# MrTornado24/IDE-3D

Measured on AMD Instinct MI355X. Metric: 512x512 RGB+seg frames/s @96 depth samples (whole job), higher is better.
Workload: dtype f32 (3x3 convs + MLPs: fp32 operands as 3 bf16 pieces, 6 products, f32 accumulate); 1 GPU; BASELINE config 2: random-init ide3d-ffhq-64-512, G.mapping + G.synthesis (64 render -> 512, 96 samples, RGB + 19-class seg) + uint8 frames, batch 4 seeds per GPU; global_batch=4, parallelism=dp1, conv_arithmetic=bf16x6, conv_arithmetic_is_library_default=True

## Files before the change

### ide-3d_amd/csrc/camera.hip

```cpp
#include "common.h"
#include "raymarch_ray.h"

namespace ide3d {

#pragma clang fp contract(off)

struct V3 { float x, y, z; };
__device__ __forceinline__ V3 normalized(V3 v) {
    const float n = sqrtf(v.x * v.x + v.y * v.y + v.z * v.z);
    return V3{v.x / n, v.y / n, v.z / n};
}
__device__ __forceinline__ V3 cross(V3 a, V3 b) { return V3{a.y * b.z - a.z * b.y, a.z * b.x - a.x * b.z, a.x * b.y - a.y * b.x}; }

__global__ void __launch_bounds__(64)
sphere_points_kernel(const float* __restrict__ theta, const float* __restrict__ pitch, int n, float r, int pitch_is_v,
                     float* __restrict__ pos, float* __restrict__ phi_out) {
    const int i = blockIdx.x * 64 + threadIdx.x;
    if (i >= n) return;
    const float kPi = 3.14159265358979323846f;
    float p = fminf(fmaxf(pitch[i], 1e-5f), (float)(3.14159265358979323846 - 1e-5));
    if (pitch[i] != pitch[i]) p = pitch[i];
    if (pitch_is_v) p = acosf(1.f - 2.f * (p * (1.f / kPi)));
    const float t = theta[i], sp = r * sinf(p);
    pos[3 * i + 0] = sp * cosf(t);
// ... 16 lines not shown
        f = V3{forward[3 * i], forward[3 * i + 1], forward[3 * i + 2]};
    }
    f = normalized(f);
    const V3 left = normalized(cross(V3{0.f, 1.f, 0.f}, f));
    const V3 up = normalized(cross(f, left));
    float* m = out + (int64_t)i * 16;
    m[0] = -left.x; m[1] = up.x; m[2]  = -f.x; m[3]  = o.x;
    m[4] = -left.y; m[5] = up.y; m[6]  = -f.y; m[7]  = o.y;
    m[8] = -left.z; m[9] = up.z; m[10] = -f.z; m[11] = o.z;
    m[12] = 0.f;    m[13] = 0.f; m[14] = 0.f;  m[15] = 1.f;
}

__global__ void __launch_bounds__(256)
plane_cells_kernel(ide3d_render_params p, int cells_h, int cells_w, int lds_cells, uint8_t* __restrict__ cells) {
    extern __shared__ __attribute__((aligned(16))) uint8_t s_cells[];
    const int n = blockIdx.y, per_img = p.rays_per_img * p.steps;
    const int i = (int)blockIdx.x * 256 + (int)threadIdx.x;
    uint8_t* const img_cells = cells + (int64_t)n * 3 * cells_h * cells_w;
    if (lds_cells) {
        for (int k = threadIdx.x * 4; k < lds_cells; k += 1024) *reinterpret_cast<uint32_t*>(s_cells + k) = 0u;
        __syncthreads();
    }
    if (i < per_img) {
        const int s = i % p.steps, r = i / p.steps;
        const float zstep = (p.steps > 1) ? (p.z_lin[1] - p.z_lin[0]) : 0.f;
        const float zl = p.z_lin[s];
        float ax, ay, az, bx, by, bz;
        ray_world_point(p, n, r, zl, 0.f, zstep, ax, ay, az);
        ray_world_point(p, n, r, zl, 1.f, zstep, bx, by, bz);
        Tap2 ta[3], tb[3];
        triplane_taps(ax, ay, az, p.W, p.H, ta);
        triplane_taps(bx, by, bz, p.W, p.H, tb);
        uint8_t* const dst = lds_cells ? s_cells : img_cells;
#pragma unroll
        for (int pl = 0; pl < 3; ++pl) {
            const int x_lo = min(max(min(ta[pl].ix0, tb[pl].ix0) - 1, 0), p.W - 1), x_hi = min(max(max(ta[pl].ix0, tb[pl].ix0) + 2, 0), p.W - 1);
            const int y_lo = min(max(min(ta[pl].iy0, tb[pl].iy0) - 1, 0), p.H - 1), y_hi = min(max(max(ta[pl].iy0, tb[pl].iy0) + 2, 0), p.H - 1);
            uint8_t* const c = dst + pl * cells_h * cells_w;
            for (int cy = y_lo >> 2; cy <= (y_hi >> 2); ++cy)
                for (int cx = x_lo >> 2; cx <= (x_hi >> 2); ++cx) c[cy * cells_w + cx] = 1;
        }
    }
    if (lds_cells) {
        __syncthreads();
        for (int k = threadIdx.x * 4; k < lds_cells; k += 1024) {
            const uint32_t v = *reinterpret_cast<const uint32_t*>(s_cells + k);
            if (v == 0u) continue;
#pragma unroll
            for (int e = 0; e < 4; ++e) if ((v >> (8 * e)) & 0xffu) img_cells[k + e] = 1;
        }
    }
}

__global__ void __launch_bounds__(1024)
plane_tile_list_kernel(ide3d_plane_gate g, int n, int tiles_y, int tiles_x, int th, int tw, int32_t* __restrict__ list) {
    __shared__ int s_wave[16];
    const int tid = threadIdx.x, lane = tid & 63, wid = tid >> 6;
    const int total = n * tiles_y * tiles_x;
    int base = 0;
    for (int t0 = 0; t0 < total; t0 += 1024) {
        const int t = t0 + tid;
        bool live = false;
        if (t < total) {
            const int tx = t % tiles_x, ty = (t / tiles_x) % tiles_y, img = t / (tiles_x * tiles_y);
            const int cy0 = (ty * th) >> 2, cy1 = min((ty * th + th - 1) >> 2, g.cells_h - 1);
            const int cx0 = (tx * tw) >> 2, cx1 = min((tx * tw + tw - 1) >> 2, g.cells_w - 1);
            for (int pl = 0; pl < 3; ++pl)
                for (int cy = cy0; cy <= cy1; ++cy)
                    for (int cx = cx0; cx <= cx1; ++cx) live |= g.cells[(((int64_t)img * 3 + pl) * g.cells_h + cy) * g.cells_w + cx] != 0;
        }
        const unsigned long long bal = __builtin_amdgcn_ballot_w64(live);
        if (lane == 0) s_wave[wid] = __popcll(bal);
        __syncthreads();
        int before = base;
        for (int w = 0; w < wid; ++w) before += s_wave[w];
        if (live) list[1 + before + __popcll(bal & ((1ull << lane) - 1ull))] = t;
        for (int w = 0; w < 16; ++w) base += s_wave[w];
        __syncthreads();
    }
    if (tid == 0) list[0] = base;
}

}

extern "C" int ide3d_plane_cells(const float* rays_d_cam, const float* z_lin, const float* cam2world, int32_t n, int32_t rays_per_img,
                                 int32_t steps, int32_t H, int32_t W, uint8_t* cells, void* stream) {
    using namespace ide3d;
    IDE3D_CHECK_ARG(rays_d_cam && z_lin && cam2world && cells, "plane_cells: null pointer");
    IDE3D_CHECK_ARG(n > 0 && rays_per_img > 0 && steps > 0 && H > 0 && W > 0, "plane_cells: bad shape");
    const int cells_h = cdiv(H, 4), cells_w = cdiv(W, 4);
    const int64_t per_img = (int64_t)rays_per_img * steps, map_bytes = 3 * (int64_t)cells_h * cells_w;
    IDE3D_CHECK_ARG(per_img < 0x7fffff00LL && n <= 65535 && n * map_bytes < 0x7fffffffLL, "plane_cells: too many samples, images or cells");
    ide3d_render_params p{};
    p.rays_d_cam = rays_d_cam; p.z_lin = z_lin; p.cam2world = cam2world;
    p.jitter = z_lin;
    p.n = n; p.rays_per_img = rays_per_img; p.steps = steps; p.H = H; p.W = W;
    hipStream_t st = (hipStream_t)stream;
    const hipError_t e = hipMemsetAsync(cells, 0, (size_t)(n * map_bytes), st);
    if (e != hipSuccess) { set_error("plane_cells: hipMemsetAsync: %s", hipGetErrorString(e)); return IDE3D_ELAUNCH; }
    const int lds_cells = (map_bytes % 4 == 0 && map_bytes <= 48 * 1024) ? (int)map_bytes : 0;
    hipLaunchKernelGGL(plane_cells_kernel, dim3((unsigned)cdiv64(per_img, 256), (unsigned)n), dim3(256), (size_t)lds_cells, st, p, cells_h, cells_w, lds_cells, cells);
    IDE3D_CHECK_LAUNCH("plane_cells");
    return IDE3D_OK;
}

extern "C" int ide3d_plane_tile_list(const ide3d_plane_gate* gate, int32_t n, int32_t h, int32_t w, int32_t tile_h, int32_t tile_w, int32_t* list, void* stream) {
    using namespace ide3d;
    IDE3D_CHECK_ARG(gate && gate->cells && list, "plane_tile_list: null pointer");
    IDE3D_CHECK_ARG(n > 0 && h > 0 && w > 0 && tile_h > 0 && tile_w > 0 && tile_h % 4 == 0 && tile_w % 4 == 0, "plane_tile_list: bad shape (tiles are multiples of the 4 x 4 cell)");
    IDE3D_CHECK_ARG(4 * (int64_t)gate->cells_h >= h && 4 * (int64_t)gate->cells_w >= w, "plane_tile_list: the cell map does not cover the output");
    const int tiles_y = cdiv(h, tile_h), tiles_x = cdiv(w, tile_w);
    IDE3D_CHECK_ARG((int64_t)n * tiles_y * tiles_x < 0x7fffffffLL, "plane_tile_list: too many tiles");
    hipLaunchKernelGGL(plane_tile_list_kernel, dim3(1), dim3(1024), 0, (hipStream_t)stream, *gate, n, tiles_y, tiles_x, tile_h, tile_w, list);
    IDE3D_CHECK_LAUNCH("plane_tile_list");
    return IDE3D_OK;
}

extern "C" int ide3d_sphere_points(const float* theta, const float* pitch, int32_t n, float r, int32_t pitch_is_v,
                                   float* pos, float* phi_out, void* stream) {
    using namespace ide3d;
    IDE3D_CHECK_ARG(theta && pitch && pos, "sphere_points: null pointer");
    IDE3D_CHECK_ARG(n > 0, "sphere_points: bad shape");
    hipLaunchKernelGGL(sphere_points_kernel, dim3(cdiv(n, 64)), dim3(64), 0, (hipStream_t)stream, theta, pitch, n, r, pitch_is_v, pos, phi_out);
    IDE3D_CHECK_LAUNCH("sphere_points");
    return IDE3D_OK;
}

extern "C" int ide3d_cam2world(const float* forward, const float* origin, const float* lookat, int32_t lookat_stride, int32_t n,
                               float* out, void* stream) {
    using namespace ide3d;
    IDE3D_CHECK_ARG(origin && out && (forward || lookat), "cam2world: null pointer");
    IDE3D_CHECK_ARG(n > 0 && (lookat_stride == 0 || lookat_stride == 3), "cam2world: bad shape");
    hipLaunchKernelGGL(cam2world_kernel, dim3(cdiv(n, 64)), dim3(64), 0, (hipStream_t)stream, forward, origin, lookat, lookat_stride, n, out);
    IDE3D_CHECK_LAUNCH("cam2world");
    return IDE3D_OK;
}
```

### ide-3d_amd/csrc/common.h

```cpp
#pragma once

#include <hip/hip_runtime.h>
#include <hip/hip_fp16.h>
#include <hip/hip_bf16.h>
#include <stdint.h>
#include <stdarg.h>
#include <stdio.h>

#include "../../include/ide3d_hip.h"

namespace ide3d {

constexpr int kWave = 64;
constexpr int kNumCU = 256;
constexpr int kNumXCD = 8;


void set_error(const char* fmt, ...);

const char* modconv_build_flags();
const char* triplane_tile_build_flags();
const char* raymarch_build_flags();

void note_exclusive_violation(const char* kernel, int blocks_per_cu);
// ... 55 lines not shown

__device__ __forceinline__ void amax_raise(float* amax, int n, float v) {
    unsigned* const slot = reinterpret_cast<unsigned*>(amax) + (size_t)n * IDE3D_AMAX_FLOATS + (blockIdx.x % IDE3D_AMAX_SLOTS) * IDE3D_AMAX_STRIDE;
    __hip_atomic_fetch_max(slot, __float_as_uint(v), __ATOMIC_RELAXED, __HIP_MEMORY_SCOPE_AGENT);
}
__device__ __forceinline__ void amax_raise_block(float* amax, int n, float v, float* scratch) {
#pragma unroll
    for (int off = 32; off > 0; off >>= 1) v = fmaxf(v, __shfl_xor(v, off));
    __syncthreads();
    if ((threadIdx.x & 63) == 0) scratch[threadIdx.x >> 6] = v;
    __syncthreads();
    if (threadIdx.x == 0) {
        float m = scratch[0];
        for (int i = 1; i < (int)(blockDim.x >> 6); ++i) m = fmaxf(m, scratch[i]);
        if (m > 0.f) amax_raise(amax, n, m);
    }
}
__device__ __forceinline__ void amax_lds_flush(unsigned* s_am, int n, float v) { if (v > 0.f) atomicMax(&s_am[n & 63], __float_as_uint(v)); }
__device__ __forceinline__ void amax_lds_commit(float* amax, const unsigned* s_am, int p_n) {
    __syncthreads();
    if ((int)threadIdx.x < p_n && threadIdx.x < 64 && s_am[threadIdx.x] != 0u) amax_raise(amax, (int)threadIdx.x, __uint_as_float(s_am[threadIdx.x]));
}

__host__ __device__ __forceinline__ int64_t cdiv64(int64_t a, int64_t b) { return (a + b - 1) / b; }
__host__ __device__ __forceinline__ int     cdiv(int a, int b) { return (a + b - 1) / b; }

__device__ __forceinline__ bool pool_gt(float v, float m) { return v > m || v != v; }

inline bool ptr_aligned(const void* p, uintptr_t bytes) { return (reinterpret_cast<uintptr_t>(p) & (bytes - 1)) == 0; }

inline int stream_grid(int64_t work_items, int per_block) {
    int64_t g = cdiv64(work_items, per_block);
    const int64_t cap = (int64_t)kNumCU * 8;
    if (g > cap) g = cap;
    if (g < 1) g = 1;
    return (int)g;
}

__device__ __forceinline__ bool plane_gate_live(const ide3d_plane_gate& g, int n, int pl0, int npl, int y0, int x0, int th, int tw) {
    const int cy0 = max(y0 >> 2, 0), cx0 = max(x0 >> 2, 0);
    const int cy1 = min((y0 + th - 1) >> 2, g.cells_h - 1), cx1 = min((x0 + tw - 1) >> 2, g.cells_w - 1);
    const int nx = cx1 - cx0 + 1, ny = cy1 - cy0 + 1;
    bool any = false;
    if (nx > 0 && ny > 0) {
        const int per = nx * ny, count = per * npl;
        for (int i = (int)(threadIdx.x & 63u); i < count; i += 64) {
            const int pl = pl0 + i / per, r = i % per;
            any |= g.cells[(((int64_t)n * 3 + pl) * g.cells_h + cy0 + r / nx) * g.cells_w + cx0 + r % nx] != 0;
        }
    }
    return __builtin_amdgcn_ballot_w64(any) != 0ull;
}
ide3d_plane_gate resolve_plane_gate(const ide3d_plane_gate* gate);

__device__ __forceinline__ int xcd_remap(int bid, int nblocks) {
    const int xcd = bid % kNumXCD;
    const int idx = bid / kNumXCD;
    const int q = nblocks / kNumXCD, r = nblocks % kNumXCD;
    const int base = (xcd < r) ? xcd * (q + 1) : r * (q + 1) + (xcd - r) * q;
    return base + idx;
}

}
```

### ide-3d_amd/csrc/core.hip

```cpp
#include "common.h"
#include "knobs.h"
#include <string.h>
#include <stdio.h>
#include <map>
#include <mutex>
#include <tuple>

namespace ide3d {

static thread_local char g_err[512] = "";

void set_error(const char* fmt, ...) {
    va_list ap;
    va_start(ap, fmt);
    vsnprintf(g_err, sizeof(g_err), fmt, ap);
    va_end(ap);
}

static int g_excl_violations = 0;
static char g_excl_text[384] = "";
void note_exclusive_violation(const char* kernel, int blocks_per_cu) {
    ++g_excl_violations;
    snprintf(g_excl_text, sizeof(g_excl_text), "%d workgroups of %.200s fit one CU of this device: exclusive residency (DESIGN.md 4.2) does not hold", blocks_per_cu, kernel);
    fprintf(stderr, "[libide3d_hip] %s; the launch is refused (select IDE3D_CONV_ARITH=fp32)\n", g_excl_text);
}
int exclusive_violations() { return g_excl_violations; }
static thread_local bool g_refused = false;
void refuse_launch(const char* kernel) {
    g_refused = true;
    set_error("%.200s: more than one workgroup fits a CU of this device, exclusive residency (DESIGN.md 4.2) does not hold; launch refused "
              "(IDE3D_CONV_ARITH=fp32 selects the arithmetic that needs none)", kernel);
}
bool take_refused() { const bool r = g_refused; g_refused = false; return r; }

bool exclusive_checked(const void* kernel, int threads, size_t dyn_lds, const char* name) {
    static std::mutex mu;
    static std::map<std::tuple<const void*, int, int, size_t>, int> table;
    int dev = 0;
    if (hipGetDevice(&dev) != hipSuccess) return true;
    int occ;
    {
        std::lock_guard<std::mutex> lock(mu);
        const auto key = std::make_tuple(kernel, dev, threads, dyn_lds);
        auto it = table.find(key);
        if (it == table.end()) {
            int n = 0;
            occ = (hipOccupancyMaxActiveBlocksPerMultiprocessor(&n, kernel, threads, dyn_lds) == hipSuccess && n > 0) ? n : -1;
            table.emplace(key, occ);
            if (occ > 1) note_exclusive_violation(name, occ);
        } else occ = it->second;
    }
    if (occ > 1) refuse_launch(name);
    return occ <= 1;
}

ide3d_plane_gate resolve_plane_gate(const ide3d_plane_gate* gate) {
    if (!gate || !gate->cells || knob_live("IDE3D_NO_PLANE_GATE")) return ide3d_plane_gate{};
    return *gate;
}

}

extern "C" int ide3d_exclusive_violations(void) { return ide3d::g_excl_violations; }
extern "C" const char* ide3d_exclusive_violation_text(void) { return ide3d::g_excl_text; }
extern "C" const char* ide3d_last_error(void) { return ide3d::g_err; }
extern "C" int ide3d_abi_version(void) { return 8; }
extern "C" const char* ide3d_build_arch(void) { return "gfx950"; }
extern "C" const char* ide3d_build_flags(void) {
    static char buf[512] = "";
    static bool done = false;
    if (!done) {
        snprintf(buf, sizeof(buf), "%s%s%s", ide3d::modconv_build_flags(), ide3d::triplane_tile_build_flags(), ide3d::raymarch_build_flags());
        const size_t n = strlen(buf);
        if (n && buf[n - 1] == ' ') buf[n - 1] = 0;
        done = true;
    }
    return buf;
}
```

### ide-3d_amd/csrc/modconv.hip

```cpp
#include "common.h"
#include "knobs.h"
#include <stdlib.h>
#include <string.h>
#include <type_traits>

namespace ide3d {

typedef float f32x16 __attribute__((ext_vector_type(16)));

#ifdef IDE3D_MC_TRACE
__device__ unsigned long long g_mc_dbg[256];
#define IDE3D_MC_TS(k) { const unsigned long long now_ = __builtin_readcyclecounter(); mc_acc[k] += now_ - mc_last; mc_last = now_; }
#else
#define IDE3D_MC_TS(k)
#endif

enum { MODE_CONV3 = 0, MODE_CONV1 = 1, MODE_TCONV3 = 2, MODE_TCONV3A = 3, MODE_CONV3S2 = 4 };

template <int MODE> struct ModeCfg;
template <> struct ModeCfg<MODE_CONV3>  { static constexpr int KC = 4, WTAPS = 9, MAXT = 9; };
template <> struct ModeCfg<MODE_CONV1>  { static constexpr int KC = 16, WTAPS = 1, MAXT = 1; };
template <> struct ModeCfg<MODE_CONV3S2> { static constexpr int KC = 4, WTAPS = 9, MAXT = 9; };
template <> struct ModeCfg<MODE_TCONV3> { static constexpr int KC = 4, WTAPS = 9, MAXT = 4; };
template <> struct ModeCfg<MODE_TCONV3A> { static constexpr int KC = 4, WTAPS = 9, MAXT = 9; };
// ... 1368 lines not shown
                                       : (TI * PH * PW <= 128 && MODE != MODE_CONV3S2) ? 3 : 2)
modconv_kernel(ide3d_modconv_params p, const float* __restrict__ wp, float* __restrict__ partial, ConvGeom g) {
    using K = McCfg<MODE, BIG, TI, PH, PW>;
    __shared__ __attribute__((aligned(16))) float s_w[2 * K::LDS_W];
    __shared__ __attribute__((aligned(16))) float s_x[2 * K::LDS_X];
    const BlockId b = decode_block(g);
    int cls = 0;
    if (MODE == MODE_TCONV3) { cls = (b.tile >= g.tile_base[1]) + (b.tile >= g.tile_base[2]) + (b.tile >= g.tile_base[3]); }
    modconv_tile<MODE, BIG, TI, PH, PW>(p, wp, partial, g, s_w, s_x, b.mb, b.tile - g.tile_base[cls], b.grp, b.split, cls, g.tiles_x[cls]);
}


#ifdef IDE3D_SP_SHARED_SIMD
constexpr bool kSpExclusive = false;
#else
constexpr bool kSpExclusive = true;
#endif
template <int MODE, int BIG, int PH, int PARTS, int WBUF, int NWV>
constexpr int sp_waves_per_simd() {
    using K = SpCfg<MODE, BIG, PH, PARTS, WBUF, NWV>;
    return (NWV == 8) ? 2 : (!kSpExclusive && K::LDS_BYTES <= 80 * 1024 && (WBUF == 1 || K::NCLS * K::MTW * K::NTW <= 8)) ? 2 : 1;
}
template <int MODE, int BIG, int PH, int PARTS, int WBUF = 2, int NWV = 4, int F16 = 0>
__global__ void __launch_bounds__(64 * NWV, (sp_waves_per_simd<MODE, BIG, PH, PARTS, WBUF, NWV>()))
modconv_split_kernel(ide3d_modconv_params p, const u32x4* __restrict__ wp, float* __restrict__ partial, ConvGeom g, const float* __restrict__ row_unscale) {
    using K = SpCfg<MODE, BIG, PH, PARTS, WBUF, NWV>;
    if constexpr (kSpExclusive) { if constexpr (NWV == 8) asm volatile("" ::: "v255"); else asm volatile("" ::: "v255", "a255"); }
    __shared__ __attribute__((aligned(16))) unsigned char sp_smem[K::LDS_BYTES];
    const BlockId b = decode_block(g);
    modconv_split_tile<MODE, BIG, PH, PARTS, WBUF, NWV, F16>(p, wp, partial, g, sp_smem, b.mb, b.tile, b.grp, b.split, g.tiles_x[0], row_unscale);
}

template <int BIG, int PH, int HEAD_MT>
__global__ void __launch_bounds__(512, 2)
modconv_split_heads_kernel(ide3d_modconv_params p, const u32x4* __restrict__ wp, ConvGeom g, HeadEpi he) {
    using K = SpCfg<MODE_CONV3, BIG, PH, 3, 2, 8>;
    if constexpr (kSpExclusive) asm volatile("" ::: "v255");
    __shared__ __attribute__((aligned(16))) unsigned char sp_smem[K::LDS_BYTES];
    BlockId b;
    if (he.gate.tile_list) {
        const int live = __builtin_amdgcn_readfirstlane(he.gate.tile_list[0]);
        if ((int)blockIdx.x >= live) return;
        const int id = __builtin_amdgcn_readfirstlane(he.gate.tile_list[1 + xcd_remap(blockIdx.x, live)]);
        b.mb = 0; b.split = 0; b.tile = id % g.tile_base[4]; b.grp = id / g.tile_base[4];
    } else {
        b = decode_block(g);
        if (he.gate.cells && !plane_gate_live(he.gate, b.grp, 0, 3, (b.tile / g.tiles_x[0]) * PH, (b.tile % g.tiles_x[0]) * K::PW, PH, K::PW)) return;
    }
    modconv_split_tile<MODE_CONV3, BIG, PH, 3, 2, 8, 0, 1, -1, HEAD_MT>(p, wp, nullptr, g, sp_smem, b.mb, b.tile, b.grp, b.split, g.tiles_x[0], nullptr, nullptr, &he);
}

template <int BIG, int PH, int PARTS, int F16 = 0>
__global__ void __launch_bounds__(512, 2)
modconv_split_pair_kernel(ide3d_modconv_params p, const u32x4* __restrict__ wp, float* __restrict__ partial, ConvGeom g, const float* __restrict__ row_unscale) {
    using K = SpCfg<MODE_TCONV3A, BIG, PH, PARTS, 2, 8, 1>;
    if constexpr (kSpExclusive) asm volatile("" ::: "v255");
    __shared__ __attribute__((aligned(16))) unsigned char sp_smem[K::LDS_BYTES];
    const int half_grid = (int)(gridDim.x >> 1);
    const int par = __builtin_amdgcn_readfirstlane((int)blockIdx.x >= half_grid ? 1 : 0);
    int bid = xcd_remap((int)blockIdx.x - par * half_grid, half_grid);
    BlockId b;
    b.mb = bid % g.mblocks; bid /= g.mblocks;
    b.tile = bid % g.tile_base[4]; bid /= g.tile_base[4];
    b.grp = bid % g.img_groups; bid /= g.img_groups;
    b.split = bid;
    if (par == 0) modconv_split_tile<MODE_TCONV3A, BIG, PH, PARTS, 2, 8, F16, 1, 0>(p, wp, partial, g, sp_smem, b.mb, b.tile, b.grp, b.split, g.tiles_x[0], row_unscale);
    else          modconv_split_tile<MODE_TCONV3A, BIG, PH, PARTS, 2, 8, F16, 1, 1>(p, wp, partial, g, sp_smem, b.mb, b.tile, b.grp, b.split, g.tiles_x[0], row_unscale);
}

template <int MODE, int BIG, int PH, int PARTS, int WBUF, int F16>
__global__ void __launch_bounds__(512, 2)
modconv_split_teams_kernel(ide3d_modconv_params p, const u32x4* __restrict__ wp, float* __restrict__ partial, ConvGeom g, const float* __restrict__ row_unscale) {
    using K = SpCfg<MODE, BIG, PH, PARTS, WBUF, 4>;
    static_assert(2 * K::LDS_BYTES <= 160 * 1024, "both teams' LDS must fit");
    asm volatile("" ::: "v255");
    __shared__ __attribute__((aligned(16))) unsigned char sp_smem[2 * K::LDS_BYTES];
    const int team = (int)(threadIdx.x >> 8);
    int bid = xcd_remap(blockIdx.x, gridDim.x);
    const int mpairs = g.mblocks >> 1;
    BlockId b;
    b.mb = 2 * (bid % mpairs) + team; bid /= mpairs;
    b.tile = bid % g.tile_base[4]; bid /= g.tile_base[4];
    b.grp = bid % g.img_groups; bid /= g.img_groups;
    b.split = bid;
    modconv_split_tile<MODE, BIG, PH, PARTS, WBUF, 4, F16, 2>(p, wp, partial, g, sp_smem + team * K::LDS_BYTES, b.mb, b.tile, b.grp, b.split, g.tiles_x[0], row_unscale,
                                                              reinterpret_cast<float*>(sp_smem));
}

__global__ void __launch_bounds__(256)
modconv_epilogue_kernel(ide3d_modconv_params p, const float* __restrict__ partial, int split_k, int oh, int ow) {
    const int64_t per = (int64_t)p.n * p.cout * oh * ow;
    const int64_t stride = (int64_t)gridDim.x * blockDim.x;
    int am_n = -1; float am = 0.f;
    __shared__ unsigned s_am[64];
    const bool am_lds = p.y_amax && p.n <= 64;
    if (p.y_amax) { if (threadIdx.x < 64) s_am[threadIdx.x] = 0u; __syncthreads(); }
    const int hw = oh * ow;
    if (p.y_pitch <= 0 && (hw & 3) == 0) {
        typedef float f32x4v __attribute__((ext_vector_type(4)));
        const int64_t per4 = per >> 2;
        for (int64_t q = (int64_t)blockIdx.x * blockDim.x + threadIdx.x; q < per4; q += stride) {
            const int64_t i = q << 2;
            f32x4v v = {0.f, 0.f, 0.f, 0.f};
            int s = 0;
            for (; s + 4 <= split_k; s += 4) {
                f32x4v t[4];
#pragma unroll
                for (int k = 0; k < 4; ++k) t[k] = *reinterpret_cast<const f32x4v*>(partial + (int64_t)(s + k) * per + i);
#pragma unroll
                for (int k = 0; k < 4; ++k) v += t[k];
            }
            for (; s < split_k; ++s) v += *reinterpret_cast<const f32x4v*>(partial + (int64_t)s * per + i);
            const int pix = (int)(i % hw);
            const int co = (int)((i / hw) % p.cout);
            const int n = (int)(i / ((int64_t)hw * p.cout));
            const float d = p.dcoefs ? p.dcoefs[(int64_t)n * p.cout + co] : 1.f, bb = p.bias ? p.bias[co] : 0.f;
#pragma unroll
            for (int e = 0; e < 4; ++e) {
// ... 200 lines not shown
        g.tiles_x[c] = cdiv(gw[c], ts.cols); g.tiles_y[c] = cdiv(gh[c], ts.rows);
        g.tile_base[c + 1] = g.tile_base[c] + (c < ncls ? g.tiles_x[c] * g.tiles_y[c] : 0);
    }
    g.img_groups = cdiv(p.n, ts.images);
    g.mblocks = pl.mblocks; g.cchunks = pl.cchunks; g.oh = pl.oh; g.ow = pl.ow;
    const int64_t base_blocks = (int64_t)g.mblocks * g.tile_base[4] * g.img_groups;
    int split = 1;
    if (base_blocks < split_min && pl.cchunks >= 8) {
        split = (int)cdiv64(768, base_blocks);
        if (split > pl.cchunks / 4) split = pl.cchunks / 4;
        if (split > 16) split = 16;
        if (split < 1) split = 1;
    }
    if (one_round) want_split = 1;
    if (want_split > 0) split = want_split < pl.cchunks ? want_split : pl.cchunks;
    g.chunks_per_split = cdiv(pl.cchunks, split);
    g.split_k = cdiv(pl.cchunks, g.chunks_per_split);
    pl.partial_floats = (g.split_k > 1) ? (int64_t)g.split_k * p.n * p.cout * pl.oh * pl.ow : 0;
}

template <int MODE, int BIG>
static void launch_tiles(const ide3d_modconv_params& p, const ConvPlan& pl, const float* wp, float* partial, hipStream_t st) {
    const ConvGeom& g = pl.g;
    const unsigned nblocks = (unsigned)((int64_t)g.mblocks * g.tile_base[4] * g.img_groups * g.split_k);
    if constexpr (MODE == MODE_TCONV3A) {
        if constexpr (BIG != 0) {
            if (pl.tile == TA8x16) hipLaunchKernelGGL((modconv_kernel<MODE, BIG, 1, 8, 16>), dim3(nblocks), dim3(256), 0, st, p, wp, partial, g);
            else if (pl.tile == TA16x16) { if constexpr (BIG == 2) hipLaunchKernelGGL((modconv_kernel<MODE, BIG, 1, 16, 16>), dim3(nblocks), dim3(256), 0, st, p, wp, partial, g); }
            else hipLaunchKernelGGL((modconv_kernel<MODE, BIG, 1, 4, 16>), dim3(nblocks), dim3(256), 0, st, p, wp, partial, g);
        }
    } else
    if (pl.tile == TFLAT128) {
        if constexpr (MODE == MODE_CONV1)
            hipLaunchKernelGGL((modconv_kernel<MODE, BIG, 1, 1, 128>), dim3(nblocks), dim3(256), 0, st, p, wp, partial, g);
    }
    else if (pl.tile == T8x16) hipLaunchKernelGGL((modconv_kernel<MODE, BIG, 1, 8, 16>), dim3(nblocks), dim3(256), 0, st, p, wp, partial, g);
    else if (pl.tile == T2x8x8) hipLaunchKernelGGL((modconv_kernel<MODE, BIG, 2, 8, 8>), dim3(nblocks), dim3(256), 0, st, p, wp, partial, g);
    else if (pl.tile == T8x4x4) hipLaunchKernelGGL((modconv_kernel<MODE, BIG, 8, 4, 4>), dim3(nblocks), dim3(256), 0, st, p, wp, partial, g);
    else if constexpr (BIG == 1 && MODE != MODE_CONV1 && MODE != MODE_CONV3S2)
        hipLaunchKernelGGL((modconv_kernel<MODE, BIG, 1, 16, 16>), dim3(nblocks), dim3(256), 0, st, p, wp, partial, g);
}


struct SpForm { int waves; bool teams; };
static SpForm sp_form(const ConvPlan& pl) {
    if constexpr (kSpExclusive) {
        if (pl.tile == TA4x16) return {4, pl.big == 2 && (pl.mblocks & 1) == 0};
        return {pl.tile == T8x16 ? 4 : 8, false};
    } else {
        return {(pl.tile == T16x16 || pl.tile == T32x16) ? 8 : 4, false};
    }
}
template <int MODE, int BIG, int PARTS, int F16 = 0>
static void launch_split(const ide3d_modconv_params& p, const ConvPlan& pl, const float* wp, float* partial, hipStream_t st) {
    const ConvGeom& g = pl.g;
    const unsigned nblocks = (unsigned)((int64_t)g.mblocks * g.tile_base[4] * g.img_groups * g.split_k);
    const u32x4* wu = reinterpret_cast<const u32x4*>(wp);
    const float* ru = F16 ? wp + pl.packed_floats + (int64_t)pl.mblocks * pl.bm : nullptr;
    if constexpr (kSpExclusive) {
        if (pl.pair) {
            if constexpr (MODE == MODE_TCONV3A) IDE3D_EXCL_LAUNCH((modconv_split_pair_kernel<BIG, (BIG == 1 ? 16 : 32), PARTS, F16>), dim3(2 * nblocks), 512, 0, st, p, wu, partial, g, ru);
        }
        else if (pl.tile == TA4x16) {
            if constexpr (MODE == MODE_TCONV3A) {
                if (sp_form(pl).teams) { if constexpr (BIG == 2) IDE3D_EXCL_LAUNCH((modconv_split_teams_kernel<MODE, BIG, 4, PARTS, 2, F16>), dim3(nblocks / 2), 512, 0, st, p, wu, partial, g, ru); }
                else IDE3D_EXCL_LAUNCH((modconv_split_kernel<MODE, BIG, 4, PARTS, 2, 4, F16>), dim3(nblocks), 256, 0, st, p, wu, partial, g, ru);
            }
        }
        else if (pl.tile == T8x16) {
            if constexpr (MODE == MODE_CONV3) IDE3D_EXCL_LAUNCH((modconv_split_kernel<MODE, BIG, 8, PARTS, 2, 4, F16>), dim3(nblocks), 256, 0, st, p, wu, partial, g, ru);
        }
        else if (pl.tile == TA8x16) {
            if constexpr (MODE == MODE_TCONV3A) IDE3D_EXCL_LAUNCH((modconv_split_kernel<MODE, BIG, 8, PARTS, 2, 8, F16>), dim3(nblocks), 512, 0, st, p, wu, partial, g, ru);
        }
        else if (pl.tile == T32x16) {
            if constexpr (MODE == MODE_CONV3 && BIG == 2) IDE3D_EXCL_LAUNCH((modconv_split_kernel<MODE, BIG, 32, PARTS, 2, 8, F16>), dim3(nblocks), 512, 0, st, p, wu, partial, g, ru);
        }
        else if constexpr (MODE == MODE_CONV3 || BIG == 2)
            IDE3D_EXCL_LAUNCH((modconv_split_kernel<MODE, BIG, 16, PARTS, 2, 8, F16>), dim3(nblocks), 512, 0, st, p, wu, partial, g, ru);
    } else {
        if (pl.tile == TA4x16) {
            if constexpr (MODE == MODE_TCONV3A) IDE3D_EXCL_LAUNCH((modconv_split_kernel<MODE, BIG, 4, PARTS, 2, 4, F16>), dim3(nblocks), 256, 0, st, p, wu, partial, g, ru);
        }
        else if (pl.tile == T8x16) {
            if constexpr (MODE == MODE_CONV3) IDE3D_EXCL_LAUNCH((modconv_split_kernel<MODE, BIG, 8, PARTS, 1, 4, F16>), dim3(nblocks), 256, 0, st, p, wu, partial, g, ru);
        }
        else if (pl.tile == TA8x16) {
            if constexpr (MODE == MODE_TCONV3A && BIG == 2) IDE3D_EXCL_LAUNCH((modconv_split_kernel<MODE, BIG, 8, PARTS, 2, 4, F16>), dim3(nblocks), 256, 0, st, p, wu, partial, g, ru);
        }
        else if (pl.tile == T16x16) {
            if constexpr (MODE == MODE_CONV3 && BIG == 1) IDE3D_EXCL_LAUNCH((modconv_split_kernel<MODE, BIG, 16, PARTS, 2, 8, F16>), dim3(nblocks), 512, 0, st, p, wu, partial, g, ru);
        }
    }
}

}

static bool head_split_applies(const ide3d_modconv_params& p, int arith) {
    return arith != 1 && p.k == 1 && p.mode == 0 && p.w_batch_stride > 0 && !p.styles && !p.dcoefs && !p.noise && p.act == 1 &&
           (p.cout <= 32 || (p.cout > 160 && p.cout <= 192)) && p.cin >= 32 &&
           (int64_t)p.n * ide3d::cdiv64((int64_t)p.h * p.w_, 32 * ide3d::head_waves(p.cout <= 32 ? 1 : 6)) >= ide3d::kNumCU;
}

static bool head_small_applies(const ide3d_modconv_params& p) {
    return p.k == 1 && p.mode == 0 && p.w_batch_stride > 0 && !p.styles && !p.dcoefs && !p.noise && p.act == 1 && (int64_t)p.h * p.w_ <= 256 &&
           p.y_pitch == 0 && p.n <= 65535;
}
static bool head_resident_applies(const ide3d_modconv_params& p) {
    const int mt = p.cout <= 32 ? 1 : 6, cchunks = ide3d::cdiv(p.cin, 16);
    const int hw = p.h * p.w_, wgs_img = ide3d::kNumCU / p.n, tiles32 = hw / 32;
    return ide3d::kSpExclusive && p.cin % 16 == 0 && hw % 32 == 0 && wgs_img >= 1 && p.y_pitch == 0 &&
           ((mt == 1 && (cchunks == 4 || cchunks == 8)) || (mt == 6 && cchunks == 8)) && tiles32 >= 2 * wgs_img * 8;
}

// ... 2 lines not shown
    IDE3D_CHECK_ARG(p.n > 0 && p.cin > 0 && p.cout > 0 && p.h > 0 && p.w_ > 0, "modconv2d: bad shape");
    IDE3D_CHECK_ARG(p.k == 1 || p.k == 3, "modconv2d: kernel size must be 1 or 3 (got %d)", p.k);
    IDE3D_CHECK_ARG(p.mode == 0 || ((p.mode == 1 || p.mode == 2) && p.k == 3),
                    "modconv2d: mode must be 0 (conv), 1 (3x3 stride-2 conv, no padding) or 2 (3x3 transposed, stride 2)");
    IDE3D_CHECK_ARG(p.mode != 1 || (p.h >= 3 && p.w_ >= 3), "modconv2d: stride-2 convolution needs an input of at least 3x3");
    IDE3D_CHECK_ARG((int64_t)p.n * p.cin * p.h * p.w_ < 0x7fffffffLL, "modconv2d: input too large for 32-bit indexing");
    return IDE3D_OK;
}

extern "C" int64_t ide3d_modconv_workspace_bytes(int32_t n, int32_t cin, int32_t cout, int32_t h, int32_t w, int32_t k, int32_t mode,
                                                 int32_t per_image_weights) {
    using namespace ide3d;
    ide3d_modconv_params p{};
    p.n = n; p.cin = cin; p.cout = cout; p.h = h; p.w_ = w; p.k = k; p.mode = mode; p.w_batch_stride = per_image_weights ? 1 : 0;
    if (check_modconv(p) != IDE3D_OK) return -1;
    p.x = nullptr;
    int64_t packed = 0, part = 0;
    static const float dummy = 0.f;
    for (int epi = 0; epi < 2; ++epi) {
        ide3d_modconv_params q0 = p;
        q0.act = 1; q0.gain = 1.f; q0.clamp = -1.f;
        if (epi == 1) { q0.noise = &dummy; q0.bias = &dummy; q0.noise_strength = 1.f; q0.act = 3; q0.alpha = 0.2f; q0.gain = 1.41421356f; }
        for (int arith : {1, 3, 6, 16}) {
            ConvPlan pl; plan_conv(q0, pl, arith);
            ConvPlan pf; plan_conv(flatten_pointwise(q0), pf, arith);
            for (const ConvPlan* q : {&pl, &pf}) {
                if (q->packed_floats + q->aux_floats > packed) packed = q->packed_floats + q->aux_floats;
                if (q->partial_floats > part) part = q->partial_floats;
            }
        }
    }
    int64_t bytes = (packed + part) * (int64_t)sizeof(float);
    if (per_image_weights && k == 1) {
        const int64_t hb = head_packed_units(n, cdiv(cin, 16), 3, cout <= 32 ? 1 : 6) * 16;
        if (hb > bytes) bytes = hb;
    }
    return bytes;
}

static void pack_split_weights(const ide3d_modconv_params& p, const ide3d::ConvPlan& pl, float* wp, hipStream_t st) {
    using namespace ide3d;
    const int64_t items = (int64_t)pl.mblocks * pl.cchunks * 9 * 2 * pl.bm;
    if (pl.f16) {
        float* const rs = wp + pl.packed_floats;
        const int rows = pl.mblocks * pl.bm;
        hipLaunchKernelGGL(modconv_row_scale_kernel, dim3(cdiv(rows, 4)), dim3(256), 0, st, p.w, p.cout, p.cin * 9, rows, rs, rs + rows);
        hipLaunchKernelGGL((modconv_pack_split_kernel<2, 1>), dim3(stream_grid(items, 256)), dim3(256), 0, st, p.w, p.cout, p.cin, pl.bm, pl.mblocks, pl.cchunks, reinterpret_cast<u32x4*>(wp), rs);
    }
    else if (pl.parts == 2) hipLaunchKernelGGL(modconv_pack_split_kernel<2>, dim3(stream_grid(items, 256)), dim3(256), 0, st, p.w, p.cout, p.cin, pl.bm, pl.mblocks, pl.cchunks, reinterpret_cast<u32x4*>(wp), nullptr);
    else               hipLaunchKernelGGL(modconv_pack_split_kernel<3>, dim3(stream_grid(items, 256)), dim3(256), 0, st, p.w, p.cout, p.cin, pl.bm, pl.mblocks, pl.cchunks, reinterpret_cast<u32x4*>(wp), nullptr);
}

extern "C" int ide3d_modconv2d(const ide3d_modconv_params* pp, void* stream) {
    using namespace ide3d;
    IDE3D_CHECK_ARG(pp != nullptr, "modconv2d: null params");
    const ide3d_modconv_params p = flatten_pointwise(*pp);
    IDE3D_CHECK_ARG(p.x && p.w && p.y && p.workspace, "modconv2d: null tensor / workspace pointer");
    int rc = check_modconv(p);
    if (rc) return rc;
    IDE3D_CHECK_ARG(p.act == 1 || p.act == 3, "modconv2d: act must be linear (1) or lrelu (3)");
    IDE3D_CHECK_ARG(p.y_pitch == 0 || (p.mode == 2 && p.y_pitch >= 2 * p.w_ + 1), "modconv2d: y_pitch is the row pitch of a transposed convolution's output (>= 2 w + 1), or 0");
    hipStream_t st_head = (hipStream_t)stream;
    {
        const int64_t hw = (int64_t)p.h * p.w_;
        if (head_small_applies(p)) {
            if (hw <= 64) hipLaunchKernelGGL((head_small_kernel<64, 32>), dim3(cdiv(p.cout, HS_RB), 1, p.n), dim3(HS_THREADS), 0, st_head, p, (int)hw);
            else          hipLaunchKernelGGL((head_small_kernel<256, 8>), dim3(cdiv(p.cout, HS_RB), cdiv((int)hw, 256), p.n), dim3(HS_THREADS), 0, st_head, p, (int)hw);
            IDE3D_CHECK_LAUNCH("modconv2d (small-map heads)");
            return IDE3D_OK;
        }
    }
    if (head_split_applies(p, resolve_arith(p.arith))) {
        const int parts = resolve_arith(p.arith) == 3 ? 2 : 3, mt = p.cout <= 32 ? 1 : 6, cchunks = cdiv(p.cin, 16);
        IDE3D_CHECK_ARG(p.workspace_bytes >= head_packed_units(p.n, cchunks, parts, mt) * 16, "modconv2d: workspace too small for the packed head weights");
        u32x4* wu = reinterpret_cast<u32x4*>(p.workspace);
        const int64_t items = (int64_t)p.n * cchunks * 2 * mt * 32;
        const int tiles = cdiv(p.h * p.w_, 32 * head_waves(mt));
        const int hw_h = p.h * p.w_, wgs_img = kNumCU / p.n, tiles32 = hw_h / 32;
        const bool resident = head_resident_applies(p);
#define IDE3D_HEAD_RES(P, M, C) IDE3D_EXCL_LAUNCH((head_resident_kernel<P, M, C>), dim3(p.n * wgs_img), 512, 0, st_head, p, wu, wgs_img, tiles32)
#define IDE3D_HEAD(P, M) do { \
            hipLaunchKernelGGL(head_pack_split_kernel<P>, dim3(stream_grid(items, 256)), dim3(256), 0, st_head, p.w, p.w_batch_stride, p.n, p.cout, p.cin, M * 32, cchunks, wu); \
            if (resident) { if (M == 6) IDE3D_HEAD_RES(P, 6, 8); else if (cchunks == 4) IDE3D_HEAD_RES(P, 1, 4); else IDE3D_HEAD_RES(P, 1, 8); } \
            else IDE3D_EXCL_LAUNCH((head_split_kernel<P, M>), dim3(p.n * tiles), 64 * head_waves(M), 0, st_head, p, wu, cchunks, tiles); } while (0)
        if (parts == 2) { if (mt == 1) IDE3D_HEAD(2, 1); else IDE3D_HEAD(2, 6); }
        else            { if (mt == 1) IDE3D_HEAD(3, 1); else IDE3D_HEAD(3, 6); }
#undef IDE3D_HEAD
#undef IDE3D_HEAD_RES
        IDE3D_CHECK_LAUNCH("modconv2d (split-bf16 heads)");
        return IDE3D_OK;
    }
    int arith_eff = resolve_arith(p.arith);
    if (arith_eff == 16 && !p.x_amax) arith_eff = 6;
    ConvPlan pl; plan_conv(p, pl, arith_eff);
    IDE3D_CHECK_ARG(p.workspace_bytes >= (pl.packed_floats + pl.aux_floats + pl.partial_floats) * (int64_t)sizeof(float),
                    "modconv2d: workspace too small (need %lld bytes)", (long long)((pl.packed_floats + pl.aux_floats + pl.partial_floats) * sizeof(float)));
    hipStream_t st = (hipStream_t)stream;
    float* wp = p.workspace;
    float* partial = p.workspace + pl.packed_floats + pl.aux_floats;
    if (pl.parts) {
        if (!p.weights_packed) pack_split_weights(p, pl, wp, st);
#define IDE3D_SP_DISPATCH(M) \
        do { if (pl.big == 1) { if (pl.f16) launch_split<M, 1, 2, 1>(p, pl, wp, partial, st); else if (pl.parts == 2) launch_split<M, 1, 2>(p, pl, wp, partial, st); else launch_split<M, 1, 3>(p, pl, wp, partial, st); } \
             else             { if (pl.f16) launch_split<M, 2, 2, 1>(p, pl, wp, partial, st); else if (pl.parts == 2) launch_split<M, 2, 2>(p, pl, wp, partial, st); else launch_split<M, 2, 3>(p, pl, wp, partial, st); } } while (0)
        if (pl.mode == MODE_CONV3) IDE3D_SP_DISPATCH(MODE_CONV3); else IDE3D_SP_DISPATCH(MODE_TCONV3A);
#undef IDE3D_SP_DISPATCH
    } else {
    if (!p.weights_packed) {
        hipLaunchKernelGGL(modconv_pack_kernel, dim3(stream_grid(pl.packed_floats, 256)), dim3(256), 0, st,
                           p.w, p.w_batch_stride, p.w_batch_stride ? p.n : 1, p.cout, p.cin, pl.taps, pl.bm, pl.kc, pl.mblocks, pl.cchunks, wp);
    }
#define IDE3D_MC_DISPATCH(M) \
    do { if (pl.big == 1) launch_tiles<M, 1>(p, pl, wp, partial, st); else if (pl.big == 2) launch_tiles<M, 2>(p, pl, wp, partial, st); \
         else launch_tiles<M, 0>(p, pl, wp, partial, st); } while (0)
    if (pl.mode == MODE_CONV3)       IDE3D_MC_DISPATCH(MODE_CONV3);
    else if (pl.mode == MODE_CONV1)  IDE3D_MC_DISPATCH(MODE_CONV1);
    else if (pl.mode == MODE_CONV3S2) IDE3D_MC_DISPATCH(MODE_CONV3S2);
    else if (pl.mode == MODE_TCONV3A) IDE3D_MC_DISPATCH(MODE_TCONV3A);
    else                             IDE3D_MC_DISPATCH(MODE_TCONV3);
#undef IDE3D_MC_DISPATCH
    }
    if (pl.g.split_k > 1) {
        const int64_t per = (int64_t)p.n * p.cout * pl.oh * pl.ow;
        hipLaunchKernelGGL(modconv_epilogue_kernel, dim3(stream_grid((p.y_pitch <= 0 && ((pl.oh * pl.ow) & 3) == 0) ? per / 4 : per, 256)), dim3(256), 0, st, p, partial, pl.g.split_k, pl.oh, pl.ow);
    }
    if (pl.mode == MODE_TCONV3A && !p.weights_packed) {
        hipLaunchKernelGGL(tconv_strip_pack_kernel, dim3(stream_grid(pl.strip_floats, 256)), dim3(256), 0, st, p.w, p.cout, p.cin, cdiv(p.cout, STRIP_CO) * STRIP_CO,
                           wp + pl.packed_floats + pl.strip_off);
    }
    if (pl.strip) {
        const int cout_pad = cdiv(p.cout, STRIP_CO) * STRIP_CO;
        float* const wstrip = wp + pl.packed_floats + pl.strip_off;
        const int nb_re = cdiv(p.w_ + 1, 64), nb_ro = cdiv(p.w_, 64), nb_ce = cdiv(p.h, 64), nb_co = cdiv(p.h, 64);
        float* const xs = wstrip + pl.strip_floats;
        hipLaunchKernelGGL(tconv_strip_gather_kernel, dim3(stream_grid((int64_t)p.n * p.cin * (p.h + p.w_), 256)), dim3(256), 0, st, p.x, p.n * p.cin, p.h, p.w_, xs);
        hipLaunchKernelGGL(tconv_strip_kernel, dim3(nb_re + nb_ro + nb_ce + nb_co, cout_pad / STRIP_CO, p.n), dim3(64 * STRIP_WAVES), 0, st, p, wstrip, xs, cout_pad,
                           pl.oh, pl.ow, (int64_t)(p.y_pitch > 0 ? p.y_pitch : pl.ow), nb_re, nb_ro, nb_ce);
    }
    IDE3D_CHECK_LAUNCH("modconv2d");
    return IDE3D_OK;
}

extern "C" int ide3d_modconv2d_heads(const ide3d_modconv_params* pp, const ide3d_modconv_head_epilogue* hp, void* stream) {
    return ide3d_modconv2d_heads_gated(pp, hp, nullptr, stream);
}

extern "C" int ide3d_modconv2d_heads_gated(const ide3d_modconv_params* pp, const ide3d_modconv_head_epilogue* hp, const ide3d_plane_gate* gate, void* stream) {
    using namespace ide3d;
    IDE3D_CHECK_ARG(pp != nullptr && hp != nullptr, "modconv2d_heads: null params");
    const ide3d_modconv_params& p = *pp;
    const ide3d_modconv_head_epilogue& h = *hp;
    IDE3D_CHECK_ARG(p.x && p.w && p.workspace && (p.y || h.no_activation_output) && h.w && h.y && h.workspace, "modconv2d_heads: null tensor / workspace pointer");
    int rc = check_modconv(p);
    if (rc) return rc;
    IDE3D_CHECK_ARG(p.act == 1 || p.act == 3, "modconv2d_heads: act must be linear (1) or lrelu (3)");
    IDE3D_CHECK_ARG(h.rows > 0, "modconv2d_heads: bad head rows");
    auto no_kernel = [](const char* why) { set_error("modconv2d_heads: %s", why); return IDE3D_ENOKERNEL; };
    if (knob_live("IDE3D_MODCONV_NO_HEAD_FUSION")) return no_kernel("IDE3D_MODCONV_NO_HEAD_FUSION is set");
    if (p.k != 3 || p.mode != 0 || p.w_batch_stride != 0 || p.y_amax || p.y_pitch != 0) return no_kernel("not a shared-weight 3x3 layer without side outputs");
    int arith = resolve_arith(p.arith);
    if (arith == 16 && !p.x_amax) arith = 6;
    if (arith != 6) return no_kernel("the fused form exists for bf16x6 only");
    ConvPlan pl; plan_conv(p, pl, arith);
    if (pl.parts != 3 || pl.f16 || pl.mode != MODE_CONV3 || pl.pair || pl.g.split_k != 1 || pl.g.mblocks != 1 || pl.bm != p.cout || kTiles[pl.tile].images != 1)
        return no_kernel("the layer's plan does not hold all channels of a tile in one workgroup");
    const bool tile16 = pl.big == 1 && p.cout == 128 && pl.tile == T16x16 && sp_form(pl).waves == 8;
    const bool tile32 = pl.big == 2 && p.cout == 64 && pl.tile == T32x16;
    const int ph = tile32 ? 32 : 16;
    if (!(tile16 || tile32) || p.h % ph != 0 || p.w_ % 16 != 0) return no_kernel("no fused instance for this tile");
    ide3d_modconv_params q{};
    q.x = p.y; q.w = h.w; q.bias = h.bias; q.y = h.y;
    q.n = p.n; q.cin = p.cout; q.cout = h.rows; q.h = p.h; q.w_ = p.w_; q.k = 1; q.mode = 0;
    q.act = 1; q.alpha = 0.f; q.gain = 1.f; q.clamp = h.clamp; q.w_batch_stride = (int64_t)h.rows * p.cout; q.arith = p.arith;
    const int mt = h.rows <= 32 ? 1 : 6, hcc = p.cout / 16;
    if (head_small_applies(q) || !head_split_applies(q, resolve_arith(q.arith)) || resolve_arith(q.arith) == 3 || (mt == 6 && !tile16))
        return no_kernel("the heads do not take the split-bf16 path");
    IDE3D_CHECK_ARG(p.workspace_bytes >= (pl.packed_floats + pl.aux_floats) * (int64_t)sizeof(float), "modconv2d_heads: workspace too small");
    IDE3D_CHECK_ARG(h.workspace_bytes >= head_packed_units(p.n, hcc, 3, mt) * 16, "modconv2d_heads: head workspace too small");
    hipStream_t st = (hipStream_t)stream;
    if (!p.weights_packed) pack_split_weights(p, pl, p.workspace, st);
    u32x4* const hw_packed = reinterpret_cast<u32x4*>(h.workspace);
    const int64_t items = (int64_t)p.n * hcc * 2 * mt * 32;
    hipLaunchKernelGGL(head_pack_split_kernel<3>, dim3(stream_grid(items, 256)), dim3(256), 0, st, h.w, q.w_batch_stride, p.n, h.rows, p.cout, mt * 32, hcc, hw_packed);
    HeadEpi e;
    e.w = hw_packed; e.bias = h.bias; e.y = h.y; e.rows = h.rows; e.clamp = h.clamp; e.store_x = !h.no_activation_output;
    e.bias_first = head_resident_applies(q) ? 1 : 0;
    e.gate = resolve_plane_gate(gate);
    if (e.gate.cells)
        IDE3D_CHECK_ARG(4 * (int64_t)e.gate.cells_h >= p.h && 4 * (int64_t)e.gate.cells_w >= p.w_, "modconv2d_heads: the plane gate's cell map does not cover the output");
    if (!e.gate.cells || e.gate.tile_h != ph || e.gate.tile_w != 16) e.gate.tile_list = nullptr;
    const ConvGeom& g = pl.g;
    const unsigned nblocks = (unsigned)((int64_t)g.mblocks * g.tile_base[4] * g.img_groups * g.split_k);
    const u32x4* wu = reinterpret_cast<const u32x4*>(p.workspace);
    if (tile32) IDE3D_EXCL_LAUNCH((modconv_split_heads_kernel<2, 32, 1>), dim3(nblocks), 512, 0, st, p, wu, g, e);
    else if (mt == 1) IDE3D_EXCL_LAUNCH((modconv_split_heads_kernel<1, 16, 1>), dim3(nblocks), 512, 0, st, p, wu, g, e);
    else IDE3D_EXCL_LAUNCH((modconv_split_heads_kernel<1, 16, 6>), dim3(nblocks), 512, 0, st, p, wu, g, e);
    IDE3D_CHECK_LAUNCH("modconv2d_heads");
    return IDE3D_OK;
}

extern "C" int ide3d_modconv_plan(const ide3d_modconv_params* pp, ide3d_modconv_plan_info* out) {
    using namespace ide3d;
    IDE3D_CHECK_ARG(pp != nullptr && out != nullptr, "modconv_plan: null argument");
    const ide3d_modconv_params p = flatten_pointwise(*pp);
    int rc = check_modconv(p);
    if (rc) return rc;
    *out = ide3d_modconv_plan_info{};
    const int arith = resolve_arith(p.arith);
    if (head_small_applies(p)) {
        const int hw = p.h * p.w_;
        out->kind = IDE3D_PLAN_HEAD_SMALL; out->tile_h = 1; out->tile_w = hw <= 64 ? 64 : 256; out->rows = HS_RB; out->waves = HS_THREADS / 64; out->split_k = 1;
        out->workgroups = (int64_t)cdiv(p.cout, HS_RB) * (hw <= 64 ? 1 : cdiv(hw, 256)) * p.n;
        return IDE3D_OK;
    }
    if (head_split_applies(p, arith)) {
        const int mt = p.cout <= 32 ? 1 : 6;
        out->rows = mt * 32; out->parts = arith == 3 ? 2 : 3; out->split_k = 1; out->tile_h = 1;
        if (head_resident_applies(p)) { out->kind = IDE3D_PLAN_HEAD_RESIDENT; out->tile_w = 32; out->waves = 8; out->workgroups = (int64_t)p.n * (kNumCU / p.n); }
        else { out->kind = IDE3D_PLAN_HEAD_SPLIT; out->waves = head_waves(mt); out->tile_w = 32 * out->waves; out->workgroups = (int64_t)p.n * cdiv(p.h * p.w_, out->tile_w); }
        return IDE3D_OK;
    }
    int arith_eff = arith;
    if (arith_eff == 16 && !p.x_amax) arith_eff = 6;
    ConvPlan pl; plan_conv(p, pl, arith_eff);
    const int64_t blocks = (int64_t)pl.g.mblocks * pl.g.tile_base[4] * pl.g.img_groups * pl.g.split_k * (pl.pair ? 2 : 1);
    out->tile_h = kTiles[pl.tile].rows; out->tile_w = kTiles[pl.tile].cols; out->images_per_tile = kTiles[pl.tile].images;
    out->rows = pl.bm; out->parts = pl.parts; out->f16 = pl.f16; out->split_k = pl.g.split_k; out->strip = pl.strip;
    out->transposed_all_class = (pl.mode == MODE_TCONV3A);
    if (pl.parts) {
        const SpForm f = sp_form(pl);
        out->kind = f.teams ? IDE3D_PLAN_SPLIT_TEAMS : IDE3D_PLAN_SPLIT; out->waves = f.teams ? 8 : f.waves; out->workgroups = f.teams ? blocks / 2 : blocks;
    } else {
        out->kind = IDE3D_PLAN_FP32; out->waves = 4; out->workgroups = blocks;
    }
    return IDE3D_OK;
}

extern "C" int ide3d_set_conv_arithmetic(int32_t arith) {
    IDE3D_CHECK_ARG(arith == 0 || arith == 1 || arith == 3 || arith == 6 || arith == 16,
                    "set_conv_arithmetic: 0 (environment default), 1 (fp32), 3 (bf16x3), 6 (bf16x6) or 16 (f16x3)");
    ide3d::g_conv_arith = arith;
    return IDE3D_OK;
}
// ... 21 lines not shown
```

### ide-3d_amd/csrc/upfirdn2d.hip

```cpp
#include "common.h"
#include "knobs.h"
#include <type_traits>

namespace ide3d {

template <class T>
__device__ __forceinline__ typename Elem<T>::math_t
apply_epilogue(typename Elem<T>::math_t v, const ide3d_upfirdn2d_epilogue& ep, int n, int c, int oy, int ox, int out_w) {
    using M = typename Elem<T>::math_t;
    if (ep.add) v += Elem<T>::ld((const T*)ep.add + n * ep.add_stride[0] + c * ep.add_stride[1] + oy * ep.add_stride[2] + ox * ep.add_stride[3]);
    if (ep.noise) v += (M)(ep.noise[oy * out_w + ox] * ep.noise_strength);
    if (ep.fused_act) {
        if (ep.bias) v += Elem<T>::ld((const T*)ep.bias + c);
        if (ep.act == 3) v = (v > 0) ? v : v * (M)ep.alpha;
        v *= (M)ep.act_gain;
        if (ep.clamp >= 0.f) v = (v > (M)ep.clamp) ? (M)ep.clamp : ((v < -(M)ep.clamp) ? -(M)ep.clamp : v);
    }
    return v;
}

template <class T, int NO>
__device__ __forceinline__ void epilogue_row(typename Elem<T>::math_t (&row)[NO], const ide3d_upfirdn2d_epilogue& ep,
                                             const T* add_plane, typename Elem<T>::math_t bias, int oy, int ox0, int out_w, bool full) {
    using M = typename Elem<T>::math_t;
// ... 415 lines not shown
            for (int wx = 0; wx < 7; ++wx) win[wy][wx] = wsrc[wy * LW + wx];
    }
    const bool has_noise = ep.noise != nullptr, act_on = ep.fused_act != 0;
    const float nstr = ep.noise_strength;
    const float bias = (act_on && ep.bias) ? ((const float*)ep.bias)[c] : 0.f;
    const bool lrelu = act_on && ep.act == 3, lrelu_max = lrelu && ep.alpha >= 0.f && ep.alpha <= 1.f;
    const float alpha = ep.alpha, again = act_on ? ep.act_gain : 1.f;
    const bool clamp_on = act_on && ep.clamp >= 0.f;
    const float cl = ep.clamp;
    float* __restrict__ yp = (float*)p.y + n * p.y_stride[0] + c * p.y_stride[1];
    const unsigned ypitch = (unsigned)p.y_stride[2];
    const int ox0 = tx_i * TCX + tx * 4, oy0 = ty_i * TCY + ty * 4;
    const bool full = ox0 + 4 <= p.out_w;
    float amax_t = 0.f;
    if (full) {
#pragma unroll
        for (int cy = 0; cy < 4; ++cy) {
            const int oy = oy0 + cy;
            if (oy >= p.out_h) break;
            float row[4];
#pragma unroll
            for (int cx = 0; cx < 4; ++cx) {
                float acc = 0.f;
#pragma unroll
                for (int ky = 0; ky < 4; ++ky)
#pragma unroll
                    for (int kx = 0; kx < 4; ++kx) acc += win[cy + ky][cx + kx] * g[ky][kx];
                row[cx] = acc;
            }
            if (has_noise) {
                const float4 a = *reinterpret_cast<const float4*>(ep.noise + ((unsigned)oy * (unsigned)p.out_w + (unsigned)ox0));
                row[0] += a.x * nstr; row[1] += a.y * nstr; row[2] += a.z * nstr; row[3] += a.w * nstr;
            }
            if (act_on) {
#pragma unroll
                for (int j = 0; j < 4; ++j) {
                    float v = row[j] + bias;
                    if (lrelu_max) v = fmaxf(v, v * alpha);
                    else if (lrelu) v = (v > 0.f) ? v : v * alpha;
                    v *= again;
                    if (clamp_on) v = (v > cl) ? cl : ((v < -cl) ? -cl : v);
                    row[j] = v;
                }
            }
#pragma unroll
            for (int j = 0; j < 4; ++j) amax_t = fmaxf(amax_t, fabsf(row[j]));
            *reinterpret_cast<float4*>(yp + ((unsigned)oy * ypitch + (unsigned)ox0)) = make_float4(row[0], row[1], row[2], row[3]);
        }
    }
    if (ep.y_amax) amax_raise_block(ep.y_amax, n, amax_t, s_in);
}

__global__ void __launch_bounds__(256)
fir_up2_kernel(ide3d_upfirdn2d_params p, ide3d_upfirdn2d_epilogue ep, int tiles_x, int tiles_y) {
    using AX = Axis<2, 1, 4>;
    constexpr int TCX = 64, TCY = 16, LW = 72, LH = TCY + 2, NV = LW / 4, NLD = (LH * NV + 255) / 256;
    static_assert(AX::window(TCX) + 3 <= LW && AX::NT == 2 && AX::window(2) == 4, "window of the 4-tap polyphase filter");
    __shared__ __attribute__((aligned(16))) float s_in[LH * LW];
    float g[4][4];
#pragma unroll
    for (int ky = 0; ky < 4; ++ky)
#pragma unroll
        for (int kx = 0; kx < 4; ++kx) {
            const int fy = p.flip ? ky : 3 - ky, fx = p.flip ? kx : 3 - kx;
            g[ky][kx] = p.f[fy * p.f_stride[0] + fx * p.f_stride[1]] * p.gain;
        }
    int bid = xcd_remap(blockIdx.x, gridDim.x);
    const int tx_i = bid % tiles_x; bid /= tiles_x;
    const int ty_i = bid % tiles_y; bid /= tiles_y;
    const int n = bid / p.c, c = bid % p.c;
    const int qx0 = floordiv(-p.pad_x0, 2) + tx_i * TCX, qy0 = floordiv(-p.pad_y0, 2) + ty_i * TCY;
    const int x_al = qx0 & ~3, xoff = qx0 - x_al;
    const float* __restrict__ xp = (const float*)p.x + n * p.x_stride[0] + c * p.x_stride[1];
    const unsigned pitch = (unsigned)p.x_stride[2];
    const int w4 = (p.in_w + 3) & ~3;
    {
        float4 v4[NLD];
        int gy[NLD], gx[NLD];
#pragma unroll
        for (int k = 0; k < NLD; ++k) {
            const int idx = (int)threadIdx.x + k * 256;
            const int ly = idx / NV, lv = idx - ly * NV;
            gy[k] = qy0 + ly; gx[k] = x_al + 4 * lv;
            const unsigned cy_ = (unsigned)min(max(gy[k], 0), p.in_h - 1), cx_ = (unsigned)min(max(gx[k], 0), w4 - 4);
            v4[k] = *reinterpret_cast<const float4*>(xp + (cy_ * pitch + cx_));
        }
#pragma unroll
        for (int k = 0; k < NLD; ++k) {
            const int idx = (int)threadIdx.x + k * 256;
            if (idx < LH * NV) {
                const bool rowok = (unsigned)gy[k] < (unsigned)p.in_h;
                float4 w = v4[k];
                w.x = (rowok && (unsigned)(gx[k] + 0) < (unsigned)p.in_w) ? w.x : 0.f;
                w.y = (rowok && (unsigned)(gx[k] + 1) < (unsigned)p.in_w) ? w.y : 0.f;
                w.z = (rowok && (unsigned)(gx[k] + 2) < (unsigned)p.in_w) ? w.z : 0.f;
                w.w = (rowok && (unsigned)(gx[k] + 3) < (unsigned)p.in_w) ? w.w : 0.f;
                *reinterpret_cast<float4*>(s_in + 4 * idx) = w;
            }
        }
    }
    __syncthreads();
    const int tx = threadIdx.x & 31, ty = threadIdx.x >> 5;
    float win[4][4];
    {
        const float* wsrc = s_in + (ty * 2) * LW + tx * 2 + xoff;
#pragma unroll
// ... 12 lines not shown
    const float* __restrict__ ap = has_add ? (const float*)ep.add + n * ep.add_stride[0] + c * ep.add_stride[1] : nullptr;
    const unsigned ypitch = (unsigned)p.y_stride[2], apitch = (unsigned)ep.add_stride[2];
    const int ox0 = (qx0 + tx * 2) * 2 + p.pad_x0;
    const bool full = ox0 >= 0 && ox0 + 4 <= p.out_w;
    float amax_t = 0.f;
    if (full) {
#pragma unroll
        for (int cy = 0; cy < 2; ++cy)
#pragma unroll
            for (int ry = 0; ry < 2; ++ry) {
                const int oy = (qy0 + ty * 2 + cy) * 2 + ry + p.pad_y0;
                if (oy < 0 || oy >= p.out_h) continue;
                float row[4];
#pragma unroll
                for (int cx = 0; cx < 2; ++cx)
#pragma unroll
                    for (int rx = 0; rx < 2; ++rx) {
                        float acc = 0.f;
#pragma unroll
                        for (int ty_ = 0; ty_ < 2; ++ty_)
#pragma unroll
                            for (int tx_ = 0; tx_ < 2; ++tx_)
                                acc += win[cy + AX::off(ry) + ty_][cx + AX::off(rx) + tx_] * g[AX::first(ry) + ty_ * 2][AX::first(rx) + tx_ * 2];
                        row[cx * 2 + rx] = acc;
                    }
                if (has_add) {
                    const float4 a = *reinterpret_cast<const float4*>(ap + ((unsigned)oy * apitch + (unsigned)ox0));
                    row[0] += a.x; row[1] += a.y; row[2] += a.z; row[3] += a.w;
                }
                if (has_noise) {
                    const float4 a = *reinterpret_cast<const float4*>(ep.noise + ((unsigned)oy * (unsigned)p.out_w + (unsigned)ox0));
                    row[0] += a.x * nstr; row[1] += a.y * nstr; row[2] += a.z * nstr; row[3] += a.w * nstr;
                }
                if (act_on) {
#pragma unroll
                    for (int j = 0; j < 4; ++j) {
                        float v = row[j] + bias;
                        if (lrelu_max) v = fmaxf(v, v * alpha);
                        else if (lrelu) v = (v > 0.f) ? v : v * alpha;
                        v *= again;
                        if (clamp_on) v = (v > cl) ? cl : ((v < -cl) ? -cl : v);
                        row[j] = v;
                    }
                }
#pragma unroll
                for (int j = 0; j < 4; ++j) amax_t = fmaxf(amax_t, fabsf(row[j]));
                *reinterpret_cast<float4*>(yp + ((unsigned)oy * ypitch + (unsigned)ox0)) = make_float4(row[0], row[1], row[2], row[3]);
            }
    }
    if (ep.y_amax) amax_raise_block(ep.y_amax, n, amax_t, s_in);
}


static bool fir44_applies(const ide3d_upfirdn2d_params& p, const ide3d_upfirdn2d_epilogue& ep) {
    const bool off = knob_live("IDE3D_FIR_NO_LEAN");
    if (off || p.dtype != IDE3D_F32 || p.f_w != 4 || p.f_h != 4 || p.up_x != 1 || p.up_y != 1 || p.down_x != 1 || p.down_y != 1) return false;
    if (p.x_stride[3] != 1 || p.y_stride[3] != 1 || ep.add || p.out_w <= 64 || (p.out_w & 3)) return false;
    const int64_t pitch = p.x_stride[2], w4 = (p.in_w + 3) & ~3;
    if ((pitch & 3) || pitch < w4 || w4 > (p.in_w > p.x_row_floats ? p.in_w : p.x_row_floats)) return false;
    if ((reinterpret_cast<uintptr_t>(p.x) & 15) || (p.x_stride[0] & 3) || (p.x_stride[1] & 3)) return false;
    if ((reinterpret_cast<uintptr_t>(p.y) & 15) || (p.y_stride[0] & 3) || (p.y_stride[1] & 3) || (p.y_stride[2] & 3)) return false;
    if (ep.noise && (reinterpret_cast<uintptr_t>(ep.noise) & 15)) return false;
    if (pitch * p.in_h >= (1ll << 29) || p.y_stride[2] * (int64_t)p.out_h >= (1ll << 29) || (int64_t)p.out_w * p.out_h >= (1ll << 29)) return false;
    if (p.x_stride[2] <= 0 || p.y_stride[2] <= 0) return false;
    return true;
}

static bool fir_up2_applies(const ide3d_upfirdn2d_params& p, const ide3d_upfirdn2d_epilogue& ep) {
    const bool off = knob_live("IDE3D_FIR_NO_LEAN");
    if (off || p.dtype != IDE3D_F32 || p.f_w != 4 || p.f_h != 4 || p.up_x != 2 || p.up_y != 2 || p.down_x != 1 || p.down_y != 1) return false;
    if (p.x_stride[3] != 1 || p.y_stride[3] != 1 || (p.out_w & 3) || (p.in_w & 3)) return false;
    if (p.pad_x0 & 1) return false;
    const int64_t pitch = p.x_stride[2];
    if ((pitch & 3) || pitch < p.in_w || pitch <= 0 || p.y_stride[2] <= 0) return false;
    if ((reinterpret_cast<uintptr_t>(p.x) & 15) || (p.x_stride[0] & 3) || (p.x_stride[1] & 3)) return false;
    if ((reinterpret_cast<uintptr_t>(p.y) & 15) || (p.y_stride[0] & 3) || (p.y_stride[1] & 3) || (p.y_stride[2] & 3)) return false;
    if (ep.add && (ep.add_stride[3] != 1 || (reinterpret_cast<uintptr_t>(ep.add) & 15) || (ep.add_stride[0] & 3) || (ep.add_stride[1] & 3) || (ep.add_stride[2] & 3) ||
                   ep.add_stride[2] <= 0 || ep.add_stride[2] * (int64_t)p.out_h >= (1ll << 29))) return false;
    if (ep.noise && (reinterpret_cast<uintptr_t>(ep.noise) & 15)) return false;
    if (pitch * p.in_h >= (1ll << 29) || p.y_stride[2] * (int64_t)p.out_h >= (1ll << 29) || (int64_t)p.out_w * p.out_h >= (1ll << 29)) return false;
    return true;
}

static bool cell_applies(const ide3d_upfirdn2d_params& p, const ide3d_upfirdn2d_epilogue& ep) {
    if (knob_live("IDE3D_FIR_NO_CELL")) return false;
    if (p.up_x != p.up_y || (p.up_x != 2 && p.up_x != 4) || p.down_x != 1 || p.down_y != 1 || ep.y_amax) return false;
    if ((int64_t)p.f_w * p.f_h < 36) return false;
    const int U = p.up_x;
    return (int64_t)cell_row_floats(cdiv(p.f_w, U), U) * (cdiv(p.f_h, U) + 1) * U * 4 <= 48 * 1024 && p.x_stride[3] * (int64_t)p.in_w < (1ll << 31);
}

static inline int cells_of(int out, int pad0, int U) {
    if (U == 1) return out;
    return floordiv(out - 1 - pad0, U) - floordiv(-pad0, U) + 1;
}

static int tile_staging(const ide3d_upfirdn2d_params& p) {
    int staged = 0, planes = 0;
    for (int n = 0; n < (p.n < 4 ? p.n : 4); ++n)
        for (int c = 0; c < (p.c < 4 ? p.c : 4); ++c, ++planes)
            staged += tile_stage16_plane(p.x_stride[2], p.in_w, p.x_row_floats,
                                         reinterpret_cast<uintptr_t>(p.x) + (uintptr_t)((n * p.x_stride[0] + c * p.x_stride[1]) * 4)) ? 1 : 0;
    return staged == planes ? 1 : staged == 0 ? 0 : 2;
}

template <int UX, int UY, int DX, int DY, int FW, int FH, int CX, int CY>
static int plan_tile(const ide3d_upfirdn2d_params& p, ide3d_upfirdn2d_plan_info* o) {
    using G = TileGeom<UX, UY, DX, DY, FW, FH, CX, CY>;
    o->form = IDE3D_UPFIRDN_TILE;
    o->ux = UX; o->uy = UY; o->dx = DX; o->dy = DY; o->fw = FW; o->fh = FH; o->cx = CX; o->cy = CY;
// ... 136 lines not shown

static int upfirdn2d_checked_plan(const ide3d_upfirdn2d_params* pp, const ide3d_upfirdn2d_epilogue* epp, ide3d_upfirdn2d_epilogue* ep_out,
                                  ide3d_upfirdn2d_plan_info* plan) {
    using namespace ide3d;
    IDE3D_CHECK_ARG(pp != nullptr, "upfirdn2d: null params");
    const ide3d_upfirdn2d_params& p = *pp;
    ide3d_upfirdn2d_epilogue ep{};
    if (epp) ep = *epp;
    IDE3D_CHECK_ARG(p.x && p.f && p.y, "upfirdn2d: null tensor pointer");
    IDE3D_CHECK_ARG(p.n > 0 && p.c > 0 && p.in_h > 0 && p.in_w > 0, "upfirdn2d: x is empty");
    IDE3D_CHECK_ARG(p.f_h >= 1 && p.f_w >= 1, "upfirdn2d: f is empty");
    IDE3D_CHECK_ARG(p.up_x >= 1 && p.up_y >= 1, "upfirdn2d: upsampling factor must be at least 1");
    IDE3D_CHECK_ARG(p.down_x >= 1 && p.down_y >= 1, "upfirdn2d: downsampling factor must be at least 1");
    IDE3D_CHECK_ARG(p.out_h >= 1 && p.out_w >= 1, "upfirdn2d: output must be at least 1x1");
    IDE3D_CHECK_ARG(!ep.fused_act || ep.act == 1 || ep.act == 3, "upfirdn2d_ex: fused activation must be linear (1) or lrelu (3)");
    if (p.dtype != IDE3D_F32 && p.dtype != IDE3D_F16 && p.dtype != IDE3D_BF16 && p.dtype != IDE3D_F64) {
        set_error("upfirdn2d: unsupported dtype code %d", p.dtype);
        return IDE3D_EINVAL;
    }
    *ep_out = ep;
    return upfirdn2d_plan(p, ep, plan);
}

static int upfirdn2d_entry(const ide3d_upfirdn2d_params* pp, const ide3d_upfirdn2d_epilogue* epp, void* stream) {
    using namespace ide3d;
    ide3d_upfirdn2d_epilogue ep;
    ide3d_upfirdn2d_plan_info plan;
    const int rc = upfirdn2d_checked_plan(pp, epp, &ep, &plan);
    if (rc != IDE3D_OK) return rc;
    const ide3d_upfirdn2d_params& p = *pp;
    hipStream_t st = (hipStream_t)stream;
    switch (p.dtype) {
    case IDE3D_F32:  return launch_planned<float>(p, ep, plan, st);
    case IDE3D_F16:  return launch_planned<__half>(p, ep, plan, st);
    case IDE3D_BF16: return launch_planned<__hip_bfloat16>(p, ep, plan, st);
    default:         return launch_planned<double>(p, ep, plan, st);
    }
}

extern "C" int ide3d_upfirdn2d_plan(const ide3d_upfirdn2d_params* pp, const ide3d_upfirdn2d_epilogue* epp, ide3d_upfirdn2d_plan_info* out) {
    using namespace ide3d;
    IDE3D_CHECK_ARG(out, "upfirdn2d_plan: null pointer");
    ide3d_upfirdn2d_epilogue ep;
    return upfirdn2d_checked_plan(pp, epp, &ep, out);
}

extern "C" int ide3d_upfirdn2d(const ide3d_upfirdn2d_params* pp, void* stream) {
    return upfirdn2d_entry(pp, nullptr, stream);
}

extern "C" int ide3d_upfirdn2d_ex(const ide3d_upfirdn2d_params* pp, const ide3d_upfirdn2d_epilogue* ep, void* stream) {
    return upfirdn2d_entry(pp, ep, stream);
}
```

### ide-3d_amd/torch_utils/hip_plugin.py

```python

import ctypes
import math
import os
import threading
import weakref

import torch

_LIB_ENV = 'IDE3D_HIP_LIB'
_ABI_VERSION = 8
AMAX_SLOTS, AMAX_STRIDE = 32, 64
AMAX_FLOATS = AMAX_SLOTS * AMAX_STRIDE

_DTYPE_CODE = {torch.float32: 0, torch.float16: 1, torch.bfloat16: 2, torch.float64: 3}

_lock = threading.Lock()
_lib = None

CALLS = {}


def lib_path():
    env = os.environ.get(_LIB_ENV)
    if env:
# ... 303 lines not shown
        lib.ide3d_build_flags.restype = ctypes.c_char_p
        lib.ide3d_build_flags.argtypes = []
        flags = lib.ide3d_build_flags().decode('ascii', 'replace').split()
        unsafe = [f for f in flags if f.startswith('!')]
        if unsafe and os.environ.get('IDE3D_ALLOW_EXPERIMENT_BUILD') != '1':
            raise RuntimeError(f'{path} was built with experiment knobs that change results or drop a safety property ({" ".join(unsafe)}); '
                               'rebuild without EXTRA=..., or set IDE3D_ALLOW_EXPERIMENT_BUILD=1 for timing experiments')
        protos = {
            'ide3d_bias_act': [vp, vp, vp, vp, vp, vp, ctypes.c_int, ctypes.c_int, ctypes.c_int, f32, f32, f32, i64, i64, i64, vp],
            'ide3d_upfirdn2d': [ctypes.POINTER(_UpfirdnParams), vp],
            'ide3d_upfirdn2d_ex': [ctypes.POINTER(_UpfirdnParams), ctypes.POINTER(_UpfirdnEpilogue), vp],
            'ide3d_upfirdn2d_plan': [ctypes.POINTER(_UpfirdnParams), ctypes.POINTER(_UpfirdnEpilogue), ctypes.POINTER(_UpfirdnPlanInfo)],
            'ide3d_filtered_lrelu': [ctypes.POINTER(_FlreluParams), vp],
            'ide3d_filtered_lrelu_act': [vp, vp, ctypes.c_int, i32, i32, i32, i32, ctypes.POINTER(i64 * 4),
                                         i32, i32, i32, i32, f32, f32, f32, ctypes.c_int, vp],
            'ide3d_triplane_sample': [vp, ctypes.POINTER(i64 * 4), i32, i32, i32, i32, vp, i64, vp, vp],
            'ide3d_triplane_sample_rays': [vp, ctypes.POINTER(i64 * 4), i32, i32, i32, i32, vp, i64, vp, i32, i32, i32, vp],
            'ide3d_triplane_taps': [i32, i32, vp, i64, vp, vp],
            'ide3d_triplane_tile_masks': [i32, i32, vp, i32, i32, i32, i32, vp, vp],
            'ide3d_triplane_sample_backward': [vp, vp, ctypes.POINTER(i64 * 4), i32, i32, i32, i32, vp, i64,
                                               vp, ctypes.POINTER(i64 * 4), vp, vp],
            'ide3d_composite': [vp, vp, vp, vp, i64, i32, i32, ctypes.c_int, ctypes.c_int, ctypes.c_int, f32,
                                ctypes.c_int, vp, vp, vp, vp],
            'ide3d_composite_plan': [vp, i64, i32, i32, ctypes.POINTER(_CompositePlanInfo)],
            'ide3d_sample_pdf': [vp, vp, vp, i64, i64, i32, i32, f32, vp, vp],
            'ide3d_render_rays': [ctypes.POINTER(_RenderParams), vp],
            'ide3d_render_ray_weights': [ctypes.POINTER(_RenderParams), vp, vp, vp, vp, vp],
            'ide3d_merge_depths': [vp, vp, i64, i32, i32, vp, vp, vp],
            'ide3d_render_rays_merged': [ctypes.POINTER(_RenderParams), vp, vp, vp, i32, vp],
            'ide3d_render_rays_backward': [ctypes.POINTER(_RenderParams), ctypes.POINTER(_RenderGrads), vp],
            'ide3d_render_param_grad_workspace_bytes': [ctypes.POINTER(_RenderParams)],
            'ide3d_render_rays_backward_params': [ctypes.POINTER(_RenderParams), ctypes.POINTER(_RenderGrads), ctypes.POINTER(_RenderParamGrads), vp],
            'ide3d_render_camera_grad_workspace_bytes': [ctypes.POINTER(_RenderParams)],
            'ide3d_render_rays_backward_camera': [ctypes.POINTER(_RenderParams), ctypes.POINTER(_RenderGrads), ctypes.POINTER(_RenderParamGrads),
                                                  ctypes.POINTER(_RenderCameraGrads), vp],
            'ide3d_render_merged_param_grad_workspace_bytes': [ctypes.POINTER(_RenderParams)],
            'ide3d_render_rays_merged_backward': [ctypes.POINTER(_RenderParams), vp, vp, vp, i32, ctypes.POINTER(_RenderGrads),
                                                  ctypes.POINTER(_RenderParamGrads), vp],
            'ide3d_sample_voxel': [ctypes.POINTER(_RenderParams), vp, i64, vp, vp, ctypes.c_int, vp],
            'ide3d_lattice_points': [ctypes.POINTER(_Lattice), i64, i64, vp, vp],
            'ide3d_density_lattice': [ctypes.POINTER(_RenderParams), ctypes.POINTER(_Lattice), i64, i64, vp, vp],
            'ide3d_mesh_workspace_bytes': [i32, i32, i32],
            'ide3d_mesh_count': [vp, i32, i32, i32, f32, vp, vp, i64, vp],
            'ide3d_mesh_emit': [vp, i32, i32, i32, f32, vp, ctypes.POINTER(_Lattice), i32, vp, i64, i64, i64, vp, vp, vp, vp],
            'ide3d_raster_workspace_bytes': [i32, i64, i32, i32],
            'ide3d_raster_project': [vp, i64, vp, i32, i32, i32, f32, f32, f32, f32, f32, f32, f32, vp, i64, vp],
            'ide3d_raster_depth': [vp, i64, i64, i32, i32, i32, i32, i32, vp, i64, vp],
            'ide3d_raster_shade': [vp, vp, i64, i32, i32, i32, vp, vp, vp, vp, i32, f32, f32, ctypes.POINTER(ctypes.c_float * 3), f32, vp, i64, vp, vp, vp, vp, vp],
            'ide3d_modconv2d': [ctypes.POINTER(_ModconvParams), vp],
            'ide3d_modconv2d_heads': [ctypes.POINTER(_ModconvParams), ctypes.POINTER(_ModconvHeadEpilogue), vp],
            'ide3d_modconv2d_heads_gated': [ctypes.POINTER(_ModconvParams), ctypes.POINTER(_ModconvHeadEpilogue), ctypes.POINTER(_PlaneGate), vp],
            'ide3d_plane_cells': [vp, vp, vp, i32, i32, i32, i32, i32, vp, vp],
            'ide3d_plane_tile_list': [ctypes.POINTER(_PlaneGate), i32, i32, i32, i32, i32, vp, vp],
            'ide3d_skip_upsample_add_cl_gated': [vp, ctypes.POINTER(i64 * 4), vp, ctypes.POINTER(i64 * 4), i32, i32, i32, i32, vp, ctypes.POINTER(_PlaneGate), vp],
            'ide3d_modconv_plan': [ctypes.POINTER(_ModconvParams), ctypes.POINTER(_ModconvPlanInfo)],
            'ide3d_modconv_workspace_bytes': [i32, i32, i32, i32, i32, i32, i32, i32],
            'ide3d_act_bwd_workspace_bytes': [i32, i32, i32, i32],
            'ide3d_modconv_act_backward': [ctypes.POINTER(_ActBwdParams), vp],
            'ide3d_modconv_scale_dot': [vp, vp, vp, vp, vp, i32, i32, i32, i32, vp, i64, vp],
            'ide3d_head_wgrad_workspace_bytes': [i32, i32, i32, i32, i32],
            'ide3d_head_weight_grad': [vp, vp, vp, i32, i32, i32, i32, i32, vp, i64, vp],
            'ide3d_wgrad_workspace_bytes': [i32, i32, i32, i32, i32],
            'ide3d_modconv_weight_grad': [ctypes.POINTER(_WgradParams), vp],
            'ide3d_bias_noise_workspace_bytes': [i32, i32, i32, i32],
            'ide3d_bias_noise_grad': [vp, vp, vp, i32, i32, i32, i32, vp, i64, vp],
            'ide3d_noise_reg_workspace_bytes': [ctypes.POINTER(i32), i32],
            'ide3d_noise_reg_levels': [ctypes.POINTER(i32), i32],
            'ide3d_noise_reg': [vp, ctypes.POINTER(i32), i32, vp, i64, vp, vp, vp],
            'ide3d_noise_reg_backward': [vp, ctypes.POINTER(i32), i32, vp, i64, vp, vp, vp, vp],
            'ide3d_noise_normalize_workspace_bytes': [ctypes.POINTER(i32), i32],
            'ide3d_noise_normalize': [vp, ctypes.POINTER(i32), i32, vp, i64, vp],
            'ide3d_lpips_prep': [vp, vp, vp, vp, i32, i32, i32, i32, f32, f32, vp],
            'ide3d_lpips_prep_backward': [vp, vp, vp, i32, i32, i32, i32, f32, vp],
            'ide3d_maxpool2': [vp, vp, i64, i32, i32, vp],
            'ide3d_lpips_stage_backward': [vp, vp, vp, vp, i64, i32, i32, vp],
            'ide3d_lpips_head_workspace_bytes': [ctypes.POINTER(_LpipsTap), i32, i32],
            'ide3d_lpips_head': [ctypes.POINTER(_LpipsTap), i32, i32, vp, i64, vp, vp],
            'ide3d_lpips_head_backward': [ctypes.POINTER(_LpipsTap), i32, i32, vp, vp],
            'ide3d_unfold2d': [vp, vp, i32, i32, i32, i32, i32, i32, i32, vp],
            'ide3d_fold2d': [vp, vp, i32, i32, i32, i32, i32, i32, i32, vp],
            'ide3d_maxpool3s2p0': [vp, vp, vp, i64, i32, i32, vp],
            'ide3d_lpips_tap_backward': [vp, vp, vp, vp, vp, i64, i32, i32, i32, vp],
            'ide3d_feat_l1_workspace_bytes': [ctypes.POINTER(_FeatL1Tap), i32, i32],
            'ide3d_feat_l1': [ctypes.POINTER(_FeatL1Tap), i32, i32, vp, i64, vp, vp],
            'ide3d_feat_l1_tap_backward': [vp, vp, vp, vp, vp, f32, i64, i32, i32, i64, vp],
            'ide3d_maxpool2_relu_backward': [vp, vp, vp, i64, i32, i32, vp],
            'ide3d_resize_bilinear': [vp, vp, i64, i32, i32, i32, i32, vp],
            'ide3d_resize_bilinear_backward': [vp, vp, i64, i32, i32, i32, i32, vp],
            'ide3d_parse_ce_workspace_bytes': [i32, i32, i32, i32, i32, i32],
            'ide3d_parse_ce': [vp, vp, i32, i32, i32, i32, i32, i32, vp, vp, i64, vp, vp],
            'ide3d_parse_ce_backward': [vp, vp, vp, vp, vp, i32, i32, i32, i32, i32, i32, vp],
            'ide3d_maxpool3s2': [vp, vp, vp, i64, i32, i32, vp],
            'ide3d_maxpool3s2_backward': [vp, vp, vp, vp, i64, i32, i32, vp],
            'ide3d_parse_join': [ctypes.POINTER(_ParseJoinParams), vp],
            'ide3d_plane_sums': [vp, vp, vp, i64, i64, f32, vp],
            'ide3d_parse_stem_backward': [vp, vp, vp, i32, i32, i32, i32, vp],
            'ide3d_id_prep': [vp, vp, i32, i32, vp],
            'ide3d_id_prep_backward': [vp, vp, i32, i32, vp],
            'ide3d_prelu': [vp, vp, vp, i32, i32, i32, i32, vp],
            'ide3d_prelu_backward': [vp, i64, i64, i32, vp, vp, vp, i32, i32, i32, i32, vp],
            'ide3d_se_gate': [vp, vp, vp, vp, i32, i32, i32, vp],
            'ide3d_se_gate_backward': [vp, vp, vp, vp, vp, vp, i32, i32, i32, vp],
            'ide3d_linear_workspace_bytes': [i32, i32, i32],
            'ide3d_linear_backward_input_workspace_bytes': [i32, i32, i32],
            'ide3d_linear': [vp, vp, vp, vp, i32, i32, i32, vp, i64, vp],
            'ide3d_linear_backward_input': [vp, vp, vp, i32, i32, i32, vp, i64, vp],
# ... 6 lines not shown
            'ide3d_frame_u8': [vp, vp, vp, i32, i32, i32, i32, vp, vp],
            'ide3d_sphere_points': [vp, vp, i32, ctypes.c_float, i32, vp, vp, vp],
            'ide3d_cam2world': [vp, vp, vp, i32, i32, vp, vp],
            'ide3d_style_demod': [vp, i64, vp, vp, vp, i32, i32, i32, i32, f32, f32, vp, vp, vp],
            'ide3d_fold_heads': [vp, i64, i32, i32, i32, f32, vp, vp, vp, i32, f32, vp, vp, vp, i32, f32, vp, vp],
            'ide3d_style_demod_batch': [ctypes.POINTER(_StyleJob), i32, i32, i32, vp],
            'ide3d_fold_heads_batch': [ctypes.POINTER(_FoldJob), i32, i32, i32, vp],
            'ide3d_mapping': [ctypes.POINTER(_MappingParams), vp],
            'ide3d_mapping_workspace_bytes': [],
            'ide3d_mapping_supported': [],
            'ide3d_skip_upsample_add_cl': [vp, ctypes.POINTER(i64 * 4), vp, ctypes.POINTER(i64 * 4), i32, i32, i32, i32, vp, vp],
            'ide3d_bilinear_up2_split': [vp, i32, i32, i32, i32, ctypes.POINTER(vp * 3), ctypes.POINTER(i32 * 3), ctypes.POINTER(i32 * 3), ctypes.POINTER(ctypes.c_int64 * 3), vp],
            'ide3d_lowres_layers_supported': [i32, i32, i32, ctypes.POINTER(i32), i32, i32],
            'ide3d_lowres_workspace_bytes': [ctypes.POINTER(_LowresParams)],
            'ide3d_lowres_group': [ctypes.POINTER(_LowresParams), vp],
        }
        for name, argtypes in protos.items():
            fn = getattr(lib, name)
            fn.restype = ctypes.c_int64 if name.endswith('_bytes') else ctypes.c_int
            fn.argtypes = argtypes
        _lib = lib
        return _lib


EXPORTED_SYMBOLS = (
    'ide3d_last_error', 'ide3d_abi_version', 'ide3d_build_arch', 'ide3d_build_flags', 'ide3d_exclusive_violations', 'ide3d_exclusive_violation_text', 'ide3d_bias_act', 'ide3d_upfirdn2d', 'ide3d_upfirdn2d_ex', 'ide3d_upfirdn2d_plan',
    'ide3d_filtered_lrelu', 'ide3d_filtered_lrelu_act', 'ide3d_triplane_sample', 'ide3d_triplane_sample_rays', 'ide3d_triplane_taps', 'ide3d_triplane_tile_masks',
    'ide3d_triplane_sample_backward', 'ide3d_composite', 'ide3d_composite_plan', 'ide3d_sample_pdf', 'ide3d_render_rays', 'ide3d_render_rays_backward', 'ide3d_sample_voxel',
    'ide3d_lattice_points', 'ide3d_density_lattice',
    'ide3d_modconv2d', 'ide3d_modconv2d_heads', 'ide3d_modconv_workspace_bytes', 'ide3d_modconv_plan', 'ide3d_set_conv_arithmetic', 'ide3d_get_conv_arithmetic', 'ide3d_frame_u8', 'ide3d_sphere_points', 'ide3d_cam2world', 'ide3d_style_demod', 'ide3d_fold_heads',
    'ide3d_style_demod_batch', 'ide3d_fold_heads_batch',
    'ide3d_skip_upsample_add_cl', 'ide3d_bilinear_up2_split', 'ide3d_mapping', 'ide3d_mapping_workspace_bytes', 'ide3d_mapping_supported',
    'ide3d_lowres_layers_supported', 'ide3d_lowres_phase_r_plan', 'ide3d_lowres_workspace_bytes', 'ide3d_lowres_group',
    'ide3d_act_bwd_workspace_bytes', 'ide3d_modconv_act_backward', 'ide3d_modconv_scale_dot', 'ide3d_head_wgrad_workspace_bytes',
    'ide3d_head_weight_grad', 'ide3d_wgrad_workspace_bytes', 'ide3d_modconv_weight_grad', 'ide3d_bias_noise_workspace_bytes',
    'ide3d_bias_noise_grad', 'ide3d_render_param_grad_workspace_bytes', 'ide3d_render_rays_backward_params',
    'ide3d_noise_reg_workspace_bytes', 'ide3d_noise_reg_levels', 'ide3d_noise_reg', 'ide3d_noise_reg_backward',
    'ide3d_noise_normalize_workspace_bytes', 'ide3d_noise_normalize',
    'ide3d_render_camera_grad_workspace_bytes', 'ide3d_render_rays_backward_camera',
    'ide3d_lpips_prep', 'ide3d_lpips_prep_backward', 'ide3d_maxpool2', 'ide3d_lpips_stage_backward', 'ide3d_lpips_head_workspace_bytes',
    'ide3d_lpips_head', 'ide3d_lpips_head_backward',
    'ide3d_unfold2d', 'ide3d_fold2d', 'ide3d_maxpool3s2p0', 'ide3d_lpips_tap_backward',
    'ide3d_feat_l1_workspace_bytes', 'ide3d_feat_l1', 'ide3d_feat_l1_tap_backward', 'ide3d_maxpool2_relu_backward',
    'ide3d_resize_bilinear', 'ide3d_resize_bilinear_backward', 'ide3d_parse_ce_workspace_bytes', 'ide3d_parse_ce', 'ide3d_parse_ce_backward',
    'ide3d_maxpool3s2', 'ide3d_maxpool3s2_backward', 'ide3d_parse_join', 'ide3d_plane_sums', 'ide3d_parse_stem_backward',
    'ide3d_id_prep', 'ide3d_id_prep_backward', 'ide3d_prelu', 'ide3d_prelu_backward', 'ide3d_se_gate', 'ide3d_se_gate_backward',
    'ide3d_linear_workspace_bytes', 'ide3d_linear_backward_input_workspace_bytes', 'ide3d_linear', 'ide3d_linear_backward_input',
    'ide3d_linear_weight_grad', 'ide3d_residual_join', 'ide3d_id_head', 'ide3d_id_head_backward',
    'ide3d_mesh_workspace_bytes', 'ide3d_mesh_count', 'ide3d_mesh_emit',
    'ide3d_render_ray_weights', 'ide3d_merge_depths', 'ide3d_render_rays_merged',
    'ide3d_render_merged_param_grad_workspace_bytes', 'ide3d_render_rays_merged_backward',
    'ide3d_raster_workspace_bytes', 'ide3d_raster_project', 'ide3d_raster_depth', 'ide3d_raster_shade',
    'ide3d_plane_cells', 'ide3d_plane_tile_list', 'ide3d_modconv2d_heads_gated', 'ide3d_skip_upsample_add_cl_gated',
)


def exclusive_violations():
    lib = load()
    lib.ide3d_exclusive_violations.restype = ctypes.c_int
    lib.ide3d_exclusive_violation_text.restype = ctypes.c_char_p
    return int(lib.ide3d_exclusive_violations()), lib.ide3d_exclusive_violation_text().decode('utf-8', 'replace')


def _check(rc, what):
    if rc == 0:
        CALLS[what] = CALLS.get(what, 0) + 1
    if rc != 0:
        msg = load().ide3d_last_error().decode('utf-8', 'replace')
        raise RuntimeError(f'{what} failed (code {rc}): {msg}')


_raw_stream = getattr(torch._C, '_cuda_getCurrentRawStream', None)


def _stream_handle(device):
    if _raw_stream is not None:
        return _raw_stream(device.index if device.index is not None else torch.cuda.current_device())
    return torch.cuda.current_stream(device).cuda_stream


def _stream(t):
    return ctypes.c_void_p(_stream_handle(t.device))


_private_streams = {}


def _hip_runtime():
    paths = _hip_runtimes_mapped()
    if len(paths) != 1:
        raise RuntimeError(f'expected exactly one HIP runtime mapped in this process, found {sorted(paths)}')
    rt = ctypes.CDLL(next(iter(paths)))
    rt.hipStreamCreateWithFlags.argtypes = [ctypes.POINTER(ctypes.c_void_p), ctypes.c_uint]
    rt.hipStreamCreateWithFlags.restype = ctypes.c_int
    return rt


def private_stream(device, purpose):
    device = torch.device(device)
    idx = device.index if device.index is not None else torch.cuda.current_device()
    key = (idx, purpose)
    st = _private_streams.get(key)
    if st is None:
        with _lock:
            st = _private_streams.get(key)
            if st is None:
# ... 118 lines not shown
        _require(b.numel() == 0 or (b.ndim == 1 and 0 <= dim < x.ndim and b.shape[0] == x.shape[dim]),
                 'b must be a vector matching dimension `dim` of x')
        _require(b.numel() == 0 or b.is_contiguous(), 'b must be contiguous')
        for name, t in (('xref', xref), ('yref', yref), ('dy', dy)):
            _require(t.numel() == 0 or (t.shape == x.shape and t.stride() == x.stride()),
                     f'{name} must have the same shape and layout as x')
        _require(grad >= 0, 'grad must be non-negative')
        _require(_dense(x) or x.numel() == 0 or x.is_non_overlapping_and_dense(), 'x must be non-overlapping and dense')
        y = torch.empty_like(x)
        _require(y.stride() == x.stride(), 'internal: output layout differs from input layout')
        if x.numel() == 0:
            return y
        step_b = x.stride(dim) if b.numel() else 1
        with _dev_guard(x.device):
            rc = load().ide3d_bias_act(_ptr(x), _ptr(b), _ptr(xref), _ptr(yref), _ptr(dy), _ptr(y),
                                       _DTYPE_CODE[x.dtype], int(grad), int(act), float(alpha), float(gain), float(clamp),
                                       x.numel(), max(b.numel(), 1), int(step_b), _stream(x))
        _check(rc, 'bias_act')
        return y



def _upfirdn_params(x_shape, x_stride, dtype, x_ptr, row_floats, f_shape, f_stride, f_ptr, upx, upy, downx, downy, padx0, padx1, pady0, pady1, flip, gain):
    _require(f_shape[0] >= 1 and f_shape[1] >= 1, 'f must be at least 1x1')
    _require(upx >= 1 and upy >= 1, 'upsampling factor must be at least 1')
    _require(downx >= 1 and downy >= 1, 'downsampling factor must be at least 1')
    n, c, ih, iw = x_shape
    ow = (iw * upx + padx0 + padx1 - f_shape[1] + downx) // downx
    oh = (ih * upy + pady0 + pady1 - f_shape[0] + downy) // downy
    _require(ow >= 1 and oh >= 1, 'output must be at least 1x1')
    cl = x_stride[1] == 1 and c > 1
    p = _UpfirdnParams()
    p.x, p.f = x_ptr, f_ptr
    p.dtype = _DTYPE_CODE[dtype]
    p.n, p.c, p.in_h, p.in_w, p.out_h, p.out_w = n, c, ih, iw, oh, ow
    p.x_stride = _i64x4(x_stride)
    p.f_h, p.f_w = f_shape
    p.f_stride = (ctypes.c_int64 * 2)(f_stride[0], f_stride[1])
    p.up_x, p.up_y, p.down_x, p.down_y = upx, upy, downx, downy
    p.pad_x0, p.pad_y0 = padx0, pady0
    p.flip, p.gain = int(bool(flip)), float(gain)
    p.x_row_floats = row_floats
    return p, (n, c, oh, ow), cl


class Upfirdn2dPlugin:

    @staticmethod
    def upfirdn2d(x, f, upx, upy, downx, downy, padx0, padx1, pady0, pady1, flip, gain):
        return Upfirdn2dPlugin.upfirdn2d_ex(x, f, upx, upy, downx, downy, padx0, padx1, pady0, pady1, flip, gain)

    @staticmethod
    def upfirdn2d_ex(x, f, upx, upy, downx, downy, padx0, padx1, pady0, pady1, flip, gain,
                     add=None, noise=None, noise_strength=1.0, bias=None, act=None, alpha=0.0, act_gain=1.0, clamp=-1.0, y_amax=None):
        _require(x.is_cuda, 'x must reside on CUDA device')
        _require(f.device == x.device, 'f must reside on the same device as x')
        _require(f.dtype == torch.float32, 'f must be float32')
        _require(x.dtype in _DTYPE_CODE, 'x must be float16, bfloat16, float32 or float64')
        _require(x.numel() > 0, 'x has zero size')
        _require(f.numel() > 0, 'f has zero size')
        _require(x.ndim == 4, 'x must be rank 4')
        _require(f.ndim == 2, 'f must be rank 2')
        p, (n, c, oh, ow), cl = _upfirdn_params(tuple(x.shape), x.stride(), x.dtype, x.data_ptr(), _row_floats_readable(x), tuple(f.shape), f.stride(), f.data_ptr(),
                                                upx, upy, downx, downy, padx0, padx1, pady0, pady1, flip, gain)
        y = torch.empty([n, c, oh, ow], dtype=x.dtype, device=x.device,
                        memory_format=torch.channels_last if cl else torch.contiguous_format)
        p.y, p.y_stride = y.data_ptr(), _i64x4(y.stride())
        plain = add is None and noise is None and act is None and y_amax is None
        with _dev_guard(x.device):
            if plain:
                rc = load().ide3d_upfirdn2d(ctypes.byref(p), _stream(x))
            else:
                ep = _UpfirdnEpilogue()
                keep = []
                if y_amax is not None:
                    _require(y_amax.is_cuda and y_amax.device == x.device and y_amax.dtype == torch.float32 and tuple(y_amax.shape) == (n, AMAX_FLOATS)
                             and y_amax.is_contiguous() and x.dtype == torch.float32, 'y_amax must be a contiguous float32 [n, AMAX_FLOATS] tensor on the device of a float32 x')
                    ep.y_amax = y_amax.data_ptr()
                if add is not None:
                    _require(add.shape == y.shape and add.dtype == x.dtype and add.device == x.device, 'add must match the output')
                    ep.add, ep.add_stride = add.data_ptr(), _i64x4(add.stride())
                if noise is not None:
                    noise = noise.to(torch.float32).contiguous(); keep.append(noise)
                    _require(tuple(noise.shape[-2:]) == (oh, ow) and noise.numel() == oh * ow, 'noise must be [out_h, out_w]')
                    ep.noise, ep.noise_strength = noise.data_ptr(), float(noise_strength)
                if act is not None:
                    ep.fused_act, ep.act = 1, int(act)
                    ep.alpha, ep.act_gain, ep.clamp = float(alpha), float(act_gain), float(clamp)
                    if bias is not None:
                        bias = bias.to(x.dtype).contiguous(); keep.append(bias)
                        _require(bias.numel() == c, 'bias must have one entry per channel')
                        ep.bias = bias.data_ptr()
                rc = load().ide3d_upfirdn2d_ex(ctypes.byref(p), ctypes.byref(ep), _stream(x))
        _check(rc, 'upfirdn2d')
        return y



class FilteredLReluPlugin:

    @staticmethod
    def filtered_lrelu(x, fu, fd, b, si, up, down, px0, px1, py0, py1, sx, sy, gain, slope, clamp, flip_filters, write_signs):
        _require(x.is_cuda, 'x must reside on CUDA device')
        _require(fu.device == x.device and fd.device == x.device and b.device == x.device,
                 'all input tensors must reside on the same device')
        _require(fu.dtype == torch.float32 and fd.dtype == torch.float32, 'fu and fd must be float32')
        _require(b.dtype == x.dtype, 'x and b must have the same dtype')
        _require(x.dtype in (torch.float16, torch.float32, torch.bfloat16), 'x and b must be float16, bfloat16 or float32')
        _require(x.ndim == 4, 'x must be rank 4')
        _require(x.numel() > 0, 'x is empty')
        _require(fu.ndim in (1, 2) and fd.ndim in (1, 2), 'fu and fd must be rank 1 or 2')
        _require(fu.numel() > 0, 'fu is empty')
        _require(fd.numel() > 0, 'fd is empty')
        _require(b.ndim == 1 and b.shape[0] == x.shape[1], 'b must be a vector with the same number of channels as x')
        _require(up >= 1 and down >= 1, 'up and down must be at least 1')
        n, c, xh, xw = x.shape
        fut_w, fut_h = fu.shape[-1] - 1, fu.shape[0] - 1
        fdt_w, fdt_h = fd.shape[-1] - 1, fd.shape[0] - 1
        cw = xw * up + (px0 + px1) - fut_w
        ch = xh * up + (py0 + py1) - fut_h
        _require(cw > fdt_w and ch > fdt_h, 'upsampled buffer must be at least the size of downsampling filter')
        yw = (cw - fdt_w + (down - 1)) // down
        yh = (ch - fdt_h + (down - 1)) // down
        _require(yw > 0 and yh > 0, 'output must be at least 1x1')
        read_signs = si.numel() > 0
        so = torch.empty([0], dtype=torch.uint8, device=x.device)
        s = si
        sw_active = 0
        if write_signs:
            sw_active = yw * down - (down - 1) + fdt_w
            sh = yh * down - (down - 1) + fdt_h
            sw = (sw_active + 15) & ~15
            s = so = torch.empty([n, c, sh, sw >> 2], dtype=torch.uint8, device=x.device)
        elif read_signs:
            sw_active = s.shape[3] << 2
        if read_signs or write_signs:
            _require(s.is_contiguous(), 'signs must be contiguous')
            _require(s.dtype == torch.uint8, 'signs must be uint8')
            _require(s.device == x.device, 'signs must reside on the same device as x')
            _require(s.ndim == 4, 'signs must be rank 4')
            _require(s.shape[0] == n and s.shape[1] == c, 'signs must have same batch & channels as x')
        cl = x.stride(1) == 1 and c > 1
        y = torch.empty([n, c, yh, yw], dtype=x.dtype, device=x.device,
                        memory_format=torch.channels_last if cl else torch.contiguous_format)
        p = _FlreluParams()
        p.x, p.y, p.b = x.data_ptr(), y.data_ptr(), b.contiguous().data_ptr()
# ... 446 lines not shown
        if count:
            with _dev_guard(tex_planes.device):
                rc = load().ide3d_density_lattice(ctypes.byref(p), ctypes.byref(lat), int(first), int(count), _ptr(sig), _stream(tex_planes))
            if rc == -2:
                return None
            _check(rc, 'density_lattice')
        return sig


class ModconvPlugin:
    _ws = _Workspaces(limit=1024)
    _heads_declined = set()

    @staticmethod
    def _workspace(lib, x, w, n, cin, cout, h, wd, k, mode, per_image, arith):
        key = (0 if per_image else w.data_ptr(), tuple(w.shape), n, h, wd, mode, x.device.index, _ws_domain(x.device), arith)
        def alloc():
            nbytes = lib.ide3d_modconv_workspace_bytes(n, cin, cout, h, wd, k, mode, int(per_image))
            _require(nbytes >= 0, 'modconv2d: unsupported configuration')
            return torch.empty([max(nbytes // 4, 1)], dtype=torch.float32, device=x.device)
        return ModconvPlugin._ws.entry(key, alloc)

    @staticmethod
    def _params(lib, x, w, y, styles, dcoefs, noise, noise_strength, bias, act, alpha, gain, clamp, mode, arith, x_amax, y_amax):
        n, cin, h, wd = x.shape
        per_image = (w.ndim == 5)
        cout, _, k, _ = w.shape[-4:]
        ent = ModconvPlugin._workspace(lib, x, w, n, cin, cout, h, wd, k, mode, per_image, arith)
        p = _ModconvParams()
        p.x, p.w, p.y = x.data_ptr(), w.data_ptr(), (y.data_ptr() if y is not None else None)
        keep = []
        for name, t in (('styles', styles), ('dcoefs', dcoefs), ('noise', noise), ('bias', bias)):
            if t is not None:
                t = t.contiguous(); keep.append(t)
                _require(t.is_cuda and t.dtype == torch.float32, f'modconv2d: {name} must be float32 on GPU')
                _require(t.device == x.device, f'modconv2d: {name} must reside on the same device as x')
                setattr(p, name, t.data_ptr())
        p.n, p.cin, p.cout, p.h, p.w_, p.k = n, cin, cout, h, wd, k
        p.noise_strength = float(noise_strength)
        p.act, p.alpha, p.gain, p.clamp = int(act), float(alpha), float(gain), float(clamp)
        p.mode = mode
        p.weights_packed = int((not per_image) and ModconvPlugin._ws.packed(ent, (w,))[0])
        p.w_batch_stride = (cout * cin * k * k) if per_image else 0
        p.arith = arith
        for name, t in (('x_amax', x_amax), ('y_amax', y_amax)):
            if t is not None:
                _require(t.is_cuda and t.device == x.device and t.dtype == torch.float32 and tuple(t.shape) == (n, AMAX_FLOATS) and t.is_contiguous(),
                         f'modconv2d: {name} must be a contiguous float32 [n, AMAX_FLOATS] tensor on the device of x')
                setattr(p, name, t.data_ptr())
        p.workspace, p.workspace_bytes = ent[0].data_ptr(), ent[0].numel() * 4
        return p, ent, keep

    @staticmethod
    def modconv2d(x, w, styles, dcoefs, noise, noise_strength, bias, act, alpha, gain, clamp, mode=0, arith=0, x_amax=None, y_amax=None, pad_rows=False):
        for t in (x, w):
            _require(t.is_cuda and t.dtype == torch.float32 and t.is_contiguous(), 'modconv2d: contiguous float32 CUDA tensors required')
        _require(w.device == x.device, 'modconv2d: w must reside on the same device as x')
        n, cin, h, wd = x.shape
        per_image = (w.ndim == 5)
        if per_image:
            _require(w.shape[0] == n and styles is None, 'modconv2d: per-image weights need w.shape[0] == batch and styles=None')
        cout, cin2, k, k2 = w.shape[-4:]
        _require(cin == cin2 and k == k2 and k in (1, 3), 'modconv2d: weight must be [cout, cin, k, k] with k in {1, 3}')
        _require(mode in (0, 1, 2), 'modconv2d: mode must be 0, 1 or 2')
        _require(mode != 1 or (k == 3 and h >= 3 and wd >= 3), 'modconv2d: mode 1 is a 3x3 stride-2 convolution on an input of at least 3x3')
        oh, ow = (2 * h + 1, 2 * wd + 1) if mode == 2 else (((h - 3) // 2 + 1, (wd - 3) // 2 + 1) if mode == 1 else (h, wd))
        pitch = (ow + 3) // 4 * 4 if (pad_rows and mode == 2) else ow
        y = torch.empty([n, cout, oh, pitch], dtype=torch.float32, device=x.device)
        lib = load()
        arith = int(arith) or int(lib.ide3d_get_conv_arithmetic())
        if arith == 16 and x_amax is None:
            arith = 6
        p, ent, keep = ModconvPlugin._params(lib, x, w, y, styles, dcoefs, noise, noise_strength, bias, act, alpha, gain, clamp, mode, arith, x_amax, y_amax)
        p.y_pitch = pitch if pitch != ow else 0
        with _dev_guard(x.device):
            rc = lib.ide3d_modconv2d(ctypes.byref(p), _stream(x))
        _check(rc, 'modconv2d')
        ModconvPlugin._ws.mark_packed(ent, () if per_image else (w,))
        return y if pitch == ow else y[..., :ow]

    @staticmethod
    def modconv2d_heads(x, w, styles, dcoefs, noise, noise_strength, bias, act, alpha, gain, clamp, head_w, head_bias, head_clamp,
                        want_x=True, arith=0, gate=None, heads_out=None):
        for t in (x, w, head_w):
            _require(t.is_cuda and t.dtype == torch.float32 and t.is_contiguous(), 'modconv2d_heads: contiguous float32 CUDA tensors required')
        n, cin, h, wd = x.shape
        cout = w.shape[0]
        _require(w.ndim == 4 and tuple(w.shape[1:]) == (cin, 3, 3), 'modconv2d_heads: w must be [cout, cin, 3, 3]')
        _require(head_w.ndim == 5 and head_w.shape[0] == n and head_w.shape[2] == cout and tuple(head_w.shape[3:]) == (1, 1),
                 'modconv2d_heads: head_w must be [n, rows, cout, 1, 1]')
        lib = load()
        arith = int(arith) or int(lib.ide3d_get_conv_arithmetic())
        if arith == 16:
            arith = 6
        rows = head_w.shape[1]
        shape_key = (n, cin, cout, h, wd, rows, arith)
        knob_off = 'IDE3D_MODCONV_NO_HEAD_FUSION' in os.environ
        if knob_off or shape_key in ModconvPlugin._heads_declined:
            return None
        y = torch.empty([n, cout, h, wd], dtype=torch.float32, device=x.device) if want_x else None
        heads = torch.empty([n, rows, h, wd], dtype=torch.float32, device=x.device) if heads_out is None else heads_out
        _require(heads.dtype == torch.float32 and heads.device == x.device and tuple(heads.shape) == (n, rows, h, wd) and heads.is_contiguous(),
                 'modconv2d_heads: heads_out must be a contiguous float32 [n, rows, h, w] tensor on the device of x')
        p, ent, keep = ModconvPlugin._params(lib, x, w, y, styles, dcoefs, noise, noise_strength, bias, act, alpha, gain, clamp, 0, arith, None, None)
        hent = ModconvPlugin._workspace(lib, heads, head_w, n, cout, rows, h, wd, 1, 0, True, arith)
        e = _ModconvHeadEpilogue()
        e.w, e.y, e.rows, e.clamp, e.no_activation_output = head_w.data_ptr(), heads.data_ptr(), rows, float(head_clamp), int(not want_x)
        if head_bias is not None:
            head_bias = head_bias.contiguous()
            _require(head_bias.is_cuda and head_bias.dtype == torch.float32 and head_bias.numel() == rows, 'modconv2d_heads: head_bias must be float32 [rows] on GPU')
            e.bias = head_bias.data_ptr()
        e.workspace, e.workspace_bytes = hent[0].data_ptr(), hent[0].numel() * 4
        with _dev_guard(x.device):
            if gate is not None:
                rc = lib.ide3d_modconv2d_heads_gated(ctypes.byref(p), ctypes.byref(e), ctypes.byref(_plane_gate(gate, n, h, wd)), _stream(x))
            else:
                rc = lib.ide3d_modconv2d_heads(ctypes.byref(p), ctypes.byref(e), _stream(x))
        if rc == -2:
            ModconvPlugin._heads_declined.add(shape_key)
            return None
        _check(rc, 'modconv2d_heads')
        ModconvPlugin._ws.mark_packed(ent, (w,))
        return y, heads


class ModconvGradPlugin:

    @staticmethod
    def _f32(t, name, dev, shape=None):
# ... 1219 lines not shown

    @staticmethod
    def mapping(z, c, embed_w, embed_b, embed_wgain, embed_bgain, fc_ws, fc_bs, lr_multiplier, alpha, act_gain, num_ws, w_avg, psi, cutoff, trusted=False):
        dev = z.device
        if trusted:
            _require(z.is_cuda and z.dtype == torch.float32 and z.is_contiguous() and (c is None or (c.device == dev and c.dtype == torch.float32 and c.is_contiguous()
                                                                                                 and tuple(c.shape) == (z.shape[0], embed_w.shape[1]))),
                     'mapping: z / c must be contiguous float32 tensors on one CUDA device, c [n, c_dim]')
            return MappingPlugin._launch(z, c, embed_w, embed_b, embed_wgain, embed_bgain, fc_ws, fc_bs, lr_multiplier, alpha, act_gain, num_ws, w_avg, psi, cutoff)
        f32c = lambda t: t is None or (t.is_cuda and t.device == dev and t.dtype == torch.float32 and t.is_contiguous())
        _require(all(f32c(t) for t in (z, c, embed_w, embed_b, w_avg, *fc_ws, *fc_bs)), 'mapping: contiguous float32 tensors on one CUDA device required')
        n, z_dim = z.shape
        embed = 0 if embed_w is None else embed_w.shape[0]
        _require(MappingPlugin.supports(n, z_dim, embed, [w.shape[0] for w in fc_ws], device=dev), 'mapping: unsupported shape')
        _require((embed_w is None) or (c is not None and embed_w.ndim == 2 and tuple(c.shape) == (n, embed_w.shape[1])),
                 f'mapping: c must be [{n}, {None if embed_w is None else embed_w.shape[1]}] (got {None if c is None else tuple(c.shape)})')
        _require(embed_b is None or (embed_w is not None and tuple(embed_b.shape) == (embed,)), 'mapping: embed bias must be [embed]')
        _require(w_avg is None or w_avg.numel() == fc_ws[-1].shape[0], 'mapping: w_avg must have w_dim elements')
        _require(num_ws >= 1, 'mapping: num_ws must be positive')
        k = z_dim + embed
        for w, b in zip(fc_ws, fc_bs):
            _require(w.ndim == 2 and w.shape[1] == k and (b is None or tuple(b.shape) == (w.shape[0],)), 'mapping: layer widths do not chain')
            k = w.shape[0]
        return MappingPlugin._launch(z, c, embed_w, embed_b, embed_wgain, embed_bgain, fc_ws, fc_bs, lr_multiplier, alpha, act_gain, num_ws, w_avg, psi, cutoff)

    @staticmethod
    def _launch(z, c, embed_w, embed_b, embed_wgain, embed_bgain, fc_ws, fc_bs, lr_multiplier, alpha, act_gain, num_ws, w_avg, psi, cutoff):
        dev = z.device
        n, z_dim = z.shape
        embed = 0 if embed_w is None else embed_w.shape[0]
        k = fc_ws[-1].shape[0]
        lib = load()
        wsp = MappingPlugin._ws.entry((dev.index, _ws_domain(dev)), lambda: torch.zeros([lib.ide3d_mapping_workspace_bytes() // 4 + 4], dtype=torch.float32, device=dev))[0]
        out = torch.empty([n, num_ws, k], dtype=torch.float32, device=dev)
        p = _MappingParams()
        p.z, p.c = z.data_ptr(), (c.data_ptr() if c is not None else 0)
        p.embed_w, p.embed_b = (embed_w.data_ptr() if embed_w is not None else 0), (embed_b.data_ptr() if embed_b is not None else 0)
        for i, (w, b) in enumerate(zip(fc_ws, fc_bs)):
            p.fc_w[i], p.fc_b[i], p.fc_out[i] = w.data_ptr(), (b.data_ptr() if b is not None else 0), w.shape[0]
        p.w_avg = w_avg.data_ptr() if w_avg is not None else 0
        p.ws, p.workspace, p.workspace_bytes = out.data_ptr(), wsp.data_ptr(), wsp.numel() * 4
        p.n, p.z_dim, p.c_dim, p.embed, p.layers, p.num_ws = n, z_dim, (c.shape[1] if c is not None else 0), embed, len(fc_ws), num_ws
        p.embed_weight_gain, p.embed_bias_gain, p.lr_multiplier = float(embed_wgain), float(embed_bgain), float(lr_multiplier)
        p.alpha, p.act_gain, p.truncation_psi = float(alpha), float(act_gain), float(psi)
        p.truncation_cutoff = -1 if cutoff is None else (int(cutoff) if cutoff >= 0 else max(num_ws + int(cutoff), 0))
        with _dev_guard(dev):
            rc = lib.ide3d_mapping(ctypes.byref(p), _stream(z))
        _check(rc, 'mapping')
        return out


class _PlaneGate(ctypes.Structure):
    _fields_ = [('cells', ctypes.c_void_p), ('cells_h', ctypes.c_int32), ('cells_w', ctypes.c_int32),
                ('tile_list', ctypes.c_void_p), ('tile_h', ctypes.c_int32), ('tile_w', ctypes.c_int32)]


def _plane_gate(gate, n, h, w):
    cells, tiles, tile_hw = gate if isinstance(gate, tuple) else (gate, None, None)
    _require(cells.is_cuda and cells.dtype == torch.uint8 and cells.is_contiguous() and tuple(cells.shape) == (n, 3, (h + 3) // 4, (w + 3) // 4),
             f'plane gate: cells must be a contiguous uint8 CUDA tensor [{n}, 3, {(h + 3) // 4}, {(w + 3) // 4}], got {list(cells.shape)} {cells.dtype}')
    g = _PlaneGate()
    g.cells, g.cells_h, g.cells_w = cells.data_ptr(), cells.shape[2], cells.shape[3]
    if tiles is not None:
        th, tw = tile_hw
        _require(tiles.is_cuda and tiles.dtype == torch.int32 and tiles.is_contiguous() and tiles.device == cells.device
                 and tiles.numel() == 1 + n * (-(-h // th)) * (-(-w // tw)), 'plane gate: the tile list must be plane_tile_list(cells, h, w, tile_h, tile_w)')
        g.tile_list, g.tile_h, g.tile_w = tiles.data_ptr(), th, tw
    return g


def plane_tile_list(cells, h, w, tile_h, tile_w):
    n = cells.shape[0]
    g = _plane_gate(cells, n, h, w)
    out = torch.empty([1 + n * (-(-h // tile_h)) * (-(-w // tile_w))], dtype=torch.int32, device=cells.device)
    with _dev_guard(cells.device):
        rc = load().ide3d_plane_tile_list(ctypes.byref(g), n, int(h), int(w), int(tile_h), int(tile_w), _ptr(out), _stream(cells))
    _check(rc, 'plane_tile_list')
    return out


def plane_cells(rays_d_cam, z_lin, cam2world, H, W):
    for t in (rays_d_cam, z_lin, cam2world):
        _require(t.is_cuda and t.dtype == torch.float32 and t.is_contiguous(), 'plane_cells: contiguous float32 CUDA tensors required')
    _require(rays_d_cam.ndim == 2 and rays_d_cam.shape[1] == 3 and z_lin.ndim == 1 and cam2world.ndim == 3 and tuple(cam2world.shape[1:]) == (4, 4),
             'plane_cells: rays_d_cam [R, 3], z_lin [S], cam2world [n, 4, 4]')
    n = cam2world.shape[0]
    cells = torch.empty([n, 3, (H + 3) // 4, (W + 3) // 4], dtype=torch.uint8, device=cam2world.device)
    with _dev_guard(cells.device):
        rc = load().ide3d_plane_cells(_ptr(rays_d_cam), _ptr(z_lin), _ptr(cam2world), n, rays_d_cam.shape[0], z_lin.shape[0], int(H), int(W),
                                      _ptr(cells), _stream(cells))
    _check(rc, 'plane_cells')
    return cells


class ResamplePlugin:
    @staticmethod
    def skip_upsample_add_cl(lo, add, gate=None, out=None):
        _require(lo.is_cuda and lo.dtype == torch.float32 and add.dtype == torch.float32 and add.device == lo.device,
                 'skip_upsample_add_cl: float32 CUDA tensors on one device required')
        n, c, h, w = lo.shape
        _require(tuple(add.shape) == (n, c, 2 * h, 2 * w), 'skip_upsample_add_cl: add must be [n, c, 2h, 2w]')
        _require(c % 4 == 0, 'skip_upsample_add_cl: channel count must be a multiple of 4')
        if out is None:
            out = torch.empty([n, c, 2 * h, 2 * w], dtype=torch.float32, device=lo.device, memory_format=torch.channels_last)
        _require(out.dtype == torch.float32 and out.device == lo.device and tuple(out.shape) == (n, c, 2 * h, 2 * w)
                 and out.is_contiguous(memory_format=torch.channels_last), 'skip_upsample_add_cl: out must be a channels_last float32 [n, c, 2h, 2w] tensor')
        with _dev_guard(lo.device):
            if gate is not None:
                rc = load().ide3d_skip_upsample_add_cl_gated(_ptr(lo), ctypes.byref(_i64x4(lo.stride())), _ptr(add), ctypes.byref(_i64x4(add.stride())),
                                                             n, c, h, w, _ptr(out), ctypes.byref(_plane_gate(gate, n, 2 * h, 2 * w)), _stream(lo))
            else:
                rc = load().ide3d_skip_upsample_add_cl(_ptr(lo), ctypes.byref(_i64x4(lo.stride())), _ptr(add), ctypes.byref(_i64x4(add.stride())),
                                                       n, c, h, w, _ptr(out), _stream(lo))
        _check(rc, 'skip_upsample_add_cl')
        return out

    @staticmethod
    def bilinear_up2_split(x, ranges, adjacent=None):
        _require(x.is_cuda and x.dtype == torch.float32, 'bilinear_up2_split: float32 CUDA tensor required')
        _require(1 <= len(ranges) <= 3, 'bilinear_up2_split: one to three channel ranges')
        x = x.contiguous()
        n, c, h, w = x.shape
        outs = [None if (adjacent and k in adjacent) else torch.empty([n, cnt, 2 * h, 2 * w], dtype=torch.float32, device=x.device) for k, (_b, cnt) in enumerate(ranges)]
        bs = [0, 0, 0]
        if adjacent:
            i, j = adjacent
            _require(j == i + 1 and 0 <= i and j < len(ranges), 'bilinear_up2_split: adjacent outputs must be consecutive')
            ci, cj = ranges[i][1], ranges[j][1]
            both = torch.empty([n, ci + cj, 2 * h, 2 * w], dtype=torch.float32, device=x.device)
            outs[i], outs[j] = both[:, :ci], both[:, ci:]
            bs[i] = bs[j] = (ci + cj) * 4 * h * w
# ... 115 lines not shown
```

### ide-3d_amd/training/graph_cache.py

```python

import collections
import contextlib
import os
import threading
import warnings
import weakref

import torch

_tls = threading.local()
_caches = weakref.WeakKeyDictionary()
_pools = {}

STATS = collections.Counter()


_PASS_ENV = ('IDE3D_NO_SKIP_MERGE', 'IDE3D_NO_STYLE_PREFETCH', 'IDE3D_NO_STYLE_BATCH', 'IDE3D_NO_LOWRES_GROUP', 'IDE3D_NO_PLANE_GATE')


def _env_int(name, default):
    try:
        return int(os.environ.get(name, default))
    except ValueError:
        return default


def enabled():
    return os.environ.get('IDE3D_AUTO_GRAPH', '1') != '0' and not getattr(_tls, 'off', 0)


@contextlib.contextmanager
def disabled():
    _tls.off = getattr(_tls, 'off', 0) + 1
    try:
        yield
    finally:
        _tls.off -= 1


def reset(module=None):
    if module is None:
        for c in list(_caches.values()):
            c.clear()
    elif module in _caches:
        _caches[module].clear()


def stats(module):
    c = _caches.get(module)
    return {'graphs': 0 if c is None else len(c.entries), 'seen': 0 if c is None else len(c.seen)}


def tree_stamp(root):
    acc = []
    push = acc.append
    requires_grad = False
    hooked = False
    stack = [root]
    while stack:
        m = stack.pop()
        if m._forward_hooks or m._forward_pre_hooks:
            hooked = True
        for p in m._parameters.values():
            if p is not None:
                push(p._version); push(p.data_ptr())
                if p.requires_grad:
                    requires_grad = True
        for b in m._buffers.values():
            if b is not None:
                push(b._version); push(b.data_ptr())
# ... 254 lines not shown
```

### ide-3d_amd/training/networks.py

```python

import math

import numpy as np
import torch

from dnnlib import util
from torch_utils import custom_ops
from torch_utils import misc
from torch_utils import persistence
from torch_utils.ops import bias_act
from torch_utils.ops import conv2d_resample
from torch_utils.ops import fma
from torch_utils.ops import upfirdn2d

_modconv_plugin = None

use_hip_modconv = True


def _upfirdn_plugin():
    upfirdn2d._init()
    return upfirdn2d._plugin


# ... 480 lines not shown


def _adjacent_views(a, b):
    if a is None or b is None or a._base is None or a._base is not b._base:
        return None
    t = a._base
    if (t.ndim != 4 or a.ndim != 4 or b.ndim != 4 or not t.is_contiguous() or t.shape[1] != a.shape[1] + b.shape[1]
            or a.shape[0] != t.shape[0] or a.shape[2:] != t.shape[2:] or b.shape[0] != t.shape[0] or b.shape[2:] != t.shape[2:]
            or a.stride() != t.stride() or b.stride() != t.stride()
            or a.data_ptr() != t.data_ptr() or b.data_ptr() != t.data_ptr() + a.shape[1] * t.stride(1) * t.element_size()):
        return None
    return t


def _dual_head_weights(torgb, toseg, w):
    wcat = _take_prefetched(torgb, w) if _prefetch_table() else None
    if wcat is None:
        wcat = _folded_head_weights(torgb, toseg, w)
    if wcat is None:
        s_rgb = torgb.affine(w) * torgb.weight_gain
        s_seg = toseg.affine(w) * toseg.weight_gain
        wr = torgb.weight[None, :, :, 0, 0] * s_rgb[:, None, :]
        ws = toseg.weight[None, :, :, 0, 0] * s_seg[:, None, :]
        wcat = torch.cat([wr, ws], dim=1)[:, :, :, None, None].contiguous()
    return wcat


def _dual_head(x, torgb, toseg, w, wcat=None):
    if (hip_conv_grad and torch.is_grad_enabled() and torgb.weight.shape[2] == 1 and torgb.conv_clamp == toseg.conv_clamp and x.ndim == 4
            and w.ndim == 2 and w.shape[0] == x.shape[0] and x.numel() < 2 ** 31
            and x.shape[0] * (torgb.weight.shape[0] + toseg.weight.shape[0]) * x.shape[2] * x.shape[3] < 2 ** 31
            and _conv_grad_ok(x, w, *_head_params(torgb, toseg))):
        y = _DualHeadGrad.apply(x, _dual_head_weights(torgb, toseg, w), _cat_cached(torgb.bias, toseg.bias),
                                -1.0 if torgb.conv_clamp is None else torgb.conv_clamp)
        co = torgb.weight.shape[0]
        return y[:, :co], y[:, co:]
    if not (use_hip_modconv and torgb.weight.shape[2] == 1 and torgb.conv_clamp == toseg.conv_clamp
            and _inference_on_gpu(x, w, *_head_params(torgb, toseg)) and _modconv_init()):
        return None
    n = x.shape[0]
    if w.shape[0] != n:
        return None
    if wcat is None:
        wcat = _dual_head_weights(torgb, toseg, w)
    bias = _cat_cached(torgb.bias, toseg.bias)
    clamp = -1.0 if torgb.conv_clamp is None else torgb.conv_clamp
    y = _modconv_plugin.modconv2d(x.contiguous(), wcat, None, None, None, 0.0, bias, 1, 0.0, 1.0, clamp)
    co = torgb.weight.shape[0]
    return y[:, :co], y[:, co:]


class PlaneGate:

    def __init__(self, cells):
        self.cells, self.taken = cells, False
        self._lists = {}

    def with_tiles(self, h, w, tile_h, tile_w):
        from torch_utils import hip_plugin
        key = (h, w, tile_h, tile_w)
        if key not in self._lists:
            self._lists[key] = hip_plugin.plane_tile_list(self.cells, h, w, tile_h, tile_w)
        return self.cells, self._lists[key], (tile_h, tile_w)


def _conv1_dual_head(block, x, w1, w_shared, want_x, noise_mode='random', gain=1, input_noise=None, _plane_gate=None, **unused):
    c1, tr, ts = block.conv1, block.torgb, block.toseg
    if not (use_hip_modconv and type(c1) is SynthesisLayer and c1.up == 1 and c1.padding == 1 and c1.weight.shape[2:] == (3, 3)
            and c1.activation in ('linear', 'lrelu') and tr.weight.shape[2] == 1 and tr.conv_clamp == ts.conv_clamp
            and x.ndim == 4 and x.shape[0] == w1.shape[0] == w_shared.shape[0]
            and _inference_on_gpu(x, w1, w_shared, *_layer_params(c1), *_head_params(tr, ts))
            and not _hooked(block, c1, tr, ts) and _modconv_init()):
        return None
    from torch_utils import hip_plugin
    if hip_plugin.conv_arithmetic() != 'bf16x6':
        return None
    noise = None
    if c1.use_noise and noise_mode != 'none':
        if input_noise is not None or noise_mode != 'const' or tuple(c1.noise_const.shape) != tuple(x.shape[2:]):
            return None
        noise = _scaled_const_noise(c1.noise_const, c1.noise_strength)
    styles, dcoefs = _styles_and_dcoefs(c1.affine, w1, c1.weight, True)
    if dcoefs is None:
        dcoefs = _demod_coefs(c1.weight, styles)
    spec = bias_act.activation_funcs[c1.activation]
    act_gain = c1.act_gain * gain
    act_clamp = c1.conv_clamp * gain if c1.conv_clamp is not None else None
    bias = c1.bias.to(x.dtype)
    wcat = _dual_head_weights(tr, ts, w_shared)
    hbias = _cat_cached(tr.bias, ts.bias)
    hclamp = -1.0 if tr.conv_clamp is None else tr.conv_clamp
    xc = x.contiguous()
    gate = None
    if _plane_gate is not None and not want_x:
        gate = _plane_gate.with_tiles(x.shape[2], x.shape[3], 16 if c1.weight.shape[0] == 128 else 32, 16)
    out = _modconv_plugin.modconv2d_heads(xc, c1.weight.contiguous(), styles.contiguous(), dcoefs, noise, 1.0, bias,
                                          spec.cuda_idx, spec.def_alpha, act_gain, -1.0 if act_clamp is None else act_clamp,
                                          wcat, hbias, hclamp, want_x=want_x, gate=gate)
    if gate is not None and out is not None:
        _plane_gate.taken = True
    if out is None:
        x = _modconv_bias_act(x, c1.weight, styles, True, noise, 1.0, bias, c1.activation, act_gain, act_clamp, dcoefs=dcoefs)
        return x, _dual_head(x, tr, ts, w_shared, wcat=wcat)
    x, y = out
    co = tr.weight.shape[0]
    return x, (y[:, :co], y[:, co:])


_lowres_plugin = None


def _lowres_init():
    global _lowres_plugin
    if _lowres_plugin is None:
        _lowres_plugin = custom_ops.get_plugin(module_name='lowres_plugin', sources=['lowres.hip'])
    return True


def _hooked(*modules):
    from torch.nn.modules import module as _m
    if _m._global_forward_hooks or _m._global_forward_pre_hooks:
        return True
    return any(m._forward_hooks or m._forward_pre_hooks for m in modules)


def lowres_group_forward(blocks, ws_per_block, noise_mode='const', force_fp32=False, **other_kwargs):
    if os.environ.get('IDE3D_NO_LOWRES_GROUP') or not use_hip_modconv or other_kwargs or noise_mode not in ('const', 'none'):
        return None
    if not blocks or len(blocks) != len(ws_per_block):
        return None
    b0 = blocks[0]
    ws0 = ws_per_block[0]
    if not (torch.is_tensor(ws0) and ws0.is_cuda and ws0.dtype == torch.float32) or (torch.is_grad_enabled() and ws0.requires_grad):
        return None
    if b0.in_channels != 0 or b0.use_single_layer or not hasattr(b0, 'const') or not _inference_on_gpu(b0.const, b0.conv1.weight):
        return None
    from torch_utils import hip_plugin
    if hip_plugin.conv_arithmetic() not in ('bf16x6', 'bf16x3'):
        return None
    C, n = b0.out_channels, ws0.shape[0]
    if C % 32 != 0 or n > 8:
        return None
    cand = []
    for bi, blk in enumerate(blocks):
        ok = (blk.architecture == 'skip' and not blk.use_single_layer and blk.out_channels == C and (bi == 0 or blk.in_channels == C)
              and not (blk.use_fp16 and not force_fp32) and not getattr(blk, 'skip_channels_last', False)
              and blk.torgb.conv_clamp == blk.toseg.conv_clamp and blk.torgb.weight.shape[2] == 1 and blk._filter_is_1331()
              and blk.resolution == b0.resolution << bi
              and not _hooked(blk, blk.conv1, blk.torgb, blk.toseg, *([blk.conv0] if bi else [])))
        if ok and torch.is_grad_enabled():
            ok = _inference_on_gpu(ws_per_block[bi], *([blk.const] if bi == 0 else _layer_params(blk.conv0)), *_layer_params(blk.conv1),
                                   *_head_params(blk.torgb, blk.toseg))
        if not ok:
            break
# ... 314 lines not shown
        x = None
        with torch.autograd.profiler.record_function('input'):
            if self.z_dim > 0:
                misc.assert_shape(z, [None, self.z_dim])
                x = normalize_2nd_moment(z.to(torch.float32))
            if self.c_dim > 0:
                misc.assert_shape(c, [None, self.c_dim])
                y = normalize_2nd_moment(self.embed(c.to(torch.float32)))
                x = torch.cat([x, y], dim=1) if x is not None else y
        for idx in range(self.num_layers):
            x = getattr(self, f'fc{idx}')(x)
        if self.training and self.w_avg_beta is not None and not skip_w_avg_update:
            self._track_w_avg(x)
        if self.num_ws is not None:
            x = x[:, None, :].repeat(1, self.num_ws, 1)
        return self._truncate(x, truncation_psi, truncation_cutoff)

    def _track_w_avg(self, w):
        batch_mean = w.detach().mean(dim=0)
        self.w_avg.copy_(torch.lerp(batch_mean, self.w_avg, self.w_avg_beta))

    def _truncate(self, ws, psi, cutoff):
        if psi == 1:
            return ws
        assert self.w_avg_beta is not None, 'truncation needs the tracked w_avg'
        if cutoff is None or self.num_ws is None:
            return torch.lerp(self.w_avg, ws, psi)
        ws[:, :cutoff] = torch.lerp(self.w_avg, ws[:, :cutoff], psi)
        return ws


@persistence.persistent_class
class SynthesisLayer(torch.nn.Module):

    def __init__(self, in_channels, out_channels, w_dim, resolution, kernel_size=3, up=1, use_noise=True,
                 activation='lrelu', resample_filter=[1, 3, 3, 1], conv_clamp=None, channels_last=False, **unused_kwargs):
        super().__init__()
        self.resolution = resolution
        self.up = up
        self.use_noise = use_noise
        self.activation = activation
        self.conv_clamp = conv_clamp
        self.register_buffer('resample_filter', upfirdn2d.setup_filter(resample_filter))
        self.padding = kernel_size // 2
        self.act_gain = bias_act.activation_funcs[activation].def_gain
        self.affine = FullyConnectedLayer(w_dim, in_channels, bias_init=1)
        memory_format = torch.channels_last if channels_last else torch.contiguous_format
        self.weight = torch.nn.Parameter(torch.randn([out_channels, in_channels, kernel_size, kernel_size]).to(memory_format=memory_format))
        if use_noise:
            self.register_buffer('noise_const', torch.randn([resolution, resolution]))
            self.noise_strength = torch.nn.Parameter(torch.zeros([]))
        self.bias = torch.nn.Parameter(torch.zeros([out_channels]))

    def forward(self, x, w, noise_mode='random', fused_modconv=True, gain=1, input_noise=None, **unused_kwargs):
        assert noise_mode in ['random', 'const', 'none']
        styles, dcoefs_pre = _styles_and_dcoefs(self.affine, w, self.weight, True)
        if styles.size(0) < x.size(0):
            dcoefs_pre = None
            assert x.size(0) % styles.size(0) == 0
            styles = styles.repeat_interleave(x.size(0) // styles.size(0), dim=0)

        noise = None
        const_noise = False
        if self.use_noise:
            if input_noise is not None:
                noise = input_noise * self.noise_strength
            elif noise_mode == 'random':
                noise = torch.randn([x.shape[0], 1, self.up * x.shape[2], self.up * x.shape[3]], device=x.device) * self.noise_strength
            elif noise_mode == 'const':
                const_noise = self.noise_const.shape[-1] >= self.up * x.shape[3]
                noise = _scaled_const_noise(self.noise_const, self.noise_strength)
                if not const_noise:
                    noise = noise.repeat(1, self.up * x.shape[3] // noise.shape[-1])

        act_gain = self.act_gain * gain
        act_clamp = self.conv_clamp * gain if self.conv_clamp is not None else None

        if hip_conv_grad and torch.is_grad_enabled() and input_noise is None and (noise is None or const_noise):
            y = _synthesis_layer_grad(self, x, styles, dcoefs_pre, noise, act_gain, act_clamp)
            if y is not None:
                return y
        if (self.up == 2 and use_hip_modconv and self.weight.shape[2] == 3 and self.padding == 1
                and _inference_on_gpu(x, self.weight, styles, self.bias, noise) and _modconv_init()):
            dcoefs = dcoefs_pre if dcoefs_pre is not None else _demod_coefs(self.weight, styles)
            xc = x.contiguous()
            y = _modconv_plugin.modconv2d(xc, self.weight.contiguous(), styles.contiguous(), dcoefs,
                                          None, 0.0, None, 1, 0.0, 1.0, -1.0, mode=2, x_amax=(_amax_of(x) if xc is x else None), pad_rows=True)
            spec = bias_act.activation_funcs[self.activation]
            if self.activation in ('linear', 'lrelu') and (noise is None or (noise.ndim == 2 and noise.shape == (2 * x.shape[2], 2 * x.shape[3]))):
                amax = _amax_wanted(y)
                return _with_amax(_upfirdn_plugin().upfirdn2d_ex(y, self.resample_filter, 1, 1, 1, 1, 1, 1, 1, 1, False, 4.0,
                                                                 noise=noise, noise_strength=1.0, bias=self.bias, act=spec.cuda_idx,
                                                                 alpha=spec.def_alpha, act_gain=act_gain,
                                                                 clamp=(-1.0 if act_clamp is None else act_clamp), y_amax=amax), amax)
            y = upfirdn2d.upfirdn2d(y, self.resample_filter, padding=[1, 1, 1, 1], gain=4)
            if noise is not None:
                y = y.add_(noise)
            return bias_act.bias_act(y, self.bias.to(x.dtype), act=self.activation, gain=act_gain, clamp=act_clamp)
        if self.up == 1:
            if noise is None or (const_noise and input_noise is None and noise.shape == x.shape[2:]):
                y = _modconv_bias_act(x, self.weight, styles, True, noise, 1.0,
                                      self.bias.to(x.dtype), self.activation, act_gain, act_clamp, dcoefs=dcoefs_pre)
                if y is not None:
                    return y
        x = modulated_conv2d(x=x, weight=self.weight, styles=styles, noise=noise, up=self.up, padding=self.padding,
                             resample_filter=(self.resample_filter if self.up > 1 else None), flip_weight=(self.up == 1),
                             fused_modconv=(fused_modconv and not _inference_on_gpu(x, self.weight, styles)))
        return bias_act.bias_act(x, self.bias.to(x.dtype), act=self.activation, gain=act_gain, clamp=act_clamp)


@persistence.persistent_class
class ToRGBLayer(torch.nn.Module):

    def __init__(self, in_channels, out_channels, w_dim, kernel_size=1, conv_clamp=None, channels_last=False, **unused):
        super().__init__()
        self.conv_clamp = conv_clamp
        self.affine = FullyConnectedLayer(w_dim, in_channels, bias_init=1)
        memory_format = torch.channels_last if channels_last else torch.contiguous_format
        self.weight = torch.nn.Parameter(torch.randn([out_channels, in_channels, kernel_size, kernel_size]).to(memory_format=memory_format))
        self.bias = torch.nn.Parameter(torch.zeros([out_channels]))
        self.weight_gain = 1 / np.sqrt(in_channels * (kernel_size ** 2))

    def forward(self, x, w, fused_modconv=True):
        styles = self.affine(w) * self.weight_gain
        if x.size(0) > styles.size(0):
            assert x.size(0) % styles.size(0) == 0
            styles = styles.repeat_interleave(x.size(0) // styles.size(0), dim=0)
        y = _modconv_bias_act(x, self.weight, styles, False, None, 0.0, self.bias.to(x.dtype), 'linear', 1.0, self.conv_clamp)
        if y is not None:
            return y
        x = modulated_conv2d(x=x, weight=self.weight, styles=styles, demodulate=False, fused_modconv=fused_modconv)
        return bias_act.bias_act(x, self.bias.to(x.dtype), clamp=self.conv_clamp)


@persistence.persistent_class
class SegSynthesisBlock(torch.nn.Module):

    def __init__(self, in_channels, out_channels, w_dim, resolution, img_channels, seg_channels, is_last,
                 architecture='skip', resample_filter=[1, 3, 3, 1], conv_clamp=None, use_fp16=False,
                 fp16_channels_last=False, use_single_layer=False, disable_upsample=False, **layer_kwargs):
        assert architecture in ['orig', 'skip']
        super().__init__()
        self.in_channels, self.out_channels = in_channels, out_channels
        self.w_dim, self.resolution = w_dim, resolution
        self.img_channels, self.seg_channels = img_channels, seg_channels
        self.is_last, self.architecture = is_last, architecture
        self.use_fp16 = use_fp16
# ... 23 lines not shown
            self.num_toseg += 1

    def _merge_skip(self, skip, x):
        if skip is None:
            return None
        if skip.size(-1) * 2 == x.size(-1):
            return upfirdn2d.upsample2d(skip, self.resample_filter)
        if skip.size(-1) == x.size(-1):
            return skip
        raise NotImplementedError

    def _accumulate(self, lo, cur, y, gate=None):
        if lo is not None:
            if (getattr(self, 'skip_channels_last', False) and lo.shape[1] % 4 == 0 and self.resample_filter.shape == (4, 4)
                    and _inference_on_gpu(lo, y) and self._filter_is_1331() and _resample_init()):
                return _resample_plugin.skip_upsample_add_cl(lo, y, gate=(gate.cells if gate is not None and lo.shape[1] % 96 == 0 else None))
            f = self.resample_filter
            return _upfirdn_plugin().upfirdn2d_ex(lo, f, 2, 2, 1, 1, 2, 1, 2, 1, False, 4.0, add=y)
        return cur.add_(y) if cur is not None else y

    def _filter_is_1331(self):
        ok = getattr(self, '_f1331', None)
        if ok is None:
            ref = upfirdn2d.setup_filter([1, 3, 3, 1])
            ok = self._f1331 = bool(torch.equal(self.resample_filter.detach().cpu(), ref))
        return ok

    def forward(self, x, img, seg, ws, force_fp32=False, fused_modconv=None, block_noise=None, disable_rgb=False, **layer_kwargs):
        misc.assert_shape(ws, [None, self.num_conv + self.num_torgb, self.w_dim])
        resume_after_conv0 = bool(layer_kwargs.pop('_resume_after_conv0', False))
        x_unused = bool(layer_kwargs.pop('_x_unused', False))
        plane_gate = layer_kwargs.pop('_plane_gate', None)
        ws_list = ws.unbind(dim=1)
        w_iter = iter(ws_list)
        dtype = torch.float16 if self.use_fp16 and not force_fp32 else torch.float32
        memory_format = torch.channels_last if self.channels_last and not force_fp32 else torch.contiguous_format
        out_dtype = dtype
        if dtype == torch.float16 and ws.is_cuda and not torch.is_grad_enabled() and use_hip_modconv:
            dtype, memory_format = torch.float32, torch.contiguous_format
        if fused_modconv is None:
            with misc.suppress_tracer_warnings():
                fused_modconv = (not self.training) and (dtype == torch.float32 or int(ws.shape[0]) == 1)

        fused = fused_heads = None
        if self.in_channels == 0:
            x = self.const.to(dtype=dtype, memory_format=memory_format)
            x = x.unsqueeze(0).expand(ws.shape[0], *x.size())
            if not self.use_single_layer:
                layer_kwargs['input_noise'] = block_noise[:, 1:2] if block_noise is not None else None
                x = self.conv1(x, next(w_iter), fused_modconv=fused_modconv, **layer_kwargs)
        else:
            x = x.to(dtype=dtype, memory_format=memory_format)
            layer_kwargs['input_noise'] = block_noise[:, 0:1] if block_noise is not None else None
            if resume_after_conv0:
                next(w_iter)
            else:
                x = self.conv0(x, next(w_iter), fused_modconv=fused_modconv, **layer_kwargs)
            if not self.use_single_layer:
                layer_kwargs['input_noise'] = block_noise[:, 1:2] if block_noise is not None else None
                w1 = next(w_iter)
                if (self.is_last or self.architecture == 'skip') and not disable_rgb and dtype == torch.float32:
                    fused = _conv1_dual_head(self, x, w1, ws_list[self.num_conv], not x_unused, _plane_gate=plane_gate, **layer_kwargs)
                if fused is not None:
                    x, fused_heads = fused
                else:
                    x = self.conv1(x, w1, fused_modconv=fused_modconv, **layer_kwargs)

        w_shared = next(w_iter) if (self.is_last or self.architecture == 'skip') else None
        ref = x if x is not None else fused_heads[0]
        img_lo = seg_lo = None
        heads_follow = (self.is_last or self.architecture == 'skip') and not disable_rgb
        if (heads_follow and _inference_on_gpu(ref, img, seg, w_shared, *_head_params(self.torgb, self.toseg)) and img is not None and seg is not None
                and img.size(-1) * 2 == ref.size(-1)):
            img_lo, seg_lo, img, seg = img, seg, None, None
        else:
            img = self._merge_skip(img, ref)
            seg = self._merge_skip(seg, ref)
        if self.is_last or self.architecture == 'skip':
            if disable_rgb:
                img = seg = None
            else:
                heads = fused_heads if fused_heads is not None else _dual_head(x, self.torgb, self.toseg, w_shared)
                if heads is not None:
                    y, y_seg = heads
                else:
                    y = self.torgb(x, w_shared, fused_modconv=fused_modconv).to(dtype=torch.float32, memory_format=torch.contiguous_format)
                    y_seg = self.toseg(x, w_shared, fused_modconv=fused_modconv).to(dtype=torch.float32, memory_format=torch.contiguous_format)
                lo_both, y_both = _adjacent_views(img_lo, seg_lo), _adjacent_views(y, y_seg)
                if (lo_both is not None and y_both is not None and img is None and seg is None and not getattr(self, 'skip_channels_last', False)
                        and not self.is_last and not os.environ.get('IDE3D_NO_SKIP_MERGE')):
                    both = self._accumulate(lo_both, None, y_both)
                    img, seg = both[:, :y.shape[1]], both[:, y.shape[1]:]
                else:
                    skip_gate = plane_gate if (plane_gate is not None and plane_gate.taken) else None
                    img = self._accumulate(img_lo, img, y, gate=skip_gate)
                    seg = self._accumulate(seg_lo, seg, y_seg, gate=skip_gate)
        assert x is None or x.dtype == dtype
        if x is not None and out_dtype != dtype:
            x = x.to(out_dtype)
        assert img is None or img.dtype == torch.float32
        assert seg is None or seg.dtype == torch.float32
        return x, img, seg
```

### ide-3d_amd/training/triplane.py

```python

import contextlib
import dataclasses
import math
import os
from typing import Dict, List, Optional

import numpy as np
import torch

from dnnlib import util
from torch_utils import misc
from torch_utils import persistence
from torch_utils.ops import bias_act
from training import graph_cache
from training import networks
from training import volumetric_rendering as vr

fused_render_grad = True

fused_render_param_grad = False

fused_render_camera_grad = False

fused_hierarchical = False
# ... 378 lines not shown
            up = lambda t: torch.nn.functional.interpolate(t, size=(size, size), mode='bilinear', align_corners=False)
            x = up(feat[:, :fc])
            img = up(feat[:, :self.img_channels])
            seg = up(feat[:, fc:])
        last = len(self.block_resolutions) - 1
        for i, (res, cur_ws) in enumerate(zip(self.block_resolutions, block_ws)):
            extra = dict(_x_unused=True) if i == last else {}
            x, img, seg = getattr(self, f'b{res}')(x, img, seg, cur_ws, **block_kwargs, **extra)
        return img, seg

    def forward(self, ws, c=None, render_params=None, noise_mode='const', return_seg=False, return_raw=False,
                return_dict=False, force_fp32=False, cond_img=None, ray_jitter=None, cached_planes=None, **unused):
        assert c is not None, 'synthesis needs the 25-D camera label c'
        render_params = dict(render_params or {})
        flags = (bool(return_seg), bool(return_raw), bool(return_dict))

        def impl(ws_, c_, jitter_, planes_):
            return self._forward_impl(ws_, c_, render_params, noise_mode, flags, force_fp32, jitter_, planes_)

        if torch.is_tensor(ws) and ws.is_cuda:
            return graph_cache.run(self, impl, ws, c, render_params, noise_mode, flags, force_fp32, ray_jitter, cached_planes, unused)
        return impl(ws, c, ray_jitter, cached_planes)

    def _plane_gate_ok(self, ws, cam2world, render_params):
        if os.environ.get('IDE3D_NO_PLANE_GATE') is not None or not ws.is_cuda or torch.is_grad_enabled() or not networks.use_hip_modconv:
            return False
        hierarchical = render_params.get('hierarchical')
        if (self.spec.hierarchical if hierarchical is None else hierarchical) or not self.renderer.fused_kernel_exists():
            return False
        if cam2world.device != ws.device or any(p.device != ws.device for p in self.renderer.decoder.parameters()):
            return False
        last = getattr(self, f'vb{self.voxel_block_resolutions[-1]}')
        if not getattr(last, 'skip_channels_last', False) or networks._hooked(self, last, self.renderer):
            return False
        from torch_utils import hip_plugin
        return last.out_channels in (64, 128) and hip_plugin.conv_arithmetic() == 'bf16x6'

    def _forward_impl(self, ws, c, render_params, noise_mode, flags, force_fp32, ray_jitter, cached_planes):
        return_seg, return_raw, return_dict = flags
        voxel_ws, block_ws = self.split_ws(ws)
        block_kwargs = dict(noise_mode=noise_mode, force_fp32=force_fp32)
        with self._pass_scope(ws, ([] if cached_planes is not None else list(zip(self.voxel_block_resolutions, voxel_ws)), list(zip(self.block_resolutions, block_ws)))):
            cam2world = c[:, :16].reshape(-1, 4, 4).to(torch.float32)
            if cached_planes is not None:
                img_v, seg_v = cached_planes
            else:
                gate = None
                if not return_dict and self._plane_gate_ok(ws, cam2world, render_params):
                    res = self.voxel_block_resolutions[-1]
                    gate = networks.PlaneGate(self.renderer.needed_cells(
                        cam2world, (res, res), fov=render_params.get('fov'), num_steps=render_params.get('num_steps'),
                        ray_start=render_params.get('ray_start'), ray_end=render_params.get('ray_end')))
                    last = getattr(self, f'vb{res}')
                    gate.with_tiles(res, res, 16 if last.out_channels == 128 else 32, 16)
                img_v, seg_v = self.backbone(voxel_ws, _plane_gate=gate, **block_kwargs)
            feat, depth, wsum = self.renderer(
                img_v, seg_v, cam2world, fov=render_params.get('fov'), num_steps=render_params.get('num_steps'),
                ray_start=render_params.get('ray_start'), ray_end=render_params.get('ray_end'),
                nerf_noise=render_params.get('nerf_noise', 0.0), jitter=ray_jitter,
                hierarchical=render_params.get('hierarchical'), importance_u=render_params.get('importance_u'))
            img, seg = self.superres(feat, block_ws, **block_kwargs)
        img_raw = feat[:, :self.img_channels]
        if return_dict:
            return dict(image=img, image_seg=seg, image_raw=img_raw, image_depth=depth, planes=(img_v, seg_v))
        if return_seg and return_raw:
            return img, seg, img_raw
        if return_seg:
            return img, seg
        if return_raw:
            return img, img_raw
        return img


@persistence.persistent_class
class TriPlaneGenerator(torch.nn.Module):

    def __init__(self, spec: Optional[GeneratorSpec] = None, **spec_overrides):
        super().__init__()
        if spec is None:
            spec = GeneratorSpec(**spec_overrides)
        elif spec_overrides:
            spec = dataclasses.replace(spec, **spec_overrides)
        self.spec = spec
        self.z_dim, self.c_dim, self.w_dim = spec.z_dim, spec.c_dim, spec.w_dim
        self.img_resolution, self.img_channels = spec.img_resolution, spec.img_channels
        self.synthesis = TriplaneSynthesisNetwork(spec)
        self.num_ws = self.synthesis.num_ws
        self.mapping = networks.MappingNetwork(z_dim=spec.z_dim, c_dim=spec.c_dim, w_dim=spec.w_dim, num_ws=self.num_ws,
                                               num_layers=spec.mapping_layers)

    def forward(self, z, c, truncation_psi=1, truncation_cutoff=None, **synthesis_kwargs):
        ws = self.mapping(z, c, truncation_psi=truncation_psi, truncation_cutoff=truncation_cutoff)
        return self.synthesis(ws, c=c, **synthesis_kwargs)



INTRINSICS = (4.2647, 0.0, 0.5, 0.0, 4.2647, 0.5, 0.0, 0.0, 1.0)


def conditioning_label(device='cpu'):
    pose = [1, 0, 0, 0, 0, 1, 0, 0, 0, 0, 1, 2.7, 0, 0, 0, 1]
    return vr.device_const(pose + list(INTRINSICS), torch.float32, device).reshape(1, -1).clone()


def camera_label(yaw, pitch=math.pi * 0.5, radius=2.7, device='cpu'):
    cam, _phi, _theta = vr.sample_camera_positions(device, n=1, r=radius, horizontal_mean=yaw + math.pi * 0.5,
                                                   vertical_mean=pitch, mode=None)
# ... 89 lines not shown
```

### include/ide3d_hip.h

```cpp
#ifndef IDE3D_HIP_H_
#define IDE3D_HIP_H_

#include <stdint.h>

#ifdef __cplusplus
extern "C" {
#endif


#define IDE3D_OK            0
#define IDE3D_EINVAL       (-1)
#define IDE3D_ENOKERNEL    (-2)
#define IDE3D_ELAUNCH      (-3)

#define IDE3D_F32  0
#define IDE3D_F16  1
#define IDE3D_BF16 2
#define IDE3D_F64  3

const char* ide3d_last_error(void);
int         ide3d_abi_version(void);
const char* ide3d_build_arch(void);
const char* ide3d_build_flags(void);
int         ide3d_exclusive_violations(void);
// ... 226 lines not shown
#define IDE3D_RASTER_CULL_FRONT 2
#define IDE3D_RASTER_BEHIND     1
#define IDE3D_RASTER_OUTSIDE    2
#define IDE3D_RASTER_BAD_INDEX  1
#define IDE3D_RASTER_DROPPED    2
int64_t ide3d_raster_workspace_bytes(int32_t N, int64_t V, int32_t H, int32_t W);
int ide3d_raster_project(const float* vertices, int64_t V, const float* world2cam, int32_t N, int32_t H, int32_t W, float fx, float fy,
                         float sx, float ox, float sy, float oy, float near, void* workspace, int64_t workspace_bytes, void* stream);
int ide3d_raster_depth(const int32_t* triangles, int64_t T, int64_t V, int32_t N, int32_t H, int32_t W, int32_t cull,
                       int32_t large_min, void* workspace, int64_t workspace_bytes, void* stream);
int ide3d_raster_shade(const float* vertices, const int32_t* triangles, int64_t V, int32_t N, int32_t H, int32_t W,
                       const float* normals, const uint8_t* colors, const int32_t* labels, const float* light, int32_t two_sided,
                       float ambient, float diffuse, const float* base_color, float bg, const void* workspace, int64_t workspace_bytes,
                       float* depth, int32_t* triangle, float* image, int32_t* label, void* stream);

typedef struct ide3d_modconv_params {
    const float* x; const float* w; const float* styles; const float* dcoefs;
    const float* noise; const float* bias; float* y;
    int32_t n, cin, cout, h, w_, k;
    float noise_strength;
    int32_t act; float alpha, gain, clamp;
    int32_t mode;
    int32_t weights_packed;
    float*  workspace;
    int64_t workspace_bytes;
    int64_t w_batch_stride;
    int32_t arith;
    const float* x_amax;
    float*       y_amax;
    int32_t      y_pitch;
} ide3d_modconv_params;

int64_t ide3d_modconv_workspace_bytes(int32_t n, int32_t cin, int32_t cout, int32_t h, int32_t w, int32_t k, int32_t mode,
                                      int32_t per_image_weights);
int ide3d_modconv2d(const ide3d_modconv_params* p, void* stream);

typedef struct ide3d_modconv_head_epilogue {
    const float* w;
    const float* bias;
    float*       y;
    int32_t      rows;
    float        clamp;
    int32_t      no_activation_output;
    float*       workspace;
    int64_t      workspace_bytes;
} ide3d_modconv_head_epilogue;
int ide3d_modconv2d_heads(const ide3d_modconv_params* p, const ide3d_modconv_head_epilogue* heads, void* stream);

typedef struct ide3d_plane_gate {
    const uint8_t* cells;
    int32_t        cells_h, cells_w;
    const int32_t* tile_list;
    int32_t        tile_h, tile_w;
} ide3d_plane_gate;
int ide3d_plane_cells(const float* rays_d_cam, const float* z_lin, const float* cam2world, int32_t n, int32_t rays_per_img, int32_t steps,
                      int32_t H, int32_t W, uint8_t* cells, void* stream);
int ide3d_plane_tile_list(const ide3d_plane_gate* gate, int32_t n, int32_t h, int32_t w, int32_t tile_h, int32_t tile_w, int32_t* list, void* stream);
int ide3d_modconv2d_heads_gated(const ide3d_modconv_params* p, const ide3d_modconv_head_epilogue* heads, const ide3d_plane_gate* gate, void* stream);

typedef struct ide3d_act_bwd_params {
    const float* dy;
    const float* y;
    float*       dz;
    const float* noise;
    float        noise_strength;
    const float* bias;
    const float* dcoefs;
    float*       ddcoefs;
    int32_t      n, c, h, w, y_pitch;
    int32_t      act;
    float        alpha, gain, clamp;
    float*       workspace;
    int64_t      workspace_bytes;
} ide3d_act_bwd_params;

int64_t ide3d_act_bwd_workspace_bytes(int32_t n, int32_t c, int32_t h, int32_t w);
int ide3d_modconv_act_backward(const ide3d_act_bwd_params* p, void* stream);

int ide3d_modconv_scale_dot(const float* x, const float* t, const float* styles, float* dx, float* dstyles,
                            int32_t n, int32_t c, int32_t h, int32_t w, float* workspace, int64_t workspace_bytes, void* stream);

int64_t ide3d_head_wgrad_workspace_bytes(int32_t n, int32_t rows, int32_t cin, int32_t h, int32_t w);
int ide3d_head_weight_grad(const float* dy, const float* x, float* dw, int32_t n, int32_t rows, int32_t cin, int32_t h, int32_t w,
                           float* workspace, int64_t workspace_bytes, void* stream);

typedef struct ide3d_wgrad_params {
    const float* g;
    const float* x;
    const float* styles;
    const float* dcoefs;
    float*       dw;
    int32_t      n, cin, cout, h, w;
    int32_t      mode;
    int32_t      arith;
    float*       workspace;
    int64_t      workspace_bytes;
} ide3d_wgrad_params;

int64_t ide3d_wgrad_workspace_bytes(int32_t n, int32_t cin, int32_t cout, int32_t h, int32_t w);
int ide3d_modconv_weight_grad(const ide3d_wgrad_params* p, void* stream);

int64_t ide3d_bias_noise_workspace_bytes(int32_t n, int32_t c, int32_t h, int32_t w);
int ide3d_bias_noise_grad(const float* dz, float* db, float* dnoise, int32_t n, int32_t c, int32_t h, int32_t w,
                          float* workspace, int64_t workspace_bytes, void* stream);

enum { IDE3D_PLAN_FP32 = 0,
       IDE3D_PLAN_SPLIT = 1,
       IDE3D_PLAN_SPLIT_TEAMS = 2,
       IDE3D_PLAN_HEAD_SPLIT = 3,
       IDE3D_PLAN_HEAD_RESIDENT = 4,
       IDE3D_PLAN_HEAD_SMALL = 5 };
// ... 236 lines not shown
```

Before: 983.1 frames/s.

## Gate the last triplane block's conv0 and FIR upsample by ray-visible cells

```diff
diff --git a/ide-3d_amd/csrc/camera.hip b/ide-3d_amd/csrc/camera.hip
--- a/ide-3d_amd/csrc/camera.hip
+++ b/ide-3d_amd/csrc/camera.hip
@@ -92,23 +92,43 @@
     }
 }
 
+struct TileListSpec { int tiles_y, tiles_x, th, tw, halo; int32_t* list; };
+struct TileListSpecs { TileListSpec s[IDE3D_PLANE_TILE_LISTS_MAX]; };
 __global__ void __launch_bounds__(1024)
-plane_tile_list_kernel(ide3d_plane_gate g, int n, int tiles_y, int tiles_x, int th, int tw, int32_t* __restrict__ list) {
+plane_tile_list_kernel(ide3d_plane_gate g, int n, TileListSpecs specs, int lds_bytes) {
+    extern __shared__ __attribute__((aligned(16))) uint8_t s_map[];
     __shared__ int s_wave[16];
-    const int tid = threadIdx.x, lane = tid & 63, wid = tid >> 6;
-    const int total = n * tiles_y * tiles_x;
+    const TileListSpec sp = specs.s[blockIdx.x];
+    int32_t* __restrict__ const list = sp.list;
+    const int tid = threadIdx.x, lane = tid & 63, wid = tid >> 6, sub = tid & 3;
+    if (lds_bytes) {
+        for (int k0 = tid * 16; k0 < lds_bytes; k0 += 4 * 16384) {
+            uint4 v[4];
+#pragma unroll
+            for (int u = 0; u < 4; ++u) if (k0 + u * 16384 < lds_bytes) v[u] = *reinterpret_cast<const uint4*>(g.cells + k0 + u * 16384);
+#pragma unroll
+            for (int u = 0; u < 4; ++u) if (k0 + u * 16384 < lds_bytes) *reinterpret_cast<uint4*>(s_map + k0 + u * 16384) = v[u];
+        }
+        __syncthreads();
+    }
+    const int total = n * sp.tiles_y * sp.tiles_x;
     int base = 0;
-    for (int t0 = 0; t0 < total; t0 += 1024) {
-        const int t = t0 + tid;
-        bool live = false;
+    for (int t0 = 0; t0 < total; t0 += 256) {
+        const int t = t0 + (tid >> 2);
+        bool any = false;
         if (t < total) {
-            const int tx = t % tiles_x, ty = (t / tiles_x) % tiles_y, img = t / (tiles_x * tiles_y);
-            const int cy0 = (ty * th) >> 2, cy1 = min((ty * th + th - 1) >> 2, g.cells_h - 1);
-            const int cx0 = (tx * tw) >> 2, cx1 = min((tx * tw + tw - 1) >> 2, g.cells_w - 1);
+            const int tx = t % sp.tiles_x, ty = (t / sp.tiles_x) % sp.tiles_y, img = t / (sp.tiles_x * sp.tiles_y);
+            const int cy0 = max(((ty * sp.th) >> 2) - sp.halo, 0), cy1 = min(((ty * sp.th + sp.th - 1) >> 2) + sp.halo, g.cells_h - 1);
+            const int cx0 = max(((tx * sp.tw) >> 2) - sp.halo, 0), cx1 = min(((tx * sp.tw + sp.tw - 1) >> 2) + sp.halo, g.cells_w - 1);
             for (int pl = 0; pl < 3; ++pl)
-                for (int cy = cy0; cy <= cy1; ++cy)
-                    for (int cx = cx0; cx <= cx1; ++cx) live |= g.cells[(((int64_t)img * 3 + pl) * g.cells_h + cy) * g.cells_w + cx] != 0;
-        }
+                for (int cy = cy0 + sub; cy <= cy1; cy += 4) {
+                    const int64_t row = (((int64_t)img * 3 + pl) * g.cells_h + cy) * g.cells_w;
+                    if (lds_bytes) { for (int cx = cx0; cx <= cx1; ++cx) any |= s_map[row + cx] != 0; }
+                    else           { for (int cx = cx0; cx <= cx1; ++cx) any |= g.cells[row + cx] != 0; }
+                }
+        }
+        const unsigned long long hit = __builtin_amdgcn_ballot_w64(any);
+        const bool live = sub == 0 && ((hit >> (lane & ~3)) & 0xfull) != 0ull;
         const unsigned long long bal = __builtin_amdgcn_ballot_w64(live);
         if (lane == 0) s_wave[wid] = __popcll(bal);
         __syncthreads();
@@ -145,13 +165,33 @@
 }
 
 extern "C" int ide3d_plane_tile_list(const ide3d_plane_gate* gate, int32_t n, int32_t h, int32_t w, int32_t tile_h, int32_t tile_w, int32_t* list, void* stream) {
-    using namespace ide3d;
-    IDE3D_CHECK_ARG(gate && gate->cells && list, "plane_tile_list: null pointer");
-    IDE3D_CHECK_ARG(n > 0 && h > 0 && w > 0 && tile_h > 0 && tile_w > 0 && tile_h % 4 == 0 && tile_w % 4 == 0, "plane_tile_list: bad shape (tiles are multiples of the 4 x 4 cell)");
+    return ide3d_plane_tile_list_halo(gate, n, h, w, tile_h, tile_w, 0, list, stream);
+}
+
+extern "C" int ide3d_plane_tile_list_halo(const ide3d_plane_gate* gate, int32_t n, int32_t h, int32_t w, int32_t tile_h, int32_t tile_w, int32_t halo_cells,
+                                          int32_t* list, void* stream) {
+    return ide3d_plane_tile_lists(gate, n, h, w, 1, &tile_h, &tile_w, &halo_cells, &list, stream);
+}
+
+extern "C" int ide3d_plane_tile_lists(const ide3d_plane_gate* gate, int32_t n, int32_t h, int32_t w, int32_t count, const int32_t* tile_h, const int32_t* tile_w,
+                                      const int32_t* halo_cells, int32_t* const* lists, void* stream) {
+    using namespace ide3d;
+    IDE3D_CHECK_ARG(gate && gate->cells && tile_h && tile_w && halo_cells && lists, "plane_tile_list: null pointer");
+    IDE3D_CHECK_ARG(count >= 1 && count <= IDE3D_PLANE_TILE_LISTS_MAX, "plane_tile_list: 1 .. %d lists per launch", IDE3D_PLANE_TILE_LISTS_MAX);
+    IDE3D_CHECK_ARG(n > 0 && h > 0 && w > 0, "plane_tile_list: bad shape");
     IDE3D_CHECK_ARG(4 * (int64_t)gate->cells_h >= h && 4 * (int64_t)gate->cells_w >= w, "plane_tile_list: the cell map does not cover the output");
-    const int tiles_y = cdiv(h, tile_h), tiles_x = cdiv(w, tile_w);
-    IDE3D_CHECK_ARG((int64_t)n * tiles_y * tiles_x < 0x7fffffffLL, "plane_tile_list: too many tiles");
-    hipLaunchKernelGGL(plane_tile_list_kernel, dim3(1), dim3(1024), 0, (hipStream_t)stream, *gate, n, tiles_y, tiles_x, tile_h, tile_w, list);
+    TileListSpecs specs{};
+    for (int k = 0; k < count; ++k) {
+        IDE3D_CHECK_ARG(lists[k], "plane_tile_list: null pointer");
+        IDE3D_CHECK_ARG(tile_h[k] > 0 && tile_w[k] > 0 && tile_h[k] % 4 == 0 && tile_w[k] % 4 == 0, "plane_tile_list: bad shape (tiles are multiples of the 4 x 4 cell)");
+        IDE3D_CHECK_ARG(halo_cells[k] >= 0 && halo_cells[k] <= 64, "plane_tile_list: the halo is 0 .. 64 cells");
+        const int tiles_y = cdiv(h, tile_h[k]), tiles_x = cdiv(w, tile_w[k]);
+        IDE3D_CHECK_ARG((int64_t)n * tiles_y * tiles_x < 0x7fffff00LL, "plane_tile_list: too many tiles");
+        specs.s[k] = TileListSpec{tiles_y, tiles_x, tile_h[k], tile_w[k], halo_cells[k], lists[k]};
+    }
+    const int64_t map_bytes = (int64_t)n * 3 * gate->cells_h * gate->cells_w;
+    const int lds_bytes = (map_bytes % 16 == 0 && map_bytes <= 60 * 1024 && ptr_aligned(gate->cells, 16)) ? (int)map_bytes : 0;
+    hipLaunchKernelGGL(plane_tile_list_kernel, dim3((unsigned)count), dim3(1024), (size_t)lds_bytes, (hipStream_t)stream, *gate, n, specs, lds_bytes);
     IDE3D_CHECK_LAUNCH("plane_tile_list");
     return IDE3D_OK;
 }
diff --git a/ide-3d_amd/csrc/common.h b/ide-3d_amd/csrc/common.h
--- a/ide-3d_amd/csrc/common.h
+++ b/ide-3d_amd/csrc/common.h
@@ -131,6 +131,8 @@
     return __builtin_amdgcn_ballot_w64(any) != 0ull;
 }
 ide3d_plane_gate resolve_plane_gate(const ide3d_plane_gate* gate);
+ide3d_plane_gate resolve_plane_gate_conv0(const ide3d_plane_gate* gate);
+constexpr int kPlaneGateConv0Halo = 1;
 
 __device__ __forceinline__ int xcd_remap(int bid, int nblocks) {
     const int xcd = bid % kNumXCD;
diff --git a/ide-3d_amd/csrc/core.hip b/ide-3d_amd/csrc/core.hip
--- a/ide-3d_amd/csrc/core.hip
+++ b/ide-3d_amd/csrc/core.hip
@@ -58,6 +58,10 @@
     if (!gate || !gate->cells || knob_live("IDE3D_NO_PLANE_GATE")) return ide3d_plane_gate{};
     return *gate;
 }
+ide3d_plane_gate resolve_plane_gate_conv0(const ide3d_plane_gate* gate) {
+    if (knob_live("IDE3D_NO_PLANE_GATE_CONV0")) return ide3d_plane_gate{};
+    return resolve_plane_gate(gate);
+}
 
 }
 
diff --git a/ide-3d_amd/csrc/modconv.hip b/ide-3d_amd/csrc/modconv.hip
--- a/ide-3d_amd/csrc/modconv.hip
+++ b/ide-3d_amd/csrc/modconv.hip
@@ -1444,18 +1444,30 @@
 
 template <int BIG, int PH, int PARTS, int F16 = 0>
 __global__ void __launch_bounds__(512, 2)
-modconv_split_pair_kernel(ide3d_modconv_params p, const u32x4* __restrict__ wp, float* __restrict__ partial, ConvGeom g, const float* __restrict__ row_unscale) {
+modconv_split_pair_kernel(ide3d_modconv_params p, const u32x4* __restrict__ wp, float* __restrict__ partial, ConvGeom g, const float* __restrict__ row_unscale,
+                          ide3d_plane_gate gate) {
     using K = SpCfg<MODE_TCONV3A, BIG, PH, PARTS, 2, 8, 1>;
     if constexpr (kSpExclusive) asm volatile("" ::: "v255");
     __shared__ __attribute__((aligned(16))) unsigned char sp_smem[K::LDS_BYTES];
     const int half_grid = (int)(gridDim.x >> 1);
     const int par = __builtin_amdgcn_readfirstlane((int)blockIdx.x >= half_grid ? 1 : 0);
-    int bid = xcd_remap((int)blockIdx.x - par * half_grid, half_grid);
+    const int hid = (int)blockIdx.x - par * half_grid;
     BlockId b;
-    b.mb = bid % g.mblocks; bid /= g.mblocks;
-    b.tile = bid % g.tile_base[4]; bid /= g.tile_base[4];
-    b.grp = bid % g.img_groups; bid /= g.img_groups;
-    b.split = bid;
+    if (gate.tile_list) {
+        const int live = __builtin_amdgcn_readfirstlane(gate.tile_list[0]) * g.mblocks;
+        if (hid >= live) return;
+        const int r = xcd_remap(hid, live);
+        const int id = __builtin_amdgcn_readfirstlane(gate.tile_list[1 + r / g.mblocks]);
+        b.mb = r % g.mblocks; b.split = 0; b.tile = id % g.tile_base[4]; b.grp = id / g.tile_base[4];
+    } else {
+        int bid = xcd_remap(hid, half_grid);
+        b.mb = bid % g.mblocks; bid /= g.mblocks;
+        b.tile = bid % g.tile_base[4]; bid /= g.tile_base[4];
+        b.grp = bid % g.img_groups; bid /= g.img_groups;
+        b.split = bid;
+        constexpr int HT = 4 * kPlaneGateConv0Halo;
+        if (gate.cells && !plane_gate_live(gate, b.grp, 0, 3, (b.tile / g.tiles_x[0]) * 2 * PH - HT, (b.tile % g.tiles_x[0]) * 2 * K::PW - HT, 2 * PH + 2 * HT, 2 * K::PW + 2 * HT)) return;
+    }
     if (par == 0) modconv_split_tile<MODE_TCONV3A, BIG, PH, PARTS, 2, 8, F16, 1, 0>(p, wp, partial, g, sp_smem, b.mb, b.tile, b.grp, b.split, g.tiles_x[0], row_unscale);
     else          modconv_split_tile<MODE_TCONV3A, BIG, PH, PARTS, 2, 8, F16, 1, 1>(p, wp, partial, g, sp_smem, b.mb, b.tile, b.grp, b.split, g.tiles_x[0], row_unscale);
 }
@@ -1762,14 +1774,14 @@
     }
 }
 template <int MODE, int BIG, int PARTS, int F16 = 0>
-static void launch_split(const ide3d_modconv_params& p, const ConvPlan& pl, const float* wp, float* partial, hipStream_t st) {
+static void launch_split(const ide3d_modconv_params& p, const ConvPlan& pl, const float* wp, float* partial, hipStream_t st, const ide3d_plane_gate& gate) {
     const ConvGeom& g = pl.g;
     const unsigned nblocks = (unsigned)((int64_t)g.mblocks * g.tile_base[4] * g.img_groups * g.split_k);
     const u32x4* wu = reinterpret_cast<const u32x4*>(wp);
     const float* ru = F16 ? wp + pl.packed_floats + (int64_t)pl.mblocks * pl.bm : nullptr;
     if constexpr (kSpExclusive) {
         if (pl.pair) {
-            if constexpr (MODE == MODE_TCONV3A) IDE3D_EXCL_LAUNCH((modconv_split_pair_kernel<BIG, (BIG == 1 ? 16 : 32), PARTS, F16>), dim3(2 * nblocks), 512, 0, st, p, wu, partial, g, ru);
+            if constexpr (MODE == MODE_TCONV3A) IDE3D_EXCL_LAUNCH((modconv_split_pair_kernel<BIG, (BIG == 1 ? 16 : 32), PARTS, F16>), dim3(2 * nblocks), 512, 0, st, p, wu, partial, g, ru, gate);
         }
         else if (pl.tile == TA4x16) {
             if constexpr (MODE == MODE_TCONV3A) {
@@ -1878,6 +1890,10 @@
 }
 
 extern "C" int ide3d_modconv2d(const ide3d_modconv_params* pp, void* stream) {
+    return ide3d_modconv2d_gated(pp, nullptr, stream);
+}
+
+extern "C" int ide3d_modconv2d_gated(const ide3d_modconv_params* pp, const ide3d_plane_gate* gate, void* stream) {
     using namespace ide3d;
     IDE3D_CHECK_ARG(pp != nullptr, "modconv2d: null params");
     const ide3d_modconv_params p = flatten_pointwise(*pp);
@@ -1921,14 +1937,19 @@
     ConvPlan pl; plan_conv(p, pl, arith_eff);
     IDE3D_CHECK_ARG(p.workspace_bytes >= (pl.packed_floats + pl.aux_floats + pl.partial_floats) * (int64_t)sizeof(float),
                     "modconv2d: workspace too small (need %lld bytes)", (long long)((pl.packed_floats + pl.aux_floats + pl.partial_floats) * sizeof(float)));
+    ide3d_plane_gate g8 = resolve_plane_gate_conv0(gate);
+    if (g8.cells && p.mode == 2)
+        IDE3D_CHECK_ARG(4 * (int64_t)g8.cells_h >= 2 * p.h && 4 * (int64_t)g8.cells_w >= 2 * p.w_, "modconv2d: the plane gate's cell map does not cover the 2h x 2w output");
+    if (!(pl.pair && pl.strip && pl.parts && pl.g.split_k == 1 && kTiles[pl.tile].images == 1 && !p.y_amax)) g8 = ide3d_plane_gate{};
+    if (!g8.cells || g8.tile_h != 2 * kTiles[pl.tile].rows || g8.tile_w != 2 * kTiles[pl.tile].cols || g8.halo_cells != kPlaneGateConv0Halo) g8.tile_list = nullptr;
     hipStream_t st = (hipStream_t)stream;
     float* wp = p.workspace;
     float* partial = p.workspace + pl.packed_floats + pl.aux_floats;
     if (pl.parts) {
         if (!p.weights_packed) pack_split_weights(p, pl, wp, st);
 #define IDE3D_SP_DISPATCH(M) \
-        do { if (pl.big == 1) { if (pl.f16) launch_split<M, 1, 2, 1>(p, pl, wp, partial, st); else if (pl.parts == 2) launch_split<M, 1, 2>(p, pl, wp, partial, st); else launch_split<M, 1, 3>(p, pl, wp, partial, st); } \
-             else             { if (pl.f16) launch_split<M, 2, 2, 1>(p, pl, wp, partial, st); else if (pl.parts == 2) launch_split<M, 2, 2>(p, pl, wp, partial, st); else launch_split<M, 2, 3>(p, pl, wp, partial, st); } } while (0)
+        do { if (pl.big == 1) { if (pl.f16) launch_split<M, 1, 2, 1>(p, pl, wp, partial, st, g8); else if (pl.parts == 2) launch_split<M, 1, 2>(p, pl, wp, partial, st, g8); else launch_split<M, 1, 3>(p, pl, wp, partial, st, g8); } \
+             else             { if (pl.f16) launch_split<M, 2, 2, 1>(p, pl, wp, partial, st, g8); else if (pl.parts == 2) launch_split<M, 2, 2>(p, pl, wp, partial, st, g8); else launch_split<M, 2, 3>(p, pl, wp, partial, st, g8); } } while (0)
         if (pl.mode == MODE_CONV3) IDE3D_SP_DISPATCH(MODE_CONV3); else IDE3D_SP_DISPATCH(MODE_TCONV3A);
 #undef IDE3D_SP_DISPATCH
     } else {
@@ -2014,7 +2035,7 @@
     e.gate = resolve_plane_gate(gate);
     if (e.gate.cells)
         IDE3D_CHECK_ARG(4 * (int64_t)e.gate.cells_h >= p.h && 4 * (int64_t)e.gate.cells_w >= p.w_, "modconv2d_heads: the plane gate's cell map does not cover the output");
-    if (!e.gate.cells || e.gate.tile_h != ph || e.gate.tile_w != 16) e.gate.tile_list = nullptr;
+    if (!e.gate.cells || e.gate.tile_h != ph || e.gate.tile_w != 16 || e.gate.halo_cells != 0) e.gate.tile_list = nullptr;
     const ConvGeom& g = pl.g;
     const unsigned nblocks = (unsigned)((int64_t)g.mblocks * g.tile_base[4] * g.img_groups * g.split_k);
     const u32x4* wu = reinterpret_cast<const u32x4*>(p.workspace);
diff --git a/ide-3d_amd/csrc/upfirdn2d.hip b/ide-3d_amd/csrc/upfirdn2d.hip
--- a/ide-3d_amd/csrc/upfirdn2d.hip
+++ b/ide-3d_amd/csrc/upfirdn2d.hip
@@ -491,6 +491,117 @@
 }
 
 __global__ void __launch_bounds__(256)
+fir44_blocks_kernel(ide3d_upfirdn2d_params p, ide3d_upfirdn2d_epilogue ep, const int32_t* __restrict__ list, int tiles_x, int tiles_y) {
+    constexpr int B = 32, LW = 40, LH = B + 3, NV = LW / 4, NLD = (LH * NV + 63) / 64;
+    __shared__ __attribute__((aligned(16))) float s_all[4 * LH * LW];
+    const int count = __builtin_amdgcn_readfirstlane(list[0]);
+    const int items = count * p.c, wgs = (items + 3) >> 2;
+    if ((int)blockIdx.x >= wgs) return;
+    const int wave = __builtin_amdgcn_readfirstlane((int)(threadIdx.x >> 6)), lane = (int)(threadIdx.x & 63u);
+    const int item = xcd_remap(blockIdx.x, wgs) * 4 + wave;
+    const bool have = item < items;
+    float* const s_in = s_all + wave * (LH * LW);
+    float g[4][4];
+#pragma unroll
+    for (int ky = 0; ky < 4; ++ky)
+#pragma unroll
+        for (int kx = 0; kx < 4; ++kx) {
+            const int fy = p.flip ? ky : 3 - ky, fx = p.flip ? kx : 3 - kx;
+            g[ky][kx] = p.f[fy * p.f_stride[0] + fx * p.f_stride[1]] * p.gain;
+        }
+    const int c = have ? item / count : 0;
+    int id = have ? __builtin_amdgcn_readfirstlane(list[1 + (item - c * count)]) : 0;
+    const int tx_i = id % tiles_x; id /= tiles_x;
+    const int ty_i = id % tiles_y;
+    const int n = id / tiles_y;
+    const int in_x0 = tx_i * B - p.pad_x0, in_y0 = ty_i * B - p.pad_y0;
+    const int x_al = in_x0 & ~3, xoff = in_x0 - x_al;
+    const float* __restrict__ xp = (const float*)p.x + n * p.x_stride[0] + c * p.x_stride[1];
+    const unsigned pitch = (unsigned)p.x_stride[2];
+    const int w4 = (p.in_w + 3) & ~3;
+    if (have) {
+        float4 v4[NLD];
+        int gy[NLD], gx[NLD];
+#pragma unroll
+        for (int k = 0; k < NLD; ++k) {
+            const int idx = lane + k * 64;
+            const int ly = idx / NV, lv = idx - ly * NV;
+            gy[k] = in_y0 + ly; gx[k] = x_al + 4 * lv;
+            const unsigned cy_ = (unsigned)min(max(gy[k], 0), p.in_h - 1), cx_ = (unsigned)min(max(gx[k], 0), w4 - 4);
+            v4[k] = *reinterpret_cast<const float4*>(xp + (cy_ * pitch + cx_));
+        }
+#pragma unroll
+        for (int k = 0; k < NLD; ++k) {
+            const int idx = lane + k * 64;
+            if (idx < LH * NV) {
+                const bool rowok = (unsigned)gy[k] < (unsigned)p.in_h;
+                float4 w = v4[k];
+                w.x = (rowok && (unsigned)(gx[k] + 0) < (unsigned)p.in_w) ? w.x : 0.f;
+                w.y = (rowok && (unsigned)(gx[k] + 1) < (unsigned)p.in_w) ? w.y : 0.f;
+                w.z = (rowok && (unsigned)(gx[k] + 2) < (unsigned)p.in_w) ? w.z : 0.f;
+                w.w = (rowok && (unsigned)(gx[k] + 3) < (unsigned)p.in_w) ? w.w : 0.f;
+                *reinterpret_cast<float4*>(s_in + 4 * idx) = w;
+            }
+        }
+    }
+    __syncthreads();
+    if (!have) return;
+    const int tx = lane & 7, ty = lane >> 3;
+    float win[7][7];
+    {
+        const float* wsrc = s_in + (ty * 4) * LW + tx * 4 + xoff;
+#pragma unroll
+        for (int wy = 0; wy < 7; ++wy)
+#pragma unroll
+            for (int wx = 0; wx < 7; ++wx) win[wy][wx] = wsrc[wy * LW + wx];
+    }
+    const bool has_noise = ep.noise != nullptr, act_on = ep.fused_act != 0;
+    const float nstr = ep.noise_strength;
+    const float bias = (act_on && ep.bias) ? ((const float*)ep.bias)[c] : 0.f;
+    const bool lrelu = act_on && ep.act == 3, lrelu_max = lrelu && ep.alpha >= 0.f && ep.alpha <= 1.f;
+    const float alpha = ep.alpha, again = act_on ? ep.act_gain : 1.f;
+    const bool clamp_on = act_on && ep.clamp >= 0.f;
+    const float cl = ep.clamp;
+    float* __restrict__ yp = (float*)p.y + n * p.y_stride[0] + c * p.y_stride[1];
+    const unsigned ypitch = (unsigned)p.y_stride[2];
+    const int ox0 = tx_i * B + tx * 4, oy0 = ty_i * B + ty * 4;
+    const bool full = ox0 + 4 <= p.out_w;
+    if (full) {
+#pragma unroll
+        for (int cy = 0; cy < 4; ++cy) {
+            const int oy = oy0 + cy;
+            if (oy >= p.out_h) break;
+            float row[4];
+#pragma unroll
+            for (int cx = 0; cx < 4; ++cx) {
+                float acc = 0.f;
+#pragma unroll
+                for (int ky = 0; ky < 4; ++ky)
+#pragma unroll
+                    for (int kx = 0; kx < 4; ++kx) acc += win[cy + ky][cx + kx] * g[ky][kx];
+                row[cx] = acc;
+            }
+            if (has_noise) {
+                const float4 a = *reinterpret_cast<const float4*>(ep.noise + ((unsigned)oy * (unsigned)p.out_w + (unsigned)ox0));
+                row[0] += a.x * nstr; row[1] += a.y * nstr; row[2] += a.z * nstr; row[3] += a.w * nstr;
+            }
+            if (act_on) {
+#pragma unroll
+                for (int j = 0; j < 4; ++j) {
+                    float v = row[j] + bias;
+                    if (lrelu_max) v = fmaxf(v, v * alpha);
+                    else if (lrelu) v = (v > 0.f) ? v : v * alpha;
+                    v *= again;
+                    if (clamp_on) v = (v > cl) ? cl : ((v < -cl) ? -cl : v);
+                    row[j] = v;
+                }
+            }
+            *reinterpret_cast<float4*>(yp + ((unsigned)oy * ypitch + (unsigned)ox0)) = make_float4(row[0], row[1], row[2], row[3]);
+        }
+    }
+}
+
+__global__ void __launch_bounds__(256)
 fir_up2_kernel(ide3d_upfirdn2d_params p, ide3d_upfirdn2d_epilogue ep, int tiles_x, int tiles_y) {
     using AX = Axis<2, 1, 4>;
     constexpr int TCX = 64, TCY = 16, LW = 72, LH = TCY + 2, NV = LW / 4, NLD = (LH * NV + 255) / 256;
@@ -609,10 +720,10 @@
 }
 
 
-static bool fir44_applies(const ide3d_upfirdn2d_params& p, const ide3d_upfirdn2d_epilogue& ep) {
+static bool fir44_applies(const ide3d_upfirdn2d_params& p, const ide3d_upfirdn2d_epilogue& ep, int min_w = 65) {
     const bool off = knob_live("IDE3D_FIR_NO_LEAN");
     if (off || p.dtype != IDE3D_F32 || p.f_w != 4 || p.f_h != 4 || p.up_x != 1 || p.up_y != 1 || p.down_x != 1 || p.down_y != 1) return false;
-    if (p.x_stride[3] != 1 || p.y_stride[3] != 1 || ep.add || p.out_w <= 64 || (p.out_w & 3)) return false;
+    if (p.x_stride[3] != 1 || p.y_stride[3] != 1 || ep.add || p.out_w < min_w || (p.out_w & 3)) return false;
     const int64_t pitch = p.x_stride[2], w4 = (p.in_w + 3) & ~3;
     if ((pitch & 3) || pitch < w4 || w4 > (p.in_w > p.x_row_floats ? p.in_w : p.x_row_floats)) return false;
     if ((reinterpret_cast<uintptr_t>(p.x) & 15) || (p.x_stride[0] & 3) || (p.x_stride[1] & 3)) return false;
@@ -855,3 +966,23 @@
 extern "C" int ide3d_upfirdn2d_ex(const ide3d_upfirdn2d_params* pp, const ide3d_upfirdn2d_epilogue* ep, void* stream) {
     return upfirdn2d_entry(pp, ep, stream);
 }
+
+extern "C" int ide3d_upfirdn2d_ex_gated(const ide3d_upfirdn2d_params* pp, const ide3d_upfirdn2d_epilogue* epp, const ide3d_plane_gate* gate, void* stream) {
+    using namespace ide3d;
+    ide3d_upfirdn2d_epilogue ep;
+    ide3d_upfirdn2d_plan_info plan;
+    const int rc = upfirdn2d_checked_plan(pp, epp, &ep, &plan);
+    if (rc != IDE3D_OK) return rc;
+    const ide3d_upfirdn2d_params& p = *pp;
+    const ide3d_plane_gate g = resolve_plane_gate_conv0(gate);
+    if (g.cells)
+        IDE3D_CHECK_ARG(4 * (int64_t)g.cells_h >= p.out_h && 4 * (int64_t)g.cells_w >= p.out_w, "upfirdn2d: the plane gate's cell map does not cover the output");
+    const int tiles_x = cdiv(p.out_w, 32), tiles_y = cdiv(p.out_h, 32);
+    if (!g.cells || !g.tile_list || g.tile_h != 32 || g.tile_w != 32 || g.halo_cells != kPlaneGateConv0Halo || p.pad_x0 != 1 || p.pad_y0 != 1 || ep.y_amax ||
+        !fir44_applies(p, ep, 4) || (int64_t)tiles_x * tiles_y * p.n * p.c / 4 + 1 > 0x7fffffffLL)
+        return upfirdn2d_entry(pp, epp, stream);
+    const unsigned grid = (unsigned)(((int64_t)tiles_x * tiles_y * p.n * p.c + 3) / 4);
+    hipLaunchKernelGGL(fir44_blocks_kernel, dim3(grid), dim3(256), 0, (hipStream_t)stream, p, ep, g.tile_list, tiles_x, tiles_y);
+    IDE3D_CHECK_LAUNCH("upfirdn2d (fir44, gated)");
+    return IDE3D_OK;
+}
diff --git a/ide-3d_amd/torch_utils/hip_plugin.py b/ide-3d_amd/torch_utils/hip_plugin.py
--- a/ide-3d_amd/torch_utils/hip_plugin.py
+++ b/ide-3d_amd/torch_utils/hip_plugin.py
@@ -379,6 +379,10 @@
             'ide3d_modconv2d_heads_gated': [ctypes.POINTER(_ModconvParams), ctypes.POINTER(_ModconvHeadEpilogue), ctypes.POINTER(_PlaneGate), vp],
             'ide3d_plane_cells': [vp, vp, vp, i32, i32, i32, i32, i32, vp, vp],
             'ide3d_plane_tile_list': [ctypes.POINTER(_PlaneGate), i32, i32, i32, i32, i32, vp, vp],
+            'ide3d_plane_tile_list_halo': [ctypes.POINTER(_PlaneGate), i32, i32, i32, i32, i32, i32, vp, vp],
+            'ide3d_plane_tile_lists': [ctypes.POINTER(_PlaneGate), i32, i32, i32, i32, vp, vp, vp, vp, vp],
+            'ide3d_modconv2d_gated': [ctypes.POINTER(_ModconvParams), ctypes.POINTER(_PlaneGate), vp],
+            'ide3d_upfirdn2d_ex_gated': [ctypes.POINTER(_UpfirdnParams), ctypes.POINTER(_UpfirdnEpilogue), ctypes.POINTER(_PlaneGate), vp],
             'ide3d_skip_upsample_add_cl_gated': [vp, ctypes.POINTER(i64 * 4), vp, ctypes.POINTER(i64 * 4), i32, i32, i32, i32, vp, ctypes.POINTER(_PlaneGate), vp],
             'ide3d_modconv_plan': [ctypes.POINTER(_ModconvParams), ctypes.POINTER(_ModconvPlanInfo)],
             'ide3d_modconv_workspace_bytes': [i32, i32, i32, i32, i32, i32, i32, i32],
@@ -491,6 +495,7 @@
     'ide3d_render_merged_param_grad_workspace_bytes', 'ide3d_render_rays_merged_backward',
     'ide3d_raster_workspace_bytes', 'ide3d_raster_project', 'ide3d_raster_depth', 'ide3d_raster_shade',
     'ide3d_plane_cells', 'ide3d_plane_tile_list', 'ide3d_modconv2d_heads_gated', 'ide3d_skip_upsample_add_cl_gated',
+    'ide3d_plane_tile_list_halo', 'ide3d_plane_tile_lists', 'ide3d_modconv2d_gated', 'ide3d_upfirdn2d_ex_gated',
 )
 
 
@@ -715,7 +720,7 @@
 
     @staticmethod
     def upfirdn2d_ex(x, f, upx, upy, downx, downy, padx0, padx1, pady0, pady1, flip, gain,
-                     add=None, noise=None, noise_strength=1.0, bias=None, act=None, alpha=0.0, act_gain=1.0, clamp=-1.0, y_amax=None):
+                     add=None, noise=None, noise_strength=1.0, bias=None, act=None, alpha=0.0, act_gain=1.0, clamp=-1.0, y_amax=None, gate=None, out=None):
         _require(x.is_cuda, 'x must reside on CUDA device')
         _require(f.device == x.device, 'f must reside on the same device as x')
         _require(f.dtype == torch.float32, 'f must be float32')
@@ -726,10 +731,12 @@
         _require(f.ndim == 2, 'f must be rank 2')
         p, (n, c, oh, ow), cl = _upfirdn_params(tuple(x.shape), x.stride(), x.dtype, x.data_ptr(), _row_floats_readable(x), tuple(f.shape), f.stride(), f.data_ptr(),
                                                 upx, upy, downx, downy, padx0, padx1, pady0, pady1, flip, gain)
-        y = torch.empty([n, c, oh, ow], dtype=x.dtype, device=x.device,
-                        memory_format=torch.channels_last if cl else torch.contiguous_format)
+        y = out if out is not None else torch.empty([n, c, oh, ow], dtype=x.dtype, device=x.device,
+                                                    memory_format=torch.channels_last if cl else torch.contiguous_format)
+        _require(y.dtype == x.dtype and y.device == x.device and tuple(y.shape) == (n, c, oh, ow)
+                 and y.is_contiguous(memory_format=torch.channels_last if cl else torch.contiguous_format), 'out must match the output in shape, dtype and memory format')
         p.y, p.y_stride = y.data_ptr(), _i64x4(y.stride())
-        plain = add is None and noise is None and act is None and y_amax is None
+        plain = add is None and noise is None and act is None and y_amax is None and gate is None
         with _dev_guard(x.device):
             if plain:
                 rc = load().ide3d_upfirdn2d(ctypes.byref(p), _stream(x))
@@ -754,7 +761,10 @@
                         bias = bias.to(x.dtype).contiguous(); keep.append(bias)
                         _require(bias.numel() == c, 'bias must have one entry per channel')
                         ep.bias = bias.data_ptr()
-                rc = load().ide3d_upfirdn2d_ex(ctypes.byref(p), ctypes.byref(ep), _stream(x))
+                if gate is not None:
+                    rc = load().ide3d_upfirdn2d_ex_gated(ctypes.byref(p), ctypes.byref(ep), ctypes.byref(_plane_gate(gate, n, oh, ow)), _stream(x))
+                else:
+                    rc = load().ide3d_upfirdn2d_ex(ctypes.byref(p), ctypes.byref(ep), _stream(x))
         _check(rc, 'upfirdn2d')
         return y
 
@@ -1307,7 +1317,8 @@
         return p, ent, keep
 
     @staticmethod
-    def modconv2d(x, w, styles, dcoefs, noise, noise_strength, bias, act, alpha, gain, clamp, mode=0, arith=0, x_amax=None, y_amax=None, pad_rows=False):
+    def modconv2d(x, w, styles, dcoefs, noise, noise_strength, bias, act, alpha, gain, clamp, mode=0, arith=0, x_amax=None, y_amax=None, pad_rows=False,
+                  gate=None, out=None):
         for t in (x, w):
             _require(t.is_cuda and t.dtype == torch.float32 and t.is_contiguous(), 'modconv2d: contiguous float32 CUDA tensors required')
         _require(w.device == x.device, 'modconv2d: w must reside on the same device as x')
@@ -1321,7 +1332,10 @@
         _require(mode != 1 or (k == 3 and h >= 3 and wd >= 3), 'modconv2d: mode 1 is a 3x3 stride-2 convolution on an input of at least 3x3')
         oh, ow = (2 * h + 1, 2 * wd + 1) if mode == 2 else (((h - 3) // 2 + 1, (wd - 3) // 2 + 1) if mode == 1 else (h, wd))
         pitch = (ow + 3) // 4 * 4 if (pad_rows and mode == 2) else ow
-        y = torch.empty([n, cout, oh, pitch], dtype=torch.float32, device=x.device)
+        y = torch.empty([n, cout, oh, pitch], dtype=torch.float32, device=x.device) if out is None else out
+        _require(y.dtype == torch.float32 and y.device == x.device and tuple(y.shape) == (n, cout, oh, pitch) and y.is_contiguous(),
+                 f'modconv2d: out must be a contiguous float32 [{n}, {cout}, {oh}, {pitch}] tensor on the device of x')
+        _require(gate is None or mode == 2, 'modconv2d: the plane gate belongs to the transposed convolution (mode 2)')
         lib = load()
         arith = int(arith) or int(lib.ide3d_get_conv_arithmetic())
         if arith == 16 and x_amax is None:
@@ -1329,7 +1343,10 @@
         p, ent, keep = ModconvPlugin._params(lib, x, w, y, styles, dcoefs, noise, noise_strength, bias, act, alpha, gain, clamp, mode, arith, x_amax, y_amax)
         p.y_pitch = pitch if pitch != ow else 0
         with _dev_guard(x.device):
-            rc = lib.ide3d_modconv2d(ctypes.byref(p), _stream(x))
+            if gate is not None:
+                rc = lib.ide3d_modconv2d_gated(ctypes.byref(p), ctypes.byref(_plane_gate(gate, n, 2 * h, 2 * wd)), _stream(x))
+            else:
+                rc = lib.ide3d_modconv2d(ctypes.byref(p), _stream(x))
         _check(rc, 'modconv2d')
         ModconvPlugin._ws.mark_packed(ent, () if per_image else (w,))
         return y if pitch == ow else y[..., :ow]
@@ -2655,10 +2672,13 @@
 
 class _PlaneGate(ctypes.Structure):
     _fields_ = [('cells', ctypes.c_void_p), ('cells_h', ctypes.c_int32), ('cells_w', ctypes.c_int32),
-                ('tile_list', ctypes.c_void_p), ('tile_h', ctypes.c_int32), ('tile_w', ctypes.c_int32)]
+                ('tile_list', ctypes.c_void_p), ('tile_h', ctypes.c_int32), ('tile_w', ctypes.c_int32), ('halo_cells', ctypes.c_int32)]
 
 
 def _plane_gate(gate, n, h, w):
+    halo = 0
+    if isinstance(gate, tuple) and len(gate) == 4:
+        gate, halo = gate[:3], int(gate[3])
     cells, tiles, tile_hw = gate if isinstance(gate, tuple) else (gate, None, None)
     _require(cells.is_cuda and cells.dtype == torch.uint8 and cells.is_contiguous() and tuple(cells.shape) == (n, 3, (h + 3) // 4, (w + 3) // 4),
              f'plane gate: cells must be a contiguous uint8 CUDA tensor [{n}, 3, {(h + 3) // 4}, {(w + 3) // 4}], got {list(cells.shape)} {cells.dtype}')
@@ -2668,18 +2688,34 @@
         th, tw = tile_hw
         _require(tiles.is_cuda and tiles.dtype == torch.int32 and tiles.is_contiguous() and tiles.device == cells.device
                  and tiles.numel() == 1 + n * (-(-h // th)) * (-(-w // tw)), 'plane gate: the tile list must be plane_tile_list(cells, h, w, tile_h, tile_w)')
-        g.tile_list, g.tile_h, g.tile_w = tiles.data_ptr(), th, tw
+        g.tile_list, g.tile_h, g.tile_w, g.halo_cells = tiles.data_ptr(), th, tw, halo
     return g
 
 
-def plane_tile_list(cells, h, w, tile_h, tile_w):
+def plane_tile_list(cells, h, w, tile_h, tile_w, halo_cells=0):
     n = cells.shape[0]
     g = _plane_gate(cells, n, h, w)
     out = torch.empty([1 + n * (-(-h // tile_h)) * (-(-w // tile_w))], dtype=torch.int32, device=cells.device)
     with _dev_guard(cells.device):
-        rc = load().ide3d_plane_tile_list(ctypes.byref(g), n, int(h), int(w), int(tile_h), int(tile_w), _ptr(out), _stream(cells))
+        if halo_cells:
+            rc = load().ide3d_plane_tile_list_halo(ctypes.byref(g), n, int(h), int(w), int(tile_h), int(tile_w), int(halo_cells), _ptr(out), _stream(cells))
+        else:
+            rc = load().ide3d_plane_tile_list(ctypes.byref(g), n, int(h), int(w), int(tile_h), int(tile_w), _ptr(out), _stream(cells))
     _check(rc, 'plane_tile_list')
     return out
+
+
+def plane_tile_lists(cells, h, w, specs):
+    n, k = cells.shape[0], len(specs)
+    g = _plane_gate(cells, n, h, w)
+    outs = [torch.empty([1 + n * (-(-h // th)) * (-(-w // tw))], dtype=torch.int32, device=cells.device) for th, tw, _ in specs]
+    arr = lambda vals: (ctypes.c_int32 * k)(*[int(v) for v in vals])
+    ths, tws, halos = arr(s[0] for s in specs), arr(s[1] for s in specs), arr(s[2] for s in specs)
+    ptrs = (ctypes.c_void_p * k)(*[o.data_ptr() for o in outs])
+    with _dev_guard(cells.device):
+        rc = load().ide3d_plane_tile_lists(ctypes.byref(g), n, int(h), int(w), k, ths, tws, halos, ptrs, _stream(cells))
+    _check(rc, 'plane_tile_list')
+    return outs
 
 
 def plane_cells(rays_d_cam, z_lin, cam2world, H, W):
diff --git a/ide-3d_amd/training/graph_cache.py b/ide-3d_amd/training/graph_cache.py
--- a/ide-3d_amd/training/graph_cache.py
+++ b/ide-3d_amd/training/graph_cache.py
@@ -15,7 +15,8 @@
 STATS = collections.Counter()
 
 
-_PASS_ENV = ('IDE3D_NO_SKIP_MERGE', 'IDE3D_NO_STYLE_PREFETCH', 'IDE3D_NO_STYLE_BATCH', 'IDE3D_NO_LOWRES_GROUP', 'IDE3D_NO_PLANE_GATE')
+_PASS_ENV = ('IDE3D_NO_SKIP_MERGE', 'IDE3D_NO_STYLE_PREFETCH', 'IDE3D_NO_STYLE_BATCH', 'IDE3D_NO_LOWRES_GROUP', 'IDE3D_NO_PLANE_GATE',
+             'IDE3D_NO_PLANE_GATE_CONV0')
 
 
 def _env_int(name, default):
diff --git a/ide-3d_amd/training/networks.py b/ide-3d_amd/training/networks.py
--- a/ide-3d_amd/training/networks.py
+++ b/ide-3d_amd/training/networks.py
@@ -556,33 +556,69 @@
 
 class PlaneGate:
 
+    CONV0_HALO = 1
+
     def __init__(self, cells):
         self.cells, self.taken = cells, False
         self._lists = {}
 
-    def with_tiles(self, h, w, tile_h, tile_w):
+    def with_tiles(self, h, w, tile_h, tile_w, halo=0):
         from torch_utils import hip_plugin
-        key = (h, w, tile_h, tile_w)
+        key = (h, w, tile_h, tile_w, halo)
         if key not in self._lists:
-            self._lists[key] = hip_plugin.plane_tile_list(self.cells, h, w, tile_h, tile_w)
-        return self.cells, self._lists[key], (tile_h, tile_w)
-
-
-def _conv1_dual_head(block, x, w1, w_shared, want_x, noise_mode='random', gain=1, input_noise=None, _plane_gate=None, **unused):
+            self._lists[key] = hip_plugin.plane_tile_list(self.cells, h, w, tile_h, tile_w, halo)
+        return (self.cells, self._lists[key], (tile_h, tile_w), halo) if halo else (self.cells, self._lists[key], (tile_h, tile_w))
+
+    def prepare(self, h, w, specs):
+        from torch_utils import hip_plugin
+        todo = [s for s in specs if (h, w, *s) not in self._lists]
+        if todo:
+            for s, lst in zip(todo, hip_plugin.plane_tile_lists(self.cells, h, w, todo)):
+                self._lists[(h, w, *s)] = lst
+
+    def for_conv0(self, h, w):
+        return self.with_tiles(h, w, 32, 32, self.CONV0_HALO)
+
+
+def _conv1_dual_head_ok(block, n, hw, like, w1, w_shared, noise_mode='random', input_noise=None, **unused):
     c1, tr, ts = block.conv1, block.torgb, block.toseg
     if not (use_hip_modconv and type(c1) is SynthesisLayer and c1.up == 1 and c1.padding == 1 and c1.weight.shape[2:] == (3, 3)
             and c1.activation in ('linear', 'lrelu') and tr.weight.shape[2] == 1 and tr.conv_clamp == ts.conv_clamp
-            and x.ndim == 4 and x.shape[0] == w1.shape[0] == w_shared.shape[0]
-            and _inference_on_gpu(x, w1, w_shared, *_layer_params(c1), *_head_params(tr, ts))
+            and like.ndim == 4 and n == w1.shape[0] == w_shared.shape[0]
+            and _inference_on_gpu(like, w1, w_shared, *_layer_params(c1), *_head_params(tr, ts))
             and not _hooked(block, c1, tr, ts) and _modconv_init()):
-        return None
+        return False
     from torch_utils import hip_plugin
     if hip_plugin.conv_arithmetic() != 'bf16x6':
+        return False
+    if c1.use_noise and noise_mode != 'none' and (input_noise is not None or noise_mode != 'const' or tuple(c1.noise_const.shape) != tuple(hw)):
+        return False
+    return True
+
+
+def _conv0_gate_ok(block, x, ws_list, disable_rgb, dtype, **layer_kwargs):
+    c0 = block.conv0
+    if os.environ.get('IDE3D_NO_PLANE_GATE_CONV0') is not None or os.environ.get('IDE3D_NO_PLANE_GATE') is not None or 'IDE3D_MODCONV_NO_HEAD_FUSION' in os.environ:
+        return False
+    if not ((block.is_last or block.architecture == 'skip') and not disable_rgb and dtype == torch.float32 and not block.use_single_layer and block.num_conv == 2
+            and type(c0) is SynthesisLayer and c0.up == 2 and c0.padding == 1 and c0.weight.shape[2:] == (3, 3) and c0.activation in ('linear', 'lrelu')
+            and x.ndim == 4 and not _hooked(c0) and block.conv1.weight.shape[0] in (64, 128) and block.conv1.weight.shape[1] == c0.weight.shape[0]):
+        return False
+    n, hw = x.shape[0], (2 * x.shape[2], 2 * x.shape[3])
+    if not _conv1_dual_head_ok(block, n, hw, x, ws_list[1], ws_list[block.num_conv], **layer_kwargs):
+        return False
+    from torch_utils import hip_plugin
+    c1 = block.conv1
+    rows = block.torgb.weight.shape[0] + block.toseg.weight.shape[0]
+    return (n, c1.weight.shape[1], c1.weight.shape[0], hw[0], hw[1], rows, 6) not in hip_plugin.ModconvPlugin._heads_declined
+
+
+def _conv1_dual_head(block, x, w1, w_shared, want_x, noise_mode='random', gain=1, input_noise=None, _plane_gate=None, _dense_x=None, **unused):
+    c1, tr, ts = block.conv1, block.torgb, block.toseg
+    if not _conv1_dual_head_ok(block, x.shape[0], tuple(x.shape[2:]), x, w1, w_shared, noise_mode=noise_mode, input_noise=input_noise):
         return None
     noise = None
     if c1.use_noise and noise_mode != 'none':
-        if input_noise is not None or noise_mode != 'const' or tuple(c1.noise_const.shape) != tuple(x.shape[2:]):
-            return None
         noise = _scaled_const_noise(c1.noise_const, c1.noise_strength)
     styles, dcoefs = _styles_and_dcoefs(c1.affine, w1, c1.weight, True)
     if dcoefs is None:
@@ -604,6 +640,8 @@
     if gate is not None and out is not None:
         _plane_gate.taken = True
     if out is None:
+        if _dense_x is not None:
+            x = _dense_x()
         x = _modconv_bias_act(x, c1.weight, styles, True, noise, 1.0, bias, c1.activation, act_gain, act_clamp, dcoefs=dcoefs)
         return x, _dual_head(x, tr, ts, w_shared, wcat=wcat)
     x, y = out
@@ -1024,7 +1062,7 @@
             self.noise_strength = torch.nn.Parameter(torch.zeros([]))
         self.bias = torch.nn.Parameter(torch.zeros([out_channels]))
 
-    def forward(self, x, w, noise_mode='random', fused_modconv=True, gain=1, input_noise=None, **unused_kwargs):
+    def forward(self, x, w, noise_mode='random', fused_modconv=True, gain=1, input_noise=None, _plane_gate=None, **unused_kwargs):
         assert noise_mode in ['random', 'const', 'none']
         styles, dcoefs_pre = _styles_and_dcoefs(self.affine, w, self.weight, True)
         if styles.size(0) < x.size(0):
@@ -1056,15 +1094,21 @@
                 and _inference_on_gpu(x, self.weight, styles, self.bias, noise) and _modconv_init()):
             dcoefs = dcoefs_pre if dcoefs_pre is not None else _demod_coefs(self.weight, styles)
             xc = x.contiguous()
+            one_fir_launch = self.activation in ('linear', 'lrelu') and (noise is None or (noise.ndim == 2 and noise.shape == (2 * x.shape[2], 2 * x.shape[3])))
+            gate = None
+            if _plane_gate is not None and one_fir_launch and os.environ.get('IDE3D_NO_PLANE_GATE_CONV0') is None:
+                from torch_utils import hip_plugin
+                if hip_plugin.conv_arithmetic() == 'bf16x6':
+                    gate = _plane_gate.for_conv0(2 * x.shape[2], 2 * x.shape[3])
             y = _modconv_plugin.modconv2d(xc, self.weight.contiguous(), styles.contiguous(), dcoefs,
-                                          None, 0.0, None, 1, 0.0, 1.0, -1.0, mode=2, x_amax=(_amax_of(x) if xc is x else None), pad_rows=True)
+                                          None, 0.0, None, 1, 0.0, 1.0, -1.0, mode=2, x_amax=(_amax_of(x) if xc is x else None), pad_rows=True, gate=gate)
             spec = bias_act.activation_funcs[self.activation]
-            if self.activation in ('linear', 'lrelu') and (noise is None or (noise.ndim == 2 and noise.shape == (2 * x.shape[2], 2 * x.shape[3]))):
+            if one_fir_launch:
                 amax = _amax_wanted(y)
                 return _with_amax(_upfirdn_plugin().upfirdn2d_ex(y, self.resample_filter, 1, 1, 1, 1, 1, 1, 1, 1, False, 4.0,
                                                                  noise=noise, noise_strength=1.0, bias=self.bias, act=spec.cuda_idx,
                                                                  alpha=spec.def_alpha, act_gain=act_gain,
-                                                                 clamp=(-1.0 if act_clamp is None else act_clamp), y_amax=amax), amax)
+                                                                 clamp=(-1.0 if act_clamp is None else act_clamp), y_amax=amax, gate=gate), amax)
             y = upfirdn2d.upfirdn2d(y, self.resample_filter, padding=[1, 1, 1, 1], gain=4)
             if noise is not None:
                 y = y.add_(noise)
@@ -1194,18 +1238,27 @@
         else:
             x = x.to(dtype=dtype, memory_format=memory_format)
             layer_kwargs['input_noise'] = block_noise[:, 0:1] if block_noise is not None else None
+            dense_conv0 = None
             if resume_after_conv0:
                 next(w_iter)
             else:
-                x = self.conv0(x, next(w_iter), fused_modconv=fused_modconv, **layer_kwargs)
+                x_in, w0, kw0 = x, next(w_iter), dict(layer_kwargs)
+                kw1 = dict(layer_kwargs, input_noise=(block_noise[:, 1:2] if block_noise is not None else None))
+                if plane_gate is not None and x_unused and _conv0_gate_ok(self, x_in, ws_list, disable_rgb, dtype, **kw1):
+                    dense_conv0 = lambda: self.conv0(x_in, w0, fused_modconv=fused_modconv, **kw0)
+                    x = self.conv0(x_in, w0, fused_modconv=fused_modconv, _plane_gate=plane_gate, **kw0)
+                else:
+                    x = self.conv0(x_in, w0, fused_modconv=fused_modconv, **kw0)
             if not self.use_single_layer:
                 layer_kwargs['input_noise'] = block_noise[:, 1:2] if block_noise is not None else None
                 w1 = next(w_iter)
                 if (self.is_last or self.architecture == 'skip') and not disable_rgb and dtype == torch.float32:
-                    fused = _conv1_dual_head(self, x, w1, ws_list[self.num_conv], not x_unused, _plane_gate=plane_gate, **layer_kwargs)
+                    fused = _conv1_dual_head(self, x, w1, ws_list[self.num_conv], not x_unused, _plane_gate=plane_gate, _dense_x=dense_conv0, **layer_kwargs)
                 if fused is not None:
                     x, fused_heads = fused
                 else:
+                    if dense_conv0 is not None:
+                        x = dense_conv0()
                     x = self.conv1(x, w1, fused_modconv=fused_modconv, **layer_kwargs)
 
         w_shared = next(w_iter) if (self.is_last or self.architecture == 'skip') else None
diff --git a/ide-3d_amd/training/triplane.py b/ide-3d_amd/training/triplane.py
--- a/ide-3d_amd/training/triplane.py
+++ b/ide-3d_amd/training/triplane.py
@@ -454,7 +454,10 @@
                         cam2world, (res, res), fov=render_params.get('fov'), num_steps=render_params.get('num_steps'),
                         ray_start=render_params.get('ray_start'), ray_end=render_params.get('ray_end')))
                     last = getattr(self, f'vb{res}')
-                    gate.with_tiles(res, res, 16 if last.out_channels == 128 else 32, 16)
+                    specs = [(16 if last.out_channels == 128 else 32, 16, 0)]
+                    if os.environ.get('IDE3D_NO_PLANE_GATE_CONV0') is None:
+                        specs.append((32, 32, networks.PlaneGate.CONV0_HALO))
+                    gate.prepare(res, res, specs)
                 img_v, seg_v = self.backbone(voxel_ws, _plane_gate=gate, **block_kwargs)
             feat, depth, wsum = self.renderer(
                 img_v, seg_v, cam2world, fov=render_params.get('fov'), num_steps=render_params.get('num_steps'),
diff --git a/include/ide3d_hip.h b/include/ide3d_hip.h
--- a/include/ide3d_hip.h
+++ b/include/ide3d_hip.h
@@ -302,11 +302,19 @@
     int32_t        cells_h, cells_w;
     const int32_t* tile_list;
     int32_t        tile_h, tile_w;
+    int32_t        halo_cells;
 } ide3d_plane_gate;
 int ide3d_plane_cells(const float* rays_d_cam, const float* z_lin, const float* cam2world, int32_t n, int32_t rays_per_img, int32_t steps,
                       int32_t H, int32_t W, uint8_t* cells, void* stream);
 int ide3d_plane_tile_list(const ide3d_plane_gate* gate, int32_t n, int32_t h, int32_t w, int32_t tile_h, int32_t tile_w, int32_t* list, void* stream);
 int ide3d_modconv2d_heads_gated(const ide3d_modconv_params* p, const ide3d_modconv_head_epilogue* heads, const ide3d_plane_gate* gate, void* stream);
+int ide3d_plane_tile_list_halo(const ide3d_plane_gate* gate, int32_t n, int32_t h, int32_t w, int32_t tile_h, int32_t tile_w, int32_t halo_cells,
+                               int32_t* list, void* stream);
+#define IDE3D_PLANE_TILE_LISTS_MAX 4
+int ide3d_plane_tile_lists(const ide3d_plane_gate* gate, int32_t n, int32_t h, int32_t w, int32_t count, const int32_t* tile_h, const int32_t* tile_w,
+                           const int32_t* halo_cells, int32_t* const* lists, void* stream);
+int ide3d_modconv2d_gated(const ide3d_modconv_params* p, const ide3d_plane_gate* gate, void* stream);
+int ide3d_upfirdn2d_ex_gated(const ide3d_upfirdn2d_params* p, const ide3d_upfirdn2d_epilogue* ep, const ide3d_plane_gate* gate, void* stream);
 
 typedef struct ide3d_act_bwd_params {
     const float* dy;
```

Result: no change. 992.4 frames/s, median of 6 (+0.9%).
